# rasd3/TODA

Hardware: AMD Instinct MI355X
Metric: LiDAR training samples/sec (higher is better)
Workload: dtype f32

## Files before the change

include/toda.h:

```cpp
#ifndef TODA_H_
#define TODA_H_

#include <stddef.h>
#include <stdint.h>

#ifdef __cplusplus
extern "C" {
#endif

#define TODA_OK 0
#define TODA_EINVAL (-1)
#define TODA_EWORKSPACE (-2)
#define TODA_ELAUNCH (-3)
#define TODA_EFAULT (-4)

#define TODA_FAULT_BN2D 1u
#define TODA_FAULT_WINO 2u
#define TODA_FAULT_FPS 4u

const char* toda_last_error(void);
int toda_abi_version(void);
int toda_device_fault(void);

size_t toda_voxelize_workspace_bytes(int n_points, int max_voxels);
int toda_voxelize_hard(const float* points, int n, int c,
                       const float* range_host ,
                       const float* vsize_host ,
                       const int32_t* grid_host ,
                       int max_pts, int max_voxels,
                       float* voxels, int32_t* coords_zyx, int32_t* num_pts,
                       int32_t* m_dev, void* ws, size_t ws_bytes, void* stream);
size_t toda_voxelize_batch_workspace_bytes(int batch, int n_cap);
int toda_voxelize_batch(const float* const* points_host, const int32_t* n_points_host, int batch, int n_cap,
                        int c, int row_stride,
                        const float* range_host, const float* vsize_host, const int32_t* grid_host,
                        int max_pts, int max_voxels,
                        float* voxels, int32_t* coords_bzyx, int32_t* num_pts, int32_t* counts_dev,
                        void* ws, size_t ws_bytes, int ws_clean, void* stream);

int toda_mean_vfe_fwd(const float* voxels, const float* num_pts, int m, int p, int c,
                      float* out, void* stream);
int toda_mean_vfe_bwd(const float* grad_out, const float* num_pts, int m, int p, int c,
                      float* grad_voxels, void* stream);

size_t toda_dynvox_workspace_bytes(int n, int batch, const int32_t* grid_host, int pillar);
int toda_dynvox_count(const float* points, int n, int width, int batch, const float* range_host, const float* vsize_host,
                      const int32_t* grid_host, int pillar, int32_t* counts_dev, void* ws, size_t ws_bytes, void* stream);
int toda_dynvox_index(const float* points, int n, int width, int batch, const float* range_host, const float* vsize_host,
                      const int32_t* grid_host, int pillar, int m, int k, uint8_t* keep, int32_t* rows, int32_t* inv,
                      int32_t* seg_pts, int32_t* seg_off, int32_t* cnt, int32_t* coords, void* ws, size_t ws_bytes,
                      void* stream);
int toda_dynvox_seg_sum(const float* src, int ld, int col0, int ncol, const int32_t* rowmap, const int32_t* seg_off,
                        const int32_t* seg_pts, int m, int divide, float* out, void* stream);
int toda_dynvox_pillar_decorate(const float* points, int width, const int32_t* rows, const int32_t* inv,
                                const int32_t* coords, const float* mean, int k, const float* vsize_host,
                                const float* offset_host, int use_abs_xyz, int with_dist, float* out, int f, void* stream);
int toda_dynvox_seg_max_fwd(const float* x, int c, const int32_t* seg_off, const int32_t* seg_pts, int m, float* out,
                            int32_t* arg, void* stream);
int toda_dynvox_seg_max_bwd(const float* gout, const int32_t* arg, int m, int c, int k, float* gx, void* stream);
int toda_dynvox_gather_concat(const float* x, const float* xmax, const int32_t* inv, int k, int c, float* out, void* stream);

size_t toda_gridindex_bytes(int batch, const int32_t* shape_host );
int toda_gridindex_from_coords(const int32_t* idx, int n, const int32_t* n_dev,
                               int batch, const int32_t* shape_host,
                               void* gi, int32_t* rowof, void* stream);
int toda_gridindex_from_coords_unordered(const int32_t* idx, int n, const int32_t* n_dev,
                                         int batch, const int32_t* shape_host,
                                         void* gi, int32_t* rowof, int gi_clean, void* stream);
int toda_gridindex_clear(const int32_t* idx, int n, const int32_t* n_dev, int batch,
                         const int32_t* shape_host, void* gi, void* stream);
int toda_gridindex_from_conv(const int32_t* idx_in, int n_in, const int32_t* n_in_dev,
                             int batch, const int32_t* shape_in_host,
                             const int32_t* ksize_host, const int32_t* stride_host,
                             const int32_t* pad_host, const int32_t* shape_out_host,
                             void* gi_out, int32_t* idx_out, int32_t* n_out_dev,
                             int out_cap, void* stream);
int toda_gridindex_from_bitmap(const void* gi_in, int batch, const int32_t* shape_in_host,
                               const int32_t* ksize_host, const int32_t* stride_host,
                               const int32_t* pad_host, const int32_t* shape_out_host,
                               void* gi_out, int32_t* idx_out, int32_t* n_out_dev,
                               int out_cap, int in_rows_marked, void* stream);

int toda_rulebook_subm(const int32_t* idx, int n, int batch, const int32_t* shape_host,
                       const int32_t* ksize_host, const int32_t* dilation_host,
                       const void* gi, const int32_t* rowof,
                       int32_t* nbr, int32_t* pair_cnt, int cnt_zeroed, void* stream);
int toda_rulebook_conv(const int32_t* idx_in, int n_in, int batch,
                       const int32_t* shape_in_host, const int32_t* ksize_host,
                       const int32_t* stride_host, const int32_t* pad_host,
                       const int32_t* shape_out_host, const void* gi_out, int n_out,
                       int32_t* nbr_o2i, int32_t* nbr_i2o, int32_t* pair_cnt,
                       const int32_t* idx_out, const void* gi_in, const int32_t* rowof_in,
                       int cnt_zeroed, void* stream);

size_t toda_spconv_packed_weight_floats(int k_vol, int c_gather, int c_produce);
int toda_matrix_path(void);
int toda_set_matrix_path(int mode);
int toda_spconv_split_supported(int c_gather, int c_produce);
int toda_spconv_pack_weight(const float* w, int cout, int k_vol, int cin,
                            int transpose, int flip_k, float* wp, void* stream);
int toda_spconv_pack_weights(int n, const float* const* w_host, const int32_t* cout_host, const int32_t* k_vol_host,
                             const int32_t* cin_host, const int32_t* transpose_host, const int32_t* flip_k_host,
                             float* const* wp_host, void* stream);
int toda_spconv_gather_gemm(const float* in, int n_in, int c_gather, const float* wp,
                            const int32_t* nbr, int n_out, int k_vol, int c_produce,
                            const float* bias , float* out, void* stream);
int toda_spconv_gather_gemm_ordered(const float* in, int n_in, int c_gather, const float* wp,
                                    const int32_t* nbr, int n_out, int k_vol, int c_produce,
                                    const float* bias, float* out, const int32_t* order, void* stream);

int toda_rulebook_class_order(const int32_t* in_coords, int n_in, const int32_t* stride_host, const int32_t* padding_host,
                              int32_t* order, unsigned char* cls_sorted, void* stream);
int toda_spconv_gather_gemm_classed(const float* in, int n_in, int c_gather, const float* wp, const int32_t* nbr, int n_out,
                                    int k_vol, int c_produce, const float* bias, float* out, const int32_t* order,
                                    const unsigned char* cls_sorted, const int32_t* ksize_host, const int32_t* stride_host,
                                    const int32_t* padding_host, void* stream);
int toda_spconv_gather_gemm_compact_supported(int c_gather, int c_produce, int k_vol);
int toda_spconv_gather_gemm_compact(const float* in, int n_in, int c_gather, const float* w, int w_cout, int w_cin,
                                    int transpose, int flip_k, const int32_t* nbr, int n_out, int k_vol, int c_produce,
                                    const float* bias , float* out, void* stream);
size_t toda_spconv_gather_gemm_compact_stats_doubles(int n_out, int c_produce);
int toda_spconv_gather_gemm_compact_stats(const float* in, int n_in, int c_gather, const float* w, int w_cout, int w_cin,
                                          int transpose, int flip_k, const int32_t* nbr, int n_out, int k_vol,
                                          int c_produce, const float* bias , float* out, double* sums,
                                          size_t sums_doubles, int* blocks_out , void* stream);

size_t toda_spconv_wgrad_workspace_bytes(int n_out, int k_vol, int cin, int cout);
int toda_spconv_wgrad(const float* in, int n_in, const float* dout, const int32_t* nbr,
                      int n_out, int k_vol, int cin, int cout, float* dw,
                      void* ws, size_t ws_bytes, void* stream);
int toda_sparse_to_dense_fwd(const float* feat, const int32_t* idx, int n, int c,
                             int batch, const int32_t* shape_host, float* dense, void* stream);
int toda_sparse_to_dense_bwd(const float* grad_dense, const int32_t* idx, int n, int c,
                             int batch, const int32_t* shape_host, float* grad_feat, void* stream);

int toda_pillar_scatter_fwd(const float* feat, const int32_t* idx, int n, int c,
                            int batch, int ny, int nx, float* canvas, void* stream);
int toda_pillar_scatter_bwd(const float* grad_canvas, const int32_t* idx, int n, int c,
                            int batch, int ny, int nx, float* grad_feat, void* stream);

size_t toda_rows_reduce_doubles(int n, int c);
int toda_rows_moments(const float* x, int n, int c, double* sums ,
                      void* stream);
int toda_rows_affine_act(const float* x, const float* scale, const float* shift,
                         const float* residual , int n, int c, int relu,
                         float* y, void* stream);

int toda_bn_finalize(const double* sums , int n, int c,
                     const float* gamma, const float* beta, float* running_mean ,
                     float* running_var , float momentum, float eps, int training,
                     float* mean, float* invstd, float* scale, float* shift, void* stream);
int toda_bn_finalize_partials(double* sums, int blocks, int n, int c, const float* gamma, const float* beta,
                              float* running_mean , float* running_var , float momentum, float eps,
                              float* mean, float* invstd, float* scale, float* shift, void* stream);
int toda_rows_bn_bwd(const float* dy, const float* x, const float* stats, const float* gamma,
                     int n, int c, int relu, double* sums , float* dx,
                     void* stream);

int toda_rows_bn_bwd_res(const float* dy, const float* x, const float* residual , const float* stats,
                         const float* gamma, int n, int c, int relu, double* sums, float* dx,
                         float* dres , void* stream);
size_t toda_rows_bn_bwd_colsum_doubles(int n, int c);
int toda_rows_bn_bwd_res_colsum(const float* dy, const float* x, const float* residual , const float* stats,
                                const float* gamma, int n, int c, int relu, double* sums, float* dx,
                                float* dres , double* colsum_ws , float* dx_colsum ,
                                void* stream);

int toda_bn2d_supported(int batch, int c, int hw);
size_t toda_bn2d_sync_bytes(void);
int toda_bn2d_fwd(const float* x, int batch, int c, int hw, const float* gamma, const float* beta,
                  float* running_mean , float* running_var , float momentum, float eps, int relu,
                  float* y, float* save, void* sync , unsigned epoch, void* stream);
int toda_bn2d_bwd(const float* x, const float* dy, int batch, int c, int hw, const float* gamma, const float* beta,
                  const float* save, int relu, float* dx, float* dgamma, float* dbeta, void* sync ,
                  unsigned epoch, void* stream);
int toda_bn2d_fwd_into(const float* x, int batch, int c, int hw, const float* gamma, const float* beta,
                       float* running_mean , float* running_var , float momentum, float eps, int relu,
                       float* y, int y_channels, int y_channel0, float* save, void* sync , unsigned epoch,
                       void* stream);
int toda_bn2d_bwd_from(const float* x, const float* dy, int dy_channels, int dy_channel0, int batch, int c, int hw,
                       const float* gamma, const float* beta, const float* save, int relu, float* dx, float* dgamma,
                       float* dbeta, void* sync , unsigned epoch, void* stream);

int toda_center_assign(const float* gt_boxes, int batch, int n_gt, int code_size,
                       int num_classes, int fm_w, int fm_h,
                       const float* range_host , const float* vsize_host ,
                       int fm_stride, int max_objs, double gaussian_overlap, int min_radius,
                       float* heatmap ,
                       float* ret_boxes ,
                       int64_t* inds , int64_t* mask ,
                       void* stream);

int toda_boxes_iou_bev(const float* boxes_a, int na, const float* boxes_b, int nb,
                       float* iou , void* stream);
int toda_boxes_overlap_bev(const float* boxes_a, int na, const float* boxes_b, int nb,
                           float* overlap , void* stream);
size_t toda_nms_workspace_bytes(int n);
int toda_nms_rotated(const float* boxes_sorted, int n, float thresh, int64_t* keep ,
                     int32_t* n_keep_dev, void* ws, size_t ws_bytes, void* stream);

int toda_roi_grid_pool_bev(const float* feat, int B, int C, int H, int W, const float* rois, int N, int roi_stride,
                           float min_x, float min_y, float step_x, float step_y, int grid_size, float* out, void* stream);
int toda_roi_iou3d_max(const float* rois, int B, int N, int roi_stride, const int64_t* roi_labels, const float* gt, int M,
                       int gt_stride, int by_class, float* max_iou , int64_t* argmax , void* stream);

int toda_voxel_query(const float* new_xyz, const int32_t* new_coords, int M, const float* xyz, int N, const void* gi, const int32_t* rowof,
                     int batch, const int32_t* shape_host, float radius, const int32_t* ranges_host, int nsample, int32_t* idx,
                     uint8_t* empty, void* stream);
size_t toda_voxel_pool_moments_doubles(void);
int toda_voxel_pool_moments(const int32_t* idx, const uint8_t* empty, int M, int nsample, const float* xyz, int N, const float* new_xyz,
                            double* ws, void* stream);
int toda_voxel_pool_fwd(const float* f, int N, int C, const int32_t* idx, const uint8_t* empty, int M, int nsample, const float* xyz,
                        const float* new_xyz, const float* ab, float* out, uint8_t* arg, void* stream);
size_t toda_voxel_pool_table_bytes(int M, int nsample, int N);
int toda_voxel_pool_table(const int32_t* idx, const uint8_t* empty, int M, int nsample, int N, int32_t* off, int32_t* ent, void* ws,
                          size_t ws_bytes, void* stream);
int toda_voxel_pool_bwd_feat(const float* gout, const uint8_t* arg, int M, int nsample, int C, const int32_t* off, const int32_t* ent,
                             int N, float* gf, void* stream);
size_t toda_voxel_pool_bwd_pos_doubles(int C);
int toda_voxel_pool_bwd_pos(const float* gout, const uint8_t* arg, const int32_t* idx, const uint8_t* empty, int M, int nsample, int C,
                            const float* xyz, int N, const float* new_xyz, double* ws, float* gab, void* stream);

int toda_fps_resident_blocks(void);
size_t toda_fps_workspace_bytes(int batch, int npoint);
int toda_fps(const float* xyz, const int32_t* starts_host, int batch, int npoint, int mode, float* temp, int32_t* idx, void* ws,
             size_t ws_bytes, void* stream);
int toda_ball_query_stack(const float* xyz, int N, const int32_t* xyz_start, const float* new_xyz, const int32_t* new_start, int batch,
                          int M, int nr, const float* radii_host, const int32_t* nsample_host, int32_t* const* idx_host,
                          uint8_t* const* empty_host, void* stream);
int toda_sa_gather_fwd(const float* P, int N, int C, const float* wd, const int32_t* idx, const uint8_t* empty, int M, int nsample,
                       const float* xyz, const float* new_xyz, float* z, void* stream);
int toda_sa_gather_bwd_feat(const float* gz, int M, int nsample, int C, const int32_t* off, const int32_t* ent, int N, float* gP,
                            void* stream);
size_t toda_sa_gather_bwd_pos_doubles(int C);
int toda_sa_gather_bwd_pos(const float* gz, const int32_t* idx, const uint8_t* empty, int M, int nsample, int C, const float* xyz, int N,
                           const float* new_xyz, double* ws, float* gwd, void* stream);
int toda_sa_max_fwd(const float* y, int M, int nsample, int C, float* out, uint8_t* arg, void* stream);
int toda_sa_max_bwd(const float* g, const uint8_t* arg, int M, int nsample, int C, float* gy, void* stream);
int toda_bev_interp_fwd(const float* map, int B, int C, int H, int W, const float* xy, const int32_t* bidx, int K, float* out,
                        int32_t* taps, float* wts, void* stream);
int toda_bev_interp_bwd(const float* g, int K, int C, const int32_t* off, const int32_t* ent, const float* wts, int B, int H, int W,
                        float* gmap, void* stream);

int toda_points_in_boxes(const float* points, int n, const int32_t* n_dev, int c, const float* boxes,
                         int k, int box_stride, int mode, int32_t* flags, void* stream);
int toda_points_sector(const float* points, int n, const int32_t* n_dev, int c, double lo, double hi,
                       int32_t* flags, void* stream);
int toda_points_rect(const float* points, int n, const int32_t* n_dev, int c, const double* lo_xy_host,
                     const double* hi_xy_host, int closed, int32_t* flags, void* stream);
int toda_points_polar_cell(const float* points, int n, const int32_t* n_dev, int c, float phase,
                           const double* yaw_edges_host, int n_yaw, const double* dis_edges_host, int n_dis,
                           float dis_lo, float dis_hi, int32_t* cell, void* stream);
int toda_points_polar_select(const float* points, int n, const int32_t* n_dev, int c, double lo, double hi, int yaw_mode,
                             int dis_mode, double dis_th, const float* pitch_range_dev, int32_t* flags, void* stream);
size_t toda_points_pitch_range_workspace_bytes(void);
int toda_points_pitch_range(const float* points, int n, const int32_t* n_dev, int c, float* range_dev, void* ws,
                            size_t ws_bytes, void* stream);
int toda_points_pitch_band(const float* points, int n, const int32_t* n_dev, int c, float z_offset, float clip_lo,
                           float clip_hi, const double* edges_host, int n_bands, int32_t* band, void* stream);
size_t toda_rows_select_workspace_bytes(int n);
int toda_rows_select_append(const float* src, int n, const int32_t* n_dev, int c, const int32_t* keys,
                            int match, int invert, float* dst, int cap_rows, int32_t* cursor_dev,
                            void* ws, size_t ws_bytes, void* stream);
int toda_points_rotate_z(const float* src, int n, const int32_t* n_dev, int c, double cosv, double sinv,
                         float* dst, void* stream);
int toda_points_world_transform(const float* src, int n, const int32_t* n_dev, int c, int flip_x, int flip_y,
                                int rotate, float cosv, float sinv, int rescale, float scale, float* dst,
                                void* stream);

int toda_spconv_gather_gemm_stats_supported(int c_gather, int c_produce);
size_t toda_spconv_gather_gemm_stats_doubles(int n_out, int c_produce);
int toda_spconv_gather_gemm_stats(const float* in, int n_in, int c_gather, const float* packed_w, const int32_t* nbr,
                                  int n_out, int k_vol, int c_produce, const float* bias, float* out, double* sums,
                                  size_t sums_doubles, void* stream);
int toda_spconv_gather_gemm_stats_partials(const float* in, int n_in, int c_gather, const float* wp, const int32_t* nbr,
                                           int n_out, int k_vol, int c_produce, const float* bias , float* out,
                                           double* sums, size_t sums_doubles, int* blocks_out, void* stream);

int toda_conv3x3_supported(int batch, int cin, int cout, int H, int W);
size_t toda_conv3x3_weight_floats(int cout, int cin);
int toda_conv3x3_transform_weight(const float* w, int cout, int cin, int mode, float* u, void* stream);
size_t toda_conv3x3_workspace_bytes(void);
size_t toda_conv3x3_wgrad_workspace_bytes(int batch, int cin, int cout, int H, int W);
int toda_conv3x3_wgrad(const float* x, const float* dy, int batch, int cin, int cout, int H, int W, float* dw,
                       void* ws, size_t ws_bytes, void* stream);
int toda_conv3x3_fwd(const float* x, const float* u, const float* bias, int batch, int cin, int cout, int H,
                     int W, float* y, void* ws, size_t ws_bytes, void* stream);

int toda_conv3x3s2_supported(int batch, int cin, int cout, int H, int W);
int toda_conv3x3s2_fwd(const float* x, const float* w, int batch, int cin, int cout, int H, int W, float* y, void* stream);
int toda_conv3x3s2_dgrad(const float* dy, const float* w, int batch, int cin, int cout, int H, int W, float* dx, void* stream);
size_t toda_conv3x3s2_wgrad_workspace_bytes(int batch, int cin, int cout, int H, int W);
int toda_conv3x3s2_wgrad(const float* x, const float* dy, int batch, int cin, int cout, int H, int W, float* dw, void* ws,
                         size_t ws_bytes, void* stream);
int toda_deconv_supported(int batch, int cin, int cout, int H, int W, int s);
int toda_deconv_fwd(const float* x, const float* w, int batch, int cin, int cout, int H, int W, int s, float* y, void* stream);
int toda_deconv_dgrad(const float* dy, const float* w, int batch, int cin, int cout, int H, int W, int s, float* dx, void* stream);
size_t toda_deconv_wgrad_workspace_bytes(int batch, int cin, int cout, int H, int W, int s);
int toda_deconv_wgrad(const float* x, const float* dy, int batch, int cin, int cout, int H, int W, int s, float* dw, void* ws,
                      size_t ws_bytes, void* stream);

size_t toda_center_loss_workspace_bytes(int batch, int classes, int H, int W, int max_objs, int code_size);
int toda_center_loss_fwd(const float* hm_logits, const float* heatmap, int batch, int classes, int H, int W, int n_branch,
                         const float* const* reg_maps_host, const int32_t* reg_channels_host, const int64_t* inds,
                         const int64_t* mask, const float* target_boxes, int max_objs, int code_size,
                         const float* code_weights_host, float cls_weight, float loc_weight, float* hm_prob, float* out4,
                         void* ws, size_t ws_bytes, void* stream);
int toda_center_loss_bwd(const float* out4, const float* up_hm, const float* up_loc, int batch, int classes, int H, int W,
                         int n_branch, float* const* reg_grads_host, const int32_t* reg_channels_host, const int64_t* inds,
                         const int64_t* mask, int max_objs, int code_size, const float* code_weights_host, float cls_weight, float loc_weight,
                         float* hm_grad, const void* ws, size_t ws_bytes, void* stream);

int toda_conv3x3_narrow_supported(int batch, int cin, int cout, int H, int W);
int toda_conv3x3_narrow_fwd(int n, const float* const* x_host, const float* const* w_host, const float* const* bias_host,
                            const int32_t* cout_host, int batch, int cin, int H, int W, long long x_image_stride,
                            float* const* y_host, void* stream);
int toda_conv3x3_narrow_dgrad(int n, const float* const* dy_host, const float* const* w_host, const int32_t* cout_host,
                              int batch, int cin, int H, int W, long long dx_image_stride, float* const* dx_host, void* stream);
size_t toda_conv3x3_narrow_wgrad_workspace_bytes(int n, int batch, int cin, int H);
int toda_conv3x3_narrow_wgrad(int n, const float* const* x_host, const float* const* dy_host, const int32_t* cout_host,
                              int batch, int cin, int H, int W, long long x_image_stride, float* out, void* ws, size_t ws_bytes,
                              void* stream);

int toda_timing_begin(int capacity);
int toda_timing_end(float* ms_out_host, int cap, int* n_out_host);

int toda_clip_adam_chunk(void);
int toda_clip_adam_step(const unsigned long long* param, const unsigned long long* grad, const unsigned long long* exp_avg,
                        const unsigned long long* exp_avg_sq, const long long* numel, const int* chunk_tensor,
                        const long long* chunk_off, int n_chunks, double* partial, float* norm_out, float max_norm,
                        float lr, float beta1, float beta2, float eps, float weight_decay, int step, void* stream);

#ifdef __cplusplus
}
#endif
#endif
```

toda_amd/csrc/dense.hip:

```cpp
#include "common.h"

namespace toda {

typedef float f32x4 __attribute__((ext_vector_type(4)));

constexpr int DN_BLOCK = 256;
constexpr int DN_ROWS = 64;
constexpr int DN_CH = 32;

struct DenseGeom {
    int D, H, W;
    int pillar;
};

__device__ __forceinline__ long long spatial_offset(const int4 q, const DenseGeom& g) {
    if (g.pillar) return (long long)q.y + (long long)q.z * g.W + q.w;
    return ((long long)q.y * g.H + q.z) * g.W + q.w;
}

template <bool FWD>
__global__ void __launch_bounds__(DN_BLOCK)
dense_tile_kernel(float* __restrict__ feat, const int4* __restrict__ idx, int n, int c, DenseGeom g,
                  float* __restrict__ dense) {
    __shared__ float tile[DN_CH][DN_ROWS + 1];
    __shared__ long long base[DN_ROWS];
    const int row0 = blockIdx.x * DN_ROWS, c0 = blockIdx.y * DN_CH;
    const long long vol = (long long)g.D * g.H * g.W;
    if (threadIdx.x < DN_ROWS) {
        const int r = row0 + threadIdx.x;
        long long b = -1;
        if (r < n) {
            const int4 q = idx[r];
            b = (long long)q.x * c * vol + spatial_offset(q, g);
        }
        base[threadIdx.x] = b;
    }
    const int fr = threadIdx.x >> 2, fc = (threadIdx.x & 3) * 8;
    const int dr = threadIdx.x & 63, dc = threadIdx.x >> 6;
    if (FWD) {
        if (row0 + fr < n) {
#pragma unroll
            for (int j = 0; j < 8; ++j) {
                const int ch = c0 + fc + j;
                tile[fc + j][fr] = ch < c ? feat[(size_t)(row0 + fr) * c + ch] : 0.f;
            }
        }
        __syncthreads();
        const long long b = base[dr];
        if (b >= 0) {
#pragma unroll
            for (int j = 0; j < DN_CH / 4; ++j) {
                const int ch = dc + 4 * j;
                if (c0 + ch < c) dense[b + (long long)(c0 + ch) * vol] = tile[ch][dr];
            }
        }
    } else {
        __syncthreads();
        const long long b = base[dr];
#pragma unroll
        for (int j = 0; j < DN_CH / 4; ++j) {
            const int ch = dc + 4 * j;
            tile[ch][dr] = (b >= 0 && c0 + ch < c) ? dense[b + (long long)(c0 + ch) * vol] : 0.f;
        }
        __syncthreads();
        if (row0 + fr < n) {
#pragma unroll
            for (int j = 0; j < 8; ++j) {
                const int ch = c0 + fc + j;
                if (ch < c) feat[(size_t)(row0 + fr) * c + ch] = tile[fc + j][fr];
            }
        }
    }
}

#ifndef TODA_MOM_ROWS
#define TODA_MOM_ROWS 256
#endif
constexpr int MOM_ROWS = TODA_MOM_ROWS;
constexpr int MOM_MAX_BLOCKS = 2048;

template <class Load>
__device__ __forceinline__ void rows_reduce2(int n, int c, int rows_per_block, Load load, double* __restrict__ sums) {
    __shared__ float sh[2][DN_BLOCK][4];
    const int lanes = c >> 2;
    const int rows_par = DN_BLOCK / lanes;
    const int cl = threadIdx.x % lanes, rsub = threadIdx.x / lanes;
    const int row_begin = blockIdx.x * rows_per_block;
    const int row_end = min(n, row_begin + rows_per_block);
    f32x4 s0 = f32x4{0.f, 0.f, 0.f, 0.f}, t0 = s0, s1 = s0, t1 = s0;
    int r = row_begin + rsub;
    for (; r + rows_par < row_end; r += 2 * rows_par) {
        f32x4 a, b, a2, b2;
        load(r, cl, a, b);
        load(r + rows_par, cl, a2, b2);
        s0 += a;
        t0 += b;
        s1 += a2;
        t1 += b2;
    }
    if (r < row_end) {
        f32x4 a, b;
        load(r, cl, a, b);
        s0 += a;
        t0 += b;
    }
    s0 += s1;
    t0 += t1;
#pragma unroll
    for (int j = 0; j < 4; ++j) {
        sh[0][threadIdx.x][j] = s0[j];
        sh[1][threadIdx.x][j] = t0[j];
    }
    __syncthreads();
    if (threadIdx.x < 2 * c) {
        const int q = threadIdx.x / c, ch = threadIdx.x % c;
        double acc = 0.0;
        for (int j = 0; j < rows_par; ++j) acc += sh[q][j * lanes + (ch >> 2)][ch & 3];
        sums[2 * c + (size_t)(q * c + ch) * gridDim.x + blockIdx.x] = acc;
    }
}

__global__ void __launch_bounds__(DN_BLOCK)
fold_partials_kernel(double* __restrict__ sums, int blocks, int cols) {
    __shared__ double part[DN_BLOCK];
    const double* src = sums + cols + (size_t)blockIdx.x * blocks;
    double acc = 0.0;
    for (int g = threadIdx.x; g < blocks; g += DN_BLOCK) acc += src[g];
    part[threadIdx.x] = acc;
    __syncthreads();
    for (int w = DN_BLOCK / 2; w > 0; w >>= 1) {
        if (threadIdx.x < w) part[threadIdx.x] += part[threadIdx.x + w];
        __syncthreads();
    }
    if (threadIdx.x == 0) sums[blockIdx.x] = part[0];
}

static inline void reduce_plan(int n, int* blocks, int* rows_per_block) {
    const int g = cdiv(n > 0 ? n : 1, MOM_ROWS);
    *blocks = g < MOM_MAX_BLOCKS ? g : MOM_MAX_BLOCKS;
    *rows_per_block = cdiv(n > 0 ? n : 1, *blocks);
}

__global__ void __launch_bounds__(DN_BLOCK)
rows_moments_kernel(const float* __restrict__ x, int n, int c, int rows_per_block, double* __restrict__ sums) {
    const f32x4* x4 = reinterpret_cast<const f32x4*>(x);
    const int lanes = c >> 2;
    rows_reduce2(n, c, rows_per_block, [&](int r, int cl, f32x4& a, f32x4& b) {
        a = x4[(size_t)r * lanes + cl];
        b = a * a;
    }, sums);
}

constexpr int EW_BLOCKS = 2048;

__global__ void __launch_bounds__(DN_BLOCK)
rows_affine_act_kernel(const f32x4* __restrict__ x, const float* __restrict__ scale, const float* __restrict__ shift,
                       const f32x4* __restrict__ res, long long n4, int c, int relu, f32x4* __restrict__ y) {
    const long long t0 = (long long)blockIdx.x * DN_BLOCK + threadIdx.x;
    const long long stride = (long long)gridDim.x * DN_BLOCK;
    const int ch = (int)((t0 * 4) % c);
    const f32x4 sc = *reinterpret_cast<const f32x4*>(scale + ch), sf = *reinterpret_cast<const f32x4*>(shift + ch);
    for (long long t = t0; t < n4; t += stride) {
        f32x4 v = x[t] * sc + sf;
        if (res) v += res[t];
        if (relu) {
#pragma unroll
            for (int j = 0; j < 4; ++j) v[j] = fmaxf(v[j], 0.f);
        }
        y[t] = v;
    }
}

__global__ void __launch_bounds__(DN_BLOCK)
rows_bn_bwd_reduce_kernel(const float* __restrict__ dy, const float* __restrict__ x, const float* __restrict__ res,
                          const float* __restrict__ stats, int n, int c, int relu, int rows_per_block,
                          double* __restrict__ sums) {
    const f32x4* dy4 = reinterpret_cast<const f32x4*>(dy);
    const f32x4* x4 = reinterpret_cast<const f32x4*>(x);
    const f32x4* r4 = reinterpret_cast<const f32x4*>(res);
    const int lanes = c >> 2;
    const int cl0 = threadIdx.x % lanes;
    const f32x4 mu = reinterpret_cast<const f32x4*>(stats)[cl0];
    const f32x4 is = reinterpret_cast<const f32x4*>(stats + c)[cl0];
    const f32x4 sc = reinterpret_cast<const f32x4*>(stats + 2 * c)[cl0];
    const f32x4 sf = reinterpret_cast<const f32x4*>(stats + 3 * c)[cl0];
    rows_reduce2(n, c, rows_per_block, [&](int r, int cl, f32x4& a, f32x4& b) {
        const f32x4 g = dy4[(size_t)r * lanes + cl], xv = x4[(size_t)r * lanes + cl];
        const f32x4 rv = r4 ? r4[(size_t)r * lanes + cl] : f32x4{0.f, 0.f, 0.f, 0.f};
#pragma unroll
        for (int j = 0; j < 4; ++j) {
            float pre = xv[j] * sc[j] + sf[j];
            if (r4) pre += rv[j];
            const float dz = (relu && !(pre > 0.f)) ? 0.f : g[j];
            a[j] = dz;
            b[j] = dz * ((xv[j] - mu[j]) * is[j]);
        }
    }, sums);
}

__global__ void __launch_bounds__(DN_BLOCK)
rows_bn_bwd_apply_kernel(const f32x4* __restrict__ dy, const f32x4* __restrict__ x, const f32x4* __restrict__ res,
                         const float* __restrict__ stats, const float* __restrict__ gamma, double* __restrict__ sums,
                         long long n4, int c, int n, int relu, f32x4* __restrict__ dx, f32x4* __restrict__ dres,
                         double* __restrict__ colsum_part) {
    if (blockIdx.x == 0 && threadIdx.x < 2 * c) reinterpret_cast<float*>(sums + 2 * c)[threadIdx.x] = (float)sums[threadIdx.x];
    const long long t0 = (long long)blockIdx.x * DN_BLOCK + threadIdx.x;
    const long long stride = (long long)gridDim.x * DN_BLOCK;
    const int ch = (int)((t0 * 4) % c);
    const float inv_n = 1.0f / (float)n;
    const f32x4 mu = *reinterpret_cast<const f32x4*>(stats + ch);
    const f32x4 is = *reinterpret_cast<const f32x4*>(stats + c + ch);
    const f32x4 sc = *reinterpret_cast<const f32x4*>(stats + 2 * c + ch);
    const f32x4 sf = *reinterpret_cast<const f32x4*>(stats + 3 * c + ch);
    const f32x4 ga = *reinterpret_cast<const f32x4*>(gamma + ch);
    f32x4 m1, m2;
#pragma unroll
    for (int j = 0; j < 4; ++j) {
        m1[j] = (float)(sums[ch + j] * (double)inv_n);
        m2[j] = (float)(sums[c + ch + j] * (double)inv_n);
    }
    const f32x4 k1 = ga * is, k2 = is * m2;
    f32x4 csum = {0.f, 0.f, 0.f, 0.f};
    for (long long t = t0; t < n4; t += stride) {
        const f32x4 g = dy[t], xv = x[t];
        const f32x4 rv = res ? res[t] : f32x4{0.f, 0.f, 0.f, 0.f};
        f32x4 out, dzv;
#pragma unroll
        for (int j = 0; j < 4; ++j) {
            float pre = xv[j] * sc[j] + sf[j];
            if (res) pre += rv[j];
            const float dz = (relu && !(pre > 0.f)) ? 0.f : g[j];
            dzv[j] = dz;
            out[j] = k1[j] * (dz - m1[j] - (xv[j] - mu[j]) * k2[j]);
        }
        dx[t] = out;
        csum += out;
        if (dres) dres[t] = dzv;
    }
    if (colsum_part) {
        __shared__ float cs[DN_BLOCK][4];
#pragma unroll
        for (int j = 0; j < 4; ++j) cs[threadIdx.x][j] = csum[j];
        __syncthreads();
        if (threadIdx.x < c) {
            const int lanes = c >> 2, cl = threadIdx.x >> 2, j = threadIdx.x & 3;
            double acc = 0.0;
            for (int t = cl; t < DN_BLOCK; t += lanes) acc += (double)cs[t][j];
            colsum_part[(size_t)threadIdx.x * gridDim.x + blockIdx.x] = acc;
        }
    }
}

__global__ void __launch_bounds__(DN_BLOCK)
colsum_fold_kernel(const double* __restrict__ part, int blocks, float* __restrict__ out) {
    __shared__ double sh[DN_BLOCK];
    const double* src = part + (size_t)blockIdx.x * blocks;
    double acc = 0.0;
    for (int g = threadIdx.x; g < blocks; g += DN_BLOCK) acc += src[g];
    sh[threadIdx.x] = acc;
    __syncthreads();
    for (int w = DN_BLOCK / 2; w > 0; w >>= 1) {
        if (threadIdx.x < w) sh[threadIdx.x] += sh[threadIdx.x + w];
        __syncthreads();
    }
    if (threadIdx.x == 0) out[blockIdx.x] = (float)sh[0];
}

__global__ void __launch_bounds__(DN_BLOCK)
bn_finalize_kernel(const double* __restrict__ sums, int n, int c, const float* __restrict__ gamma,
                   const float* __restrict__ beta, float* __restrict__ running_mean, float* __restrict__ running_var,
                   float momentum, float eps, int training, float* __restrict__ mean_out, float* __restrict__ invstd_out,
                   float* __restrict__ scale_out, float* __restrict__ shift_out) {
    const int ch = threadIdx.x;
    if (ch >= c) return;
    float mean, var;
    if (training) {
        const double m = sums[ch] / (double)n;
        double v = sums[c + ch] / (double)n - m * m;
        if (v < 0.0) v = 0.0;
        mean = (float)m;
        var = (float)v;
        if (running_mean) {
            const double unbiased = n > 1 ? v * (double)n / (double)(n - 1) : v;
            running_mean[ch] = (1.0f - momentum) * running_mean[ch] + momentum * mean;
            running_var[ch] = (1.0f - momentum) * running_var[ch] + momentum * (float)unbiased;
        }
    } else {
        mean = running_mean[ch];
        var = running_var[ch];
    }
    const float invstd = 1.0f / sqrtf(var + eps);
    const float g = gamma ? gamma[ch] : 1.0f, b = beta ? beta[ch] : 0.0f;
    mean_out[ch] = mean;
    invstd_out[ch] = invstd;
    scale_out[ch] = g * invstd;
    shift_out[ch] = b - mean * g * invstd;
}

__global__ void __launch_bounds__(DN_BLOCK)
bn_fold_finalize_kernel(double* __restrict__ sums, int blocks, int n, int c, const float* __restrict__ gamma,
                        const float* __restrict__ beta, float* __restrict__ running_mean, float* __restrict__ running_var,
                        float momentum, float eps, float* __restrict__ mean_out, float* __restrict__ invstd_out,
                        float* __restrict__ scale_out, float* __restrict__ shift_out) {
    __shared__ double part[DN_BLOCK];
    const int ch = blockIdx.x;
    double tot[2];
#pragma unroll
    for (int q = 0; q < 2; ++q) {
        const double* src = sums + 2 * c + (size_t)(q * c + ch) * blocks;
        double acc = 0.0;
        for (int g = threadIdx.x; g < blocks; g += DN_BLOCK) acc += src[g];
        part[threadIdx.x] = acc;
        __syncthreads();
        for (int w = DN_BLOCK / 2; w > 0; w >>= 1) {
            if (threadIdx.x < w) part[threadIdx.x] += part[threadIdx.x + w];
            __syncthreads();
        }
        tot[q] = part[0];
        __syncthreads();
    }
    if (threadIdx.x != 0) return;
    sums[ch] = tot[0];
    sums[c + ch] = tot[1];
    const double m = tot[0] / (double)n;
    double v = tot[1] / (double)n - m * m;
    if (v < 0.0) v = 0.0;
    const float mean = (float)m, var = (float)v;
    if (running_mean) {
        const double unbiased = n > 1 ? v * (double)n / (double)(n - 1) : v;
        running_mean[ch] = (1.0f - momentum) * running_mean[ch] + momentum * mean;
        running_var[ch] = (1.0f - momentum) * running_var[ch] + momentum * (float)unbiased;
    }
    const float invstd = 1.0f / sqrtf(var + eps);
    const float g = gamma ? gamma[ch] : 1.0f, b = beta ? beta[ch] : 0.0f;
    mean_out[ch] = mean;
    invstd_out[ch] = invstd;
    scale_out[ch] = g * invstd;
    shift_out[ch] = b - mean * g * invstd;
}

static int ew_grid(long long n4, int c) {
    long long blocks = (n4 + DN_BLOCK - 1) / DN_BLOCK;
    if (blocks > EW_BLOCKS) blocks = EW_BLOCKS;
    while ((blocks * DN_BLOCK * 4) % c != 0) ++blocks;
    return (int)blocks;
}

static int scatter_common(bool fwd, float* feat, const int32_t* idx, int n, int c, int batch, DenseGeom g,
                          float* dense, hipStream_t s) {
    TODA_CHECK_ARG(n >= 0 && c >= 1 && batch >= 1, "sparse<->dense: bad sizes n=%d c=%d batch=%d", n, c, batch);
    const size_t total = (size_t)batch * c * g.D * g.H * g.W;
    if (fwd) TODA_HIP(hipMemsetAsync(dense, 0, total * sizeof(float), s));
    if (n == 0) return TODA_OK;
    const dim3 grid(cdiv(n, DN_ROWS), cdiv(c, DN_CH));
    if (fwd)
        hipLaunchKernelGGL(HIP_KERNEL_NAME(dense_tile_kernel<true>), grid, dim3(DN_BLOCK), 0, s, feat, (const int4*)idx, n,
                           c, g, dense);
    else
        hipLaunchKernelGGL(HIP_KERNEL_NAME(dense_tile_kernel<false>), grid, dim3(DN_BLOCK), 0, s, feat, (const int4*)idx, n,
                           c, g, dense);
    TODA_LAUNCH_CHECK();
    return TODA_OK;
}

}

using namespace toda;

extern "C" int toda_sparse_to_dense_fwd(const float* feat, const int32_t* idx, int n, int c, int batch,
                                        const int32_t* shape_host, float* dense, void* stream) {
    const DenseGeom g{shape_host[0], shape_host[1], shape_host[2], 0};
    return scatter_common(true, const_cast<float*>(feat), idx, n, c, batch, g, dense, (hipStream_t)stream);
}
extern "C" int toda_sparse_to_dense_bwd(const float* grad_dense, const int32_t* idx, int n, int c, int batch,
                                        const int32_t* shape_host, float* grad_feat, void* stream) {
    const DenseGeom g{shape_host[0], shape_host[1], shape_host[2], 0};
    return scatter_common(false, grad_feat, idx, n, c, batch, g, const_cast<float*>(grad_dense), (hipStream_t)stream);
}
extern "C" int toda_pillar_scatter_fwd(const float* feat, const int32_t* idx, int n, int c, int batch, int ny, int nx,
                                       float* canvas, void* stream) {
    const DenseGeom g{1, ny, nx, 1};
    return scatter_common(true, const_cast<float*>(feat), idx, n, c, batch, g, canvas, (hipStream_t)stream);
}
extern "C" int toda_pillar_scatter_bwd(const float* grad_canvas, const int32_t* idx, int n, int c, int batch, int ny,
                                       int nx, float* grad_feat, void* stream) {
    const DenseGeom g{1, ny, nx, 1};
    return scatter_common(false, grad_feat, idx, n, c, batch, g, const_cast<float*>(grad_canvas), (hipStream_t)stream);
}

extern "C" size_t toda_rows_reduce_doubles(int n, int c) {
    int blocks, rpb;
    reduce_plan(n, &blocks, &rpb);
    return (size_t)2 * c * (1 + (size_t)blocks);
}

extern "C" int toda_rows_moments(const float* x, int n, int c, double* sums, void* stream) {
    hipStream_t s = (hipStream_t)stream;
    TODA_CHECK_ARG(c >= 4 && c % 4 == 0 && c <= DN_BLOCK / 2 && DN_BLOCK % c == 0,
                   "rows_moments: channels must be a multiple of 4 dividing 256, <= 128 (got %d)", c);
    if (n <= 0) {
        TODA_HIP(hipMemsetAsync(sums, 0, 2 * c * sizeof(double), s));
        return TODA_OK;
    }
    int blocks, rpb;
    reduce_plan(n, &blocks, &rpb);
    hipLaunchKernelGGL(rows_moments_kernel, dim3(blocks), dim3(DN_BLOCK), 0, s, x, n, c, rpb, sums);
    hipLaunchKernelGGL(fold_partials_kernel, dim3(2 * c), dim3(DN_BLOCK), 0, s, sums, blocks, 2 * c);
    TODA_LAUNCH_CHECK();
    return TODA_OK;
}

extern "C" int toda_rows_affine_act(const float* x, const float* scale, const float* shift, const float* residual,
                                    int n, int c, int relu, float* y, void* stream) {
    TODA_CHECK_ARG(c >= 4 && c % 4 == 0 && c <= 1024, "rows_affine_act: channels must be a multiple of 4, <= 1024 (got %d)", c);
    if (n <= 0) return TODA_OK;
    const long long n4 = (long long)n * c / 4;
    hipLaunchKernelGGL(rows_affine_act_kernel, dim3(ew_grid(n4, c)), dim3(DN_BLOCK), 0, (hipStream_t)stream,
                       (const f32x4*)x, scale, shift, (const f32x4*)residual, n4, c, relu, (f32x4*)y);
    TODA_LAUNCH_CHECK();
    return TODA_OK;
}

extern "C" size_t toda_rows_bn_bwd_colsum_doubles(int n, int c) {
    if (n <= 0 || c < 4) return 1;
    return (size_t)c * ew_grid((long long)n * c / 4, c);
}

extern "C" int toda_rows_bn_bwd_res_colsum(const float* dy, const float* x, const float* residual, const float* stats,
                                           const float* gamma, int n, int c, int relu, double* sums, float* dx, float* dres,
                                           double* colsum_ws, float* dx_colsum, void* stream) {
    hipStream_t s = (hipStream_t)stream;
    TODA_CHECK_ARG((colsum_ws == nullptr) == (dx_colsum == nullptr), "rows_bn_bwd: colsum workspace and result go together");
    TODA_CHECK_ARG(c >= 4 && c % 4 == 0 && c <= DN_BLOCK / 2 && DN_BLOCK % c == 0,
                   "rows_bn_bwd: channels must be a multiple of 4 dividing 256, <= 128 (got %d)", c);
    if (n <= 0) {
        TODA_HIP(hipMemsetAsync(sums, 0, 3 * c * sizeof(double), s));
        if (dx_colsum) TODA_HIP(hipMemsetAsync(dx_colsum, 0, c * sizeof(float), s));
        return TODA_OK;
    }
    int blocks, rpb;
    reduce_plan(n, &blocks, &rpb);
    hipLaunchKernelGGL(rows_bn_bwd_reduce_kernel, dim3(blocks), dim3(DN_BLOCK), 0, s, dy, x, residual, stats, n, c, relu, rpb, sums);
    hipLaunchKernelGGL(fold_partials_kernel, dim3(2 * c), dim3(DN_BLOCK), 0, s, sums, blocks, 2 * c);
    const long long n4 = (long long)n * c / 4;
    const int grid = ew_grid(n4, c);
    hipLaunchKernelGGL(rows_bn_bwd_apply_kernel, dim3(grid), dim3(DN_BLOCK), 0, s, (const f32x4*)dy,
                       (const f32x4*)x, (const f32x4*)residual, stats, gamma, sums, n4, c, n, relu, (f32x4*)dx, (f32x4*)dres, colsum_ws);
    if (dx_colsum) hipLaunchKernelGGL(colsum_fold_kernel, dim3(c), dim3(DN_BLOCK), 0, s, (const double*)colsum_ws, grid, dx_colsum);
    TODA_LAUNCH_CHECK();
    return TODA_OK;
}

extern "C" int toda_rows_bn_bwd_res(const float* dy, const float* x, const float* residual, const float* stats,
                                    const float* gamma, int n, int c, int relu, double* sums, float* dx, float* dres,
                                    void* stream) {
    return toda_rows_bn_bwd_res_colsum(dy, x, residual, stats, gamma, n, c, relu, sums, dx, dres, nullptr, nullptr, stream);
}

extern "C" int toda_rows_bn_bwd(const float* dy, const float* x, const float* stats, const float* gamma, int n, int c,
                                int relu, double* sums, float* dx, void* stream) {
    return toda_rows_bn_bwd_res(dy, x, nullptr, stats, gamma, n, c, relu, sums, dx, nullptr, stream);
}

extern "C" int toda_bn_finalize_partials(double* sums, int blocks, int n, int c, const float* gamma, const float* beta,
                                         float* running_mean, float* running_var, float momentum, float eps, float* mean,
                                         float* invstd, float* scale, float* shift, void* stream) {
    TODA_CHECK_ARG(sums && mean && invstd && scale && shift, "bn_finalize_partials: null argument");
    TODA_CHECK_ARG(c >= 1 && c <= DN_BLOCK && blocks >= 1 && n >= 1, "bn_finalize_partials: channels must be <= 256, blocks and rows >= 1 (got %d, %d, %d)", c,
                   blocks, n);
    TODA_CHECK_ARG((running_mean == nullptr) == (running_var == nullptr), "bn_finalize_partials: running_mean and running_var go together");
    hipLaunchKernelGGL(bn_fold_finalize_kernel, dim3(c), dim3(DN_BLOCK), 0, (hipStream_t)stream, sums, blocks, n, c, gamma, beta, running_mean,
                       running_var, momentum, eps, mean, invstd, scale, shift);
    TODA_LAUNCH_CHECK();
    return TODA_OK;
}

extern "C" int toda_bn_finalize(const double* sums, int n, int c, const float* gamma, const float* beta,
                                float* running_mean, float* running_var, float momentum, float eps, int training,
                                float* mean, float* invstd, float* scale, float* shift, void* stream) {
    TODA_CHECK_ARG(c >= 1 && c <= DN_BLOCK, "bn_finalize: channels must be <= 256 (got %d)", c);
    TODA_CHECK_ARG(training || (running_mean && running_var), "bn_finalize: eval mode needs running statistics");
    hipLaunchKernelGGL(bn_finalize_kernel, dim3(1), dim3(DN_BLOCK), 0, (hipStream_t)stream, sums, n, c, gamma, beta,
                       running_mean, running_var, momentum, eps, training, mean, invstd, scale, shift);
    TODA_LAUNCH_CHECK();
    return TODA_OK;
}
```

toda_amd/csrc/spconv.hip:

```cpp
#include <stdlib.h>

#include <type_traits>

#include <hip/hip_ext.h>

#include <mutex>
#include <vector>

#include "common.h"


namespace toda {

typedef float f32x4 __attribute__((ext_vector_type(4)));

constexpr int SC_BLOCK = 256;

static int tiles_pow2(int channels) {
    int t = (channels + 15) / 16, p = 1;
    while (p < t) p <<= 1;
    return p;
}

__global__ void __launch_bounds__(SC_BLOCK)
// ... 861 lines not shown
    };
    const unsigned long long in_addr = (unsigned long long)in;
    const u32x4 in_desc = {(unsigned)__builtin_amdgcn_readfirstlane((int)(unsigned)in_addr),
                           (unsigned)__builtin_amdgcn_readfirstlane((int)((unsigned)(in_addr >> 32) & 0xFFFFu)),
                           (unsigned)__builtin_amdgcn_readfirstlane((int)((unsigned)n_in * (unsigned)cg * 4u)), 0x00020000u};
    constexpr int LOADS = VEC ? Q : 4 * Q;
    auto prepare = [&](int k, Stage& st) {
        const int i = row_ok ? ids[k] : -1;
        const unsigned long long vote = __ballot(i >= 0);
        int* qi = q_id[wv][k % (CG_DEPTH + 1)];
        int* qr = q_row[wv][k % (CG_DEPTH + 1)];
        st.cnt = __popcll(vote);
        const unsigned long long below = (1ull << lane) - 1;
        const int pos = i >= 0 ? __popcll(vote & below) : st.cnt + __popcll(~vote & below);
        qi[pos] = i;
        qr[pos] = i >= 0 ? lane : 64;
        __builtin_amdgcn_wave_barrier();
        const int src = qi[c];
        const bool ok = src >= 0;
        const unsigned base = (unsigned)src * (unsigned)cg * 4u;
#pragma unroll
        for (int q = 0; q < Q; ++q) {
            if constexpr (VEC) {
                const unsigned off = (ok && 16 * q + 4 * g < cg) ? base + (unsigned)(16 * q + 4 * g) * 4u : OOB;
                asm volatile("buffer_load_dwordx4 %0, %1, %2, 0 offen" : "=v"(st.a[q]) : "v"(off), "s"(in_desc) : "memory");
            } else {
#pragma unroll
                for (int j = 0; j < 4; ++j) {
                    const unsigned off = (ok && 16 * q + 4 * g + j < cg) ? base + (unsigned)(16 * q + 4 * g + j) * 4u : OOB;
                    asm volatile("buffer_load_dword %0, %1, %2, 0 offen" : "=v"(st.s[q][j]) : "v"(off), "s"(in_desc) : "memory");
                }
            }
        }
    };
    auto multiply_add = [&](int k, int tt, int cnt, const f32x4 (&a)[Q]) {
        f32x4 r = f32x4{0.f, 0.f, 0.f, 0.f};
#pragma unroll
        for (int q = 0; q < Q; ++q) {
            const f32x4 b = w_lds[(k * Q + q) * 64 + lane];
#pragma unroll
            for (int j = 0; j < 4; ++j) r = __builtin_amdgcn_mfma_f32_16x16x4f32(a[q][j], b[j], r, 0, 0, 0);
        }
        const i32x4 rows = *reinterpret_cast<const i32x4*>(q_row[wv][k % (CG_DEPTH + 1)] + 16 * tt + 4 * g);
        float* const acc_w = acc_lds + wv * 65 * 16 + c;
        float old[4];
#pragma unroll
        for (int reg = 0; reg < 4; ++reg) old[reg] = acc_w[rows[reg] * 16];
#pragma unroll
        for (int reg = 0; reg < 4; ++reg) acc_w[rows[reg] * 16] = old[reg] + r[reg];
        __builtin_amdgcn_wave_barrier();
    };

    asm volatile("s_waitcnt vmcnt(0)" ::: "memory");
    float dummy = 0.f;
    Stage st[CG_DEPTH];
#pragma unroll
    for (int k = 0; k < CG_DEPTH; ++k) prepare(k, st[k]);
#pragma unroll
    for (int k = 0; k < CG_K; ++k) {
        Stage& ring = st[k % CG_DEPTH];
        if constexpr (VEC) {
            if constexpr (Q == 1)
                asm volatile("s_waitcnt vmcnt(%1)" : "+v"(ring.a[0]) : "n"((CG_DEPTH - 1) * LOADS));
            else
                asm volatile("s_waitcnt vmcnt(%2)" : "+v"(ring.a[0]), "+v"(ring.a[1]) : "n"((CG_DEPTH - 1) * LOADS));
        } else {
#pragma unroll
            for (int q = 0; q < Q; ++q)
                asm volatile("s_waitcnt vmcnt(%4)" : "+v"(ring.s[q][0]), "+v"(ring.s[q][1]), "+v"(ring.s[q][2]), "+v"(ring.s[q][3]) : "n"((CG_DEPTH - 1) * LOADS));
        }
        Stage cur = ring;
        if constexpr (!VEC) {
#pragma unroll
            for (int q = 0; q < Q; ++q) cur.a[q] = f32x4{ring.s[q][0], ring.s[q][1], ring.s[q][2], ring.s[q][3]};
        }
        if (k + CG_DEPTH < CG_K) {
            prepare(k + CG_DEPTH, ring);
        } else {
#pragma unroll
            for (int d = 0; d < LOADS; ++d)
                asm volatile("buffer_load_dword %0, %1, %2, 0 offen" : "+v"(dummy) : "v"(OOB), "s"(in_desc) : "memory");
        }
        multiply_add(k, 0, cur.cnt, cur.a);
        for (int tt = 1; 16 * tt < cur.cnt; ++tt) {
            const int src = q_id[wv][k % (CG_DEPTH + 1)][16 * tt + c];
            const bool ok = src >= 0;
            const unsigned base = (unsigned)src * (unsigned)cg * 4u;
            f32x4 a[Q];
#pragma unroll
            for (int q = 0; q < Q; ++q) {
                if constexpr (VEC) {
                    a[q] = __builtin_bit_cast(f32x4, __builtin_amdgcn_raw_buffer_load_b128(in_rsrc, (ok && 16 * q + 4 * g < cg) ? base + (unsigned)(16 * q + 4 * g) * 4u : OOB, 0, 0));
                } else {
#pragma unroll
                    for (int j = 0; j < 4; ++j)
                        a[q][j] = __builtin_bit_cast(float, __builtin_amdgcn_raw_buffer_load_b32(in_rsrc, (ok && 16 * q + 4 * g + j < cg) ? base + (unsigned)(16 * q + 4 * g + j) * 4u : OOB, 0, 0));
                }
            }
            multiply_add(k, tt, cur.cnt, a);
        }
    }
    asm volatile("s_waitcnt vmcnt(0)" : "+v"(dummy)::"memory");
    __builtin_amdgcn_wave_barrier();
    if (stats) {
        __shared__ float st_sh[2][16][16];
        __syncthreads();
        static_assert(CG_BLOCK % 256 == 0, "one (row group, channel) pair per thread of each 256-thread slice");
        for (int base = 0; base < CG_ROWS; base += 256) {
            float sm = 0.f, sq = 0.f;
            if (tid < 256) {
                const int ch = tid & 15, rg = tid >> 4;
#pragma unroll
                for (int i = 0; i < 16; ++i) {
                    const int R = base + rg * 16 + i;
                    if (blockIdx.x * CG_ROWS + R < n_out) {
                        const float v = acc_lds[((R >> 6) * 65 + (R & 63)) * 16 + ch];
                        sm += v;
                        sq += v * v;
                    }
                }
                st_sh[0][rg][ch] = sm;
                st_sh[1][rg][ch] = sq;
            }
            __syncthreads();
            if (tid < 32) {
                const int qq = tid >> 4, ch = tid & 15;
                double a = 0.0;
#pragma unroll
                for (int rg = 0; rg < 16; ++rg) a += (double)st_sh[qq][rg][ch];
                if (co0 + ch < cp) {
                    double* dst = stats + 2 * cp + (size_t)(qq * cp + co0 + ch) * gridDim.x + blockIdx.x;
                    *dst = base == 0 ? a : *dst + a;
                }
            }
            __syncthreads();
        }
    }
#pragma unroll
    for (int it = 0; it < 4; ++it) {
        const int r = it * 16 + (lane >> 2), c4 = (lane & 3) * 4;
        const f32x4 v = *reinterpret_cast<const f32x4*>(&acc_lds[(wv * 65 + r) * 16 + c4]);
        const int row = row0 + r;
        if (row < n_out) {
            float* dst = out + (size_t)row * cp + co0 + c4;
            if (co0 + c4 + 3 < cp) {
                *reinterpret_cast<f32x4*>(dst) = v;
            } else {
#pragma unroll
                for (int j = 0; j < 4; ++j)
                    if (co0 + c4 + j < cp) dst[j] = v[j];
            }
        }
    }
}

static void wgrad_plan(int n_out, int k_vol, int cin, int cout, int* chunks, int* rows_per_chunk) {
    static const int env_chunks = getenv("TODA_WG_CHUNKS") ? atoi(getenv("TODA_WG_CHUNKS")) : 0;
    int max_chunks = env_chunks > 0 ? env_chunks : ((tiles_pow2(cin) * tiles_pow2(cout) >= 16) ? 48 : 144);
    if (env_chunks <= 0 && k_vol <= 9) max_chunks *= 2;
    int ch = k_vol <= 9 ? n_out / 1024 : n_out / 2048;
    if (ch < 1) ch = 1;
    if (ch > max_chunks) ch = max_chunks;
    if (env_chunks <= 0 && k_vol > 9 && max_chunks == 48 && n_out / 4096 > 48) ch = n_out / 4096 < 96 ? n_out / 4096 : 96;
    if (ch >= 8) ch = (ch + 7) / 8 * 8;
    int rpc = (n_out + ch - 1) / ch;
    rpc = (rpc + 15) / 16 * 16;
    if (rpc < 16) rpc = 16;
    *rows_per_chunk = rpc;
    *chunks = n_out > 0 ? (n_out + rpc - 1) / rpc : 1;
}

}

#include "spconv_split.cuh"

using namespace toda;

#include <atomic>
static std::atomic<int> g_matrix_path{-1};
static int matrix_path() {
    int m = g_matrix_path.load(std::memory_order_relaxed);
    if (m < 0) {
        const char* e = getenv("TODA_MM");
        m = (e && (e[0] == 'n' || e[0] == '0')) ? 0 : 1;
        g_matrix_path.store(m, std::memory_order_relaxed);
    }
    return m;
}
static inline bool use_split(int c_gather, int c_produce) { return matrix_path() == 1 && toda::split_shape_ok(c_gather, c_produce); }

extern "C" int toda_matrix_path(void) { return matrix_path(); }
extern "C" int toda_set_matrix_path(int mode) {
    TODA_CHECK_ARG(mode == 0 || mode == 1, "set_matrix_path: mode must be 0 (native) or 1 (split)");
    g_matrix_path.store(mode, std::memory_order_relaxed);
    return TODA_OK;
}
extern "C" int toda_spconv_split_supported(int c_gather, int c_produce) { return toda::split_shape_ok(c_gather, c_produce) ? 1 : 0; }

extern "C" size_t toda_spconv_packed_weight_floats(int k_vol, int c_gather, int c_produce) {
    const size_t native = (size_t)k_vol * tiles_pow2(c_gather) * tiles_pow2(c_produce) * 256;
    if (!toda::split_shape_ok(c_gather, c_produce)) return native;
    const size_t split = toda::split_packed_bytes(k_vol, c_gather, c_produce) / 4;
    return split > native ? split : native;
}

static void split_pack_fill(toda::SplitPackBatch& b, int i, const float* w, int cout, int k_vol, int cin, int transpose, int flip_k, float* wp) {
    const int cgather = transpose ? cout : cin, cprod = transpose ? cin : cout;
    b.w[i] = w, b.wps[i] = reinterpret_cast<toda::u32x4*>(wp), b.cout[i] = cout, b.K[i] = k_vol, b.cin[i] = cin;
    b.transpose[i] = transpose != 0, b.flip[i] = flip_k != 0;
    b.KC[i] = (unsigned char)(cgather / 32), b.NT[i] = (unsigned char)(cprod / 16);
}

extern "C" int toda_spconv_pack_weight(const float* w, int cout, int k_vol, int cin, int transpose, int flip_k,
                                       float* wp, void* stream) {
    TODA_CHECK_ARG(cout >= 1 && cin >= 1 && k_vol >= 1, "pack_weight: bad shape");
    const int cgather = transpose ? cout : cin, cprod = transpose ? cin : cout;
    TODA_CHECK_ARG(cgather <= 128 && cprod <= 128, "pack_weight: channels > 128 unsupported (gather %d, produce %d)",
                   cgather, cprod);
    if (use_split(cgather, cprod)) {
        toda::SplitPackBatch b = {};
        split_pack_fill(b, 0, w, cout, k_vol, cin, transpose, flip_k, wp);
        hipLaunchKernelGGL(split_pack_batch_kernel, dim3(cdiv((long long)k_vol * b.KC[0] * b.NT[0] * 192, SC_BLOCK), 1), dim3(SC_BLOCK), 0,
                           (hipStream_t)stream, b);
        TODA_LAUNCH_CHECK();
        return TODA_OK;
    }
    const int Q = tiles_pow2(cgather), NT = tiles_pow2(cprod);
    const long long total = (long long)k_vol * Q * NT * 256;
    hipLaunchKernelGGL(pack_weight_kernel, dim3(cdiv(total, SC_BLOCK)), dim3(SC_BLOCK), 0, (hipStream_t)stream, w, cout,
                       k_vol, cin, transpose, flip_k, Q, NT, wp);
    TODA_LAUNCH_CHECK();
    return TODA_OK;
}

extern "C" int toda_spconv_pack_weights(int n, const float* const* w, const int32_t* cout, const int32_t* k_vol, const int32_t* cin,
                                        const int32_t* transpose, const int32_t* flip_k, float* const* wp, void* stream) {
    TODA_CHECK_ARG(n >= 0 && w && cout && k_vol && cin && transpose && flip_k && wp, "pack_weights: null argument");
    PackBatch b = {};
    toda::SplitPackBatch sb = {};
    int m = 0, sm = 0;
    long long most = 0, smost = 0;
    auto flush = [&]() -> int {
        if (m > 0) {
            hipLaunchKernelGGL(pack_weight_batch_kernel, dim3(cdiv(most, SC_BLOCK), m), dim3(SC_BLOCK), 0, (hipStream_t)stream, b);
            TODA_LAUNCH_CHECK();
        }
        m = 0, most = 0;
        return TODA_OK;
    };
    auto sflush = [&]() -> int {
        if (sm > 0) {
            hipLaunchKernelGGL(split_pack_batch_kernel, dim3(cdiv(smost, SC_BLOCK), sm), dim3(SC_BLOCK), 0, (hipStream_t)stream, sb);
            TODA_LAUNCH_CHECK();
        }
        sm = 0, smost = 0;
        return TODA_OK;
    };
    for (int s = 0; s < n; ++s) {
        TODA_CHECK_ARG(w[s] && wp[s] && cout[s] >= 1 && cin[s] >= 1 && k_vol[s] >= 1, "pack_weights: bad segment %d", s);
        const int cgather = transpose[s] ? cout[s] : cin[s], cprod = transpose[s] ? cin[s] : cout[s];
        TODA_CHECK_ARG(cgather <= 128 && cprod <= 128, "pack_weights: channels > 128 unsupported (segment %d)", s);
        if (use_split(cgather, cprod)) {
            split_pack_fill(sb, sm, w[s], cout[s], k_vol[s], cin[s], transpose[s], flip_k[s], wp[s]);
            const long long total = (long long)k_vol[s] * sb.KC[sm] * sb.NT[sm] * 192;
            if (total > smost) smost = total;
            if (++sm == toda::SPLIT_PACK_MAX_SEG) {
                const int rc = sflush();
                if (rc != TODA_OK) return rc;
            }
            continue;
        }
        const int i = m;
        b.w[i] = w[s], b.wp[i] = wp[s], b.cout[i] = cout[s], b.K[i] = k_vol[s], b.cin[i] = cin[s];
        b.transpose[i] = transpose[s] != 0, b.flip[i] = flip_k[s] != 0;
        b.Q[i] = (unsigned char)tiles_pow2(cgather), b.NT[i] = (unsigned char)tiles_pow2(cprod);
        const long long total = (long long)k_vol[s] * b.Q[i] * b.NT[i] * 256;
        if (total > most) most = total;
        if (++m == PACK_MAX_SEG) {
            const int rc = flush();
            if (rc != TODA_OK) return rc;
        }
    }
    {
        const int rc = flush();
        if (rc != TODA_OK) return rc;
    }
    return sflush();
}

namespace toda {
__global__ void fold_partials_kernel(double* __restrict__ sums, int blocks, int cols);
}
static thread_local int* g_stats_blocks_out = nullptr;
static void fold_or_defer(double* stats, int blocks, int c_produce, hipStream_t s) {
    if (g_stats_blocks_out) {
        *g_stats_blocks_out = blocks;
        return;
    }
    hipLaunchKernelGGL(toda::fold_partials_kernel, dim3(2 * c_produce), dim3(256), 0, s, stats, blocks, 2 * c_produce);
}

static int gather_gemm_impl(const float* in, int n_in, int c_gather, const float* wp, const int32_t* nbr, int n_out, int k_vol,
                            int c_produce, const float* bias, float* out, const int32_t* order, double* stats, void* stream,
                            const unsigned char* cls_sorted = nullptr, const toda::GatherClasses* cls_table = nullptr);

namespace toda {
constexpr int CLS_ROWS = 8192, CLS_PER = CLS_ROWS / 256;
struct ClassGeom {
    int stride[3], pad[3];
};
__global__ void __launch_bounds__(256)
class_order_kernel(const int4* __restrict__ coords, int n, const ClassGeom gm, int32_t* __restrict__ order, unsigned char* __restrict__ cls_sorted) {
    __shared__ int cnt[8][256 + 1];
    const int base = blockIdx.x * CLS_ROWS, t = threadIdx.x;
    unsigned char c[CLS_PER];
    int mine[8] = {0, 0, 0, 0, 0, 0, 0, 0};
#pragma unroll
    for (int i = 0; i < CLS_PER; ++i) {
        const int r = base + t * CLS_PER + i;
        int cl = 0;
        if (r < n) {
            const int4 v = coords[r];
            cl = (((v.y + gm.pad[0]) % gm.stride[0]) * gm.stride[1] + (v.z + gm.pad[1]) % gm.stride[1]) * gm.stride[2] + (v.w + gm.pad[2]) % gm.stride[2];
            ++mine[cl & 7];
        }
        c[i] = (unsigned char)cl;
    }
#pragma unroll
    for (int k = 0; k < 8; ++k) cnt[k][t] = mine[k];
    __syncthreads();
    if (t < 8) {
        int run = 0;
        for (int j = 0; j < 256; ++j) {
            const int v = cnt[t][j];
            cnt[t][j] = run;
            run += v;
        }
        cnt[t][256] = run;
    }
    __syncthreads();
    int cls_base[8], run = 0;
#pragma unroll
    for (int k = 0; k < 8; ++k) {
        cls_base[k] = run + cnt[k][t];
        run += cnt[k][256];
    }
#pragma unroll
    for (int i = 0; i < CLS_PER; ++i) {
        const int r = base + t * CLS_PER + i;
        if (r >= n) break;
        const int k = c[i] & 7;
        int pos = 0;
#pragma unroll
        for (int q = 0; q < 8; ++q)
            if (q == k) pos = cls_base[q]++;
        order[base + pos] = r;
        cls_sorted[base + pos] = c[i];
    }
}

static int class_table(const int32_t* ksize, const int32_t* stride, const int32_t* pad, GatherClasses* out) {
    const int n_class = stride[0] * stride[1] * stride[2];
    if (n_class < 1 || n_class > 8 || ksize[0] * ksize[1] * ksize[2] > 27) return -1;
    *out = GatherClasses{};
    for (int rz = 0; rz < stride[0]; ++rz)
        for (int ry = 0; ry < stride[1]; ++ry)
            for (int rx = 0; rx < stride[2]; ++rx) {
                const int c = (rz * stride[1] + ry) * stride[2] + rx;
                int m = 0;
                for (int kz = 0; kz < ksize[0]; ++kz)
                    for (int ky = 0; ky < ksize[1]; ++ky)
                        for (int kx = 0; kx < ksize[2]; ++kx)
                            if (kz % stride[0] == rz && ky % stride[1] == ry && kx % stride[2] == rx)
                                out->k[c][m++] = (unsigned char)((kz * ksize[1] + ky) * ksize[2] + kx);
                out->count[c] = (unsigned char)m;
            }
    return 0;
}
}

extern "C" int toda_rulebook_class_order(const int32_t* in_coords, int n_in, const int32_t* stride, const int32_t* padding, int32_t* order,
                                         unsigned char* cls_sorted, void* stream) {
    TODA_CHECK_ARG(in_coords && stride && padding && order && cls_sorted && n_in >= 0, "rulebook_class_order: null argument");
    ClassGeom gm;
    for (int a = 0; a < 3; ++a) {
        TODA_CHECK_ARG(stride[a] >= 1 && stride[a] <= 2 && padding[a] >= 0, "rulebook_class_order: stride 1 or 2 per axis (got %d)", stride[a]);
        gm.stride[a] = stride[a], gm.pad[a] = padding[a];
    }
    if (n_in == 0) return TODA_OK;
    hipLaunchKernelGGL(class_order_kernel, dim3(cdiv(n_in, CLS_ROWS)), dim3(256), 0, (hipStream_t)stream, (const int4*)in_coords, n_in, gm, order,
                       cls_sorted);
    TODA_LAUNCH_CHECK();
    return TODA_OK;
}

extern "C" int toda_spconv_gather_gemm_classed(const float* in, int n_in, int c_gather, const float* wp, const int32_t* nbr, int n_out, int k_vol,
                                               int c_produce, const float* bias, float* out, const int32_t* order,
                                               const unsigned char* cls_sorted, const int32_t* ksize, const int32_t* stride,
                                               const int32_t* padding, void* stream) {
    TODA_CHECK_ARG(order && cls_sorted && ksize && stride && padding, "gather_gemm_classed: null argument");
    TODA_CHECK_ARG(ksize[0] * ksize[1] * ksize[2] == k_vol, "gather_gemm_classed: kernel size does not match the table's %d offsets", k_vol);
    GatherClasses table;
    TODA_CHECK_ARG(class_table(ksize, stride, padding, &table) == 0, "gather_gemm_classed: needs <= 8 residue classes and <= 27 offsets");
    return gather_gemm_impl(in, n_in, c_gather, wp, nbr, n_out, k_vol, c_produce, bias, out, order, nullptr, stream, cls_sorted, &table);
}

namespace toda {
struct LaunchTimer {
    std::vector<hipEvent_t> ev;
    int used = 0;
    bool on = false;
};
static LaunchTimer g_timer;
static std::mutex g_timer_mu;
static inline void timer_next(hipEvent_t* start, hipEvent_t* stop) {
    *start = *stop = nullptr;
    if (!g_timer.on) return;
    std::lock_guard<std::mutex> lock(g_timer_mu);
    if (!g_timer.on || 2 * (g_timer.used + 1) > (int)g_timer.ev.size()) return;
    *start = g_timer.ev[2 * g_timer.used];
    *stop = g_timer.ev[2 * g_timer.used + 1];
    g_timer.used++;
}
}

#define GG_LAUNCH(kernel, grid, block, shmem, stream, ...)                                              \
    do {                                                                                               \
        hipEvent_t t0_, t1_;                                                                           \
        toda::timer_next(&t0_, &t1_);                                                                  \
        hipExtLaunchKernelGGL(kernel, grid, block, shmem, stream, t0_, t1_, 0, __VA_ARGS__);           \
    } while (0)

extern "C" int toda_timing_begin(int capacity) {
    TODA_CHECK_ARG(capacity > 0 && capacity <= (1 << 20), "timing_begin: capacity in (0, 2^20]");
    std::lock_guard<std::mutex> lock(toda::g_timer_mu);
    for (hipEvent_t e : g_timer.ev) (void)hipEventDestroy(e);
    g_timer.ev.assign((size_t)2 * capacity, nullptr);
    for (auto& e : g_timer.ev) TODA_HIP(hipEventCreate(&e));
    g_timer.used = 0;
    g_timer.on = true;
    return TODA_OK;
}

extern "C" int toda_timing_end(float* ms_out, int cap, int* n_out) {
    std::lock_guard<std::mutex> lock(toda::g_timer_mu);
    g_timer.on = false;
    const int n = g_timer.used < cap ? g_timer.used : cap;
    for (int i = 0; i < n; ++i) {
        TODA_HIP(hipEventSynchronize(g_timer.ev[2 * i + 1]));
        TODA_HIP(hipEventElapsedTime(&ms_out[i], g_timer.ev[2 * i], g_timer.ev[2 * i + 1]));
    }
    if (n_out) *n_out = g_timer.used;
    for (hipEvent_t e : g_timer.ev) (void)hipEventDestroy(e);
    g_timer.ev.clear();
    g_timer.used = 0;
    return TODA_OK;
}

namespace toda {
__global__ void fold_partials_kernel(double* __restrict__ sums, int blocks, int cols);
static bool gg_stats_supported(int c_gather, int c_produce) {
    const int Q = tiles_pow2(c_gather), NT = tiles_pow2(c_produce);
    return (c_gather & 3) == 0 && Q >= 2 && NT >= Q && Q * NT <= 32 && !(Q == 8 && NT == 8) && c_produce % 4 == 0 && c_produce == 16 * NT;
}
}



extern "C" int toda_spconv_gather_gemm_ordered(const float* in, int n_in, int c_gather, const float* wp, const int32_t* nbr,
                                               int n_out, int k_vol, int c_produce, const float* bias, float* out,
                                               const int32_t* order, void* stream) {
    return gather_gemm_impl(in, n_in, c_gather, wp, nbr, n_out, k_vol, c_produce, bias, out, order, nullptr, stream);
}

extern "C" int toda_spconv_gather_gemm_stats_supported(int c_gather, int c_produce) {
    return gg_stats_supported(c_gather, c_produce) ? 1 : 0;
}

extern "C" size_t toda_spconv_gather_gemm_stats_doubles(int n_out, int c_produce) {
    return (size_t)2 * c_produce * (1 + (size_t)cdiv(n_out > 0 ? n_out : 1, 64));
}

extern "C" int toda_spconv_gather_gemm_stats(const float* in, int n_in, int c_gather, const float* wp, const int32_t* nbr,
                                             int n_out, int k_vol, int c_produce, const float* bias, float* out, double* sums,
                                             size_t sums_doubles, void* stream) {
    TODA_CHECK_ARG(sums != nullptr && gg_stats_supported(c_gather, c_produce) && n_out > 0 && n_in > 0,
                   "gather_gemm_stats: unsupported channel pair (%d -> %d) or empty table", c_gather, c_produce);
    TODA_CHECK_ARG(sums_doubles >= toda_spconv_gather_gemm_stats_doubles(n_out, c_produce), "gather_gemm_stats: statistics buffer too small");
    return gather_gemm_impl(in, n_in, c_gather, wp, nbr, n_out, k_vol, c_produce, bias, out, nullptr, sums, stream);
}

extern "C" int toda_spconv_gather_gemm_stats_partials(const float* in, int n_in, int c_gather, const float* wp, const int32_t* nbr,
                                                      int n_out, int k_vol, int c_produce, const float* bias, float* out, double* sums,
                                                      size_t sums_doubles, int* blocks_out, void* stream) {
    TODA_CHECK_ARG(sums != nullptr && blocks_out != nullptr && gg_stats_supported(c_gather, c_produce) && n_out > 0 && n_in > 0,
                   "gather_gemm_stats_partials: unsupported channel pair (%d -> %d), empty table or null argument", c_gather, c_produce);
    TODA_CHECK_ARG(sums_doubles >= toda_spconv_gather_gemm_stats_doubles(n_out, c_produce), "gather_gemm_stats_partials: statistics buffer too small");
    *blocks_out = 0;
    g_stats_blocks_out = blocks_out;
    const int rc = gather_gemm_impl(in, n_in, c_gather, wp, nbr, n_out, k_vol, c_produce, bias, out, nullptr, sums, stream);
    g_stats_blocks_out = nullptr;
    if (rc == TODA_OK && *blocks_out <= 0) {
        set_error("gather_gemm_stats_partials: the launch took no statistics");
        return TODA_EINVAL;
    }
    return rc;
}


static int gather_gemm_impl(const float* in, int n_in, int c_gather, const float* wp, const int32_t* nbr, int n_out, int k_vol,
                            int c_produce, const float* bias, float* out, const int32_t* order, double* stats, void* stream,
                            const unsigned char* cls_sorted, const toda::GatherClasses* cls_table) {
    toda::GatherClasses classes = {};
    if (cls_sorted && cls_table) classes = *cls_table;
    else cls_sorted = nullptr;
    TODA_CHECK_ARG(c_gather >= 1 && c_gather <= 128 && c_produce >= 1 && c_produce <= 128,
                   "gather_gemm: channels must be in [1,128] (gather %d, produce %d)", c_gather, c_produce);
    TODA_CHECK_ARG(n_out >= 0 && n_in >= 0 && k_vol >= 1, "gather_gemm: bad sizes");
    TODA_CHECK_ARG((unsigned long long)n_in * c_gather * 4ull < 0xFFFFFFF0ull, "gather_gemm: gathered table must be < 4 GiB");
    if (n_out == 0) return TODA_OK;
    if (n_in == 0) {
        TODA_CHECK_ARG(bias == nullptr, "gather_gemm: empty input with bias is unsupported");
        TODA_HIP(hipMemsetAsync(out, 0, (size_t)n_out * c_produce * sizeof(float), (hipStream_t)stream));
        return TODA_OK;
    }
    const int Q = tiles_pow2(c_gather), NT = tiles_pow2(c_produce);
    hipStream_t s = (hipStream_t)stream;
    const bool vec_ok = (c_gather & 3) == 0;
    static const int env_lds_raw = getenv("TODA_GG_LDS") ? atoi(getenv("TODA_GG_LDS")) : 1;
    const int env_lds = env_lds_raw == 2 ? 1 : (env_lds_raw == 1 ? (Q >= 2 && NT >= Q) : 0);
    if (use_split(c_gather, c_produce)) {
        TODA_CHECK_ARG(k_vol >= 1 && !(cls_sorted && stats), "gather_gemm (split path): no statistics on a class-sorted launch");
        const toda::u32x4* wps = reinterpret_cast<const toda::u32x4*>(wp);
#define SPL(KK, SS, NN, BB, WW)                                                                                                            \
    GG_LAUNCH(HIP_KERNEL_NAME(gg_split_kernel<KK, SS, NN, 2, BB, WW, (NN == 2)>), dim3(cdiv(cdiv(n_out, 32), BB / 64)), dim3(BB), 0, s, in, n_in, wps, \
              nbr, n_out, k_vol, c_produce, bias, out, order, stats, cls_sorted, classes)
        const int blk = 256;
        const int kc = c_gather / 32, nt = c_produce / 16;
        if (0) {}
        else if (kc == 1 && nt == 2) SPL(1, 1, 2, 256, 4);
        else if (kc == 1 && nt == 4) SPL(1, 1, 4, 256, 4);
        else if (kc == 1 && nt == 8) SPL(1, 1, 8, 256, 3);
        else if (kc == 2 && nt == 2) SPL(2, 1, 2, 256, 4);
        else if (kc == 2 && nt == 4) SPL(2, 1, 4, 256, 4);
        else if (kc == 2 && nt == 8) SPL(2, 1, 8, 256, 3);
        else if (kc == 4 && nt == 2) SPL(4, 1, 2, 256, 4);
        else if (kc == 4 && nt == 4) SPL(4, 1, 4, 256, 4);
        else SPL(4, 1, 8, 256, 3);
#undef SPL
        TODA_LAUNCH_CHECK();
        if (stats) {
            fold_or_defer(stats, cdiv(cdiv(n_out, 32), blk / 64), c_produce, s);
            TODA_LAUNCH_CHECK();
        }
        return TODA_OK;
    }
    if (vec_ok && Q == 8 && NT == 8 && !cls_sorted) {
        GG_LAUNCH(HIP_KERNEL_NAME(gather_gemm_lds_kernel<8, 8, 1, true, false, 512>), dim3(cdiv(cdiv(n_out, 16), 8)), dim3(512), 0, s, in, n_in,
                  c_gather, wp, nbr, n_out, k_vol, c_produce, bias, out, order, stats);
        TODA_LAUNCH_CHECK();
        return TODA_OK;
    }
    if ((env_lds || stats) && !cls_sorted && vec_ok && Q * NT <= 32) {
#define GL(QQ, NN, RR)                                                                                                   \
    GG_LAUNCH(HIP_KERNEL_NAME(gather_gemm_lds_kernel<QQ, NN, RR, true, true, SC_BLOCK, false, (QQ <= 4 && NN <= 4 && RR == 2)>), \
              dim3(cdiv(cdiv(n_out, 16 * RR), SC_BLOCK / 64)), dim3(SC_BLOCK), 0, s, in, n_in, c_gather, wp, nbr, n_out, k_vol,  \
              c_produce, bias, out, order, stats)
#define GL_ROW(QQ)                 \
    switch (NT) {                  \
        case 1: GL(QQ, 1, 2); break; \
        case 2: GL(QQ, 2, 2); break; \
        case 4: GL(QQ, 4, 2); break; \
        default: GL(QQ, 8, 1); break; \
    }
        switch (Q) {
            case 1: GL_ROW(1); break;
            case 2: GL_ROW(2); break;
            case 4: GL_ROW(4); break;
            default: GL_ROW(8); break;
        }
#undef GL_ROW
#undef GL
        TODA_LAUNCH_CHECK();
        if (stats) {
            const int rr = NT >= 8 ? 1 : 2;
            fold_or_defer(stats, cdiv(cdiv(n_out, 16 * rr), SC_BLOCK / 64), c_produce, s);
            TODA_LAUNCH_CHECK();
        }
        return TODA_OK;
    }
    TODA_CHECK_ARG(stats == nullptr, "gather_gemm: statistics requested on a launch shape without the fused epilogue");
#define GGV(QQ, NN, RR, VV)                                                                                           \
    if (cls_sorted && (VV))                                                                                           \
        GG_LAUNCH(HIP_KERNEL_NAME(gather_gemm_kernel<QQ, NN, RR, false, true, true>),                                 \
                  dim3(cdiv(cdiv(n_out, 16 * RR), SC_BLOCK / 64)), dim3(SC_BLOCK), 0, s, in, n_in, c_gather, wp, nbr, \
                  n_out, k_vol, c_produce, bias, out, 0, order, cls_sorted, classes);                                 \
    else                                                                                                              \
        GG_LAUNCH(HIP_KERNEL_NAME(gather_gemm_kernel<QQ, NN, RR, false, VV>),                                         \
                  dim3(cdiv(cdiv(n_out, 16 * RR), SC_BLOCK / 64)), dim3(SC_BLOCK), 0, s, in, n_in, c_gather, wp, nbr, \
                  n_out, k_vol, c_produce, bias, out, 0, order, nullptr, classes)
#define GG_ROW(QQ)                                                                      \
    switch (NT) {                                                                       \
        case 1: GGV(QQ, 1, 2, true); break;                                             \
        case 2: GGV(QQ, 2, 2, true); break;                                             \
        case 4: GGV(QQ, 4, 2, true); break;                                             \
        default:                                                                        \
            if (QQ < 8) { GGV(QQ, 8, 1, true); } else { GGV(QQ, 8, 2, true); }           \
            break;          \
    }
    if (!vec_ok) {
        TODA_CHECK_ARG(Q == 1, "gather_gemm: gathered channel counts above 16 must be multiples of 4 (got %d)", c_gather);
        switch (NT) {
            case 1: GGV(1, 1, 2, false); break;
            case 2: GGV(1, 2, 2, false); break;
            case 4: GGV(1, 4, 2, false); break;
            default: GGV(1, 8, 1, false); break;
        }
        TODA_LAUNCH_CHECK();
        return TODA_OK;
    }
    switch (Q) {
        case 1: GG_ROW(1); break;
        case 2: GG_ROW(2); break;
        case 4: GG_ROW(4); break;
        default: GG_ROW(8); break;
    }
#undef GG_ROW
#undef GGV
    TODA_LAUNCH_CHECK();
    return TODA_OK;
}

extern "C" int toda_spconv_gather_gemm(const float* in, int n_in, int c_gather, const float* wp, const int32_t* nbr,
                                       int n_out, int k_vol, int c_produce, const float* bias, float* out,
                                       void* stream) {
    return toda_spconv_gather_gemm_ordered(in, n_in, c_gather, wp, nbr, n_out, k_vol, c_produce, bias, out, nullptr, stream);
}

extern "C" int toda_spconv_gather_gemm_compact_supported(int c_gather, int c_produce, int k_vol) {
    return k_vol == CG_K && c_gather >= 1 && c_gather <= 32 && c_produce >= 1 && c_produce <= 32 && c_produce % 4 == 0;
}

static int gather_gemm_compact_impl(const float* in, int n_in, int c_gather, const float* w, int w_cout, int w_cin, int transpose,
                                    int flip_k, const int32_t* nbr, int n_out, int k_vol, int c_produce, const float* bias,
                                    float* out, double* stats, void* stream) {
    TODA_CHECK_ARG(toda_spconv_gather_gemm_compact_supported(c_gather, c_produce, k_vol),
                   "gather_gemm_compact: needs K = 27, <= 32 gathered and <= 32 produced channels (a multiple of 4) (got K %d, %d -> %d)", k_vol, c_gather,
                   c_produce);
    TODA_CHECK_ARG((transpose ? w_cout : w_cin) == c_gather && (transpose ? w_cin : w_cout) == c_produce,
                   "gather_gemm_compact: weight [%d][27][%d] (transpose %d) does not map %d -> %d channels", w_cout, w_cin, transpose, c_gather, c_produce);
    TODA_CHECK_ARG(n_out >= 0 && n_in >= 0, "gather_gemm_compact: bad sizes");
    TODA_CHECK_ARG((unsigned long long)n_in * c_gather * 4ull < 0xFFFFFFF0ull && (unsigned long long)n_out * CG_K * 4ull < 0xFFFFFFF0ull,
                   "gather_gemm_compact: gathered table and neighbour table must be < 4 GiB each");
    if (n_out == 0) return TODA_OK;
    hipStream_t s = (hipStream_t)stream;
    const dim3 grid(cdiv(n_out, CG_ROWS), cdiv(c_produce, 16));
    const bool vec = c_gather % 4 == 0;
#define CG_LAUNCH(QQ, VV)                                                                                                       \
    hipLaunchKernelGGL(HIP_KERNEL_NAME(gather_gemm_compact_kernel<QQ, VV>), grid, dim3(CG_BLOCK), 0, s, in, n_in, c_gather, w, w_cout, w_cin, \
                       transpose, flip_k, nbr, n_out, c_produce, bias, out, stats)
    if (c_gather <= 16) {
        if (vec) CG_LAUNCH(1, true);
        else CG_LAUNCH(1, false);
    } else {
        if (vec) CG_LAUNCH(2, true);
        else CG_LAUNCH(2, false);
    }
#undef CG_LAUNCH
    TODA_LAUNCH_CHECK();
    return TODA_OK;
}

extern "C" int toda_spconv_gather_gemm_compact(const float* in, int n_in, int c_gather, const float* w, int w_cout, int w_cin, int transpose,
                                               int flip_k, const int32_t* nbr, int n_out, int k_vol, int c_produce, const float* bias,
                                               float* out, void* stream) {
    return gather_gemm_compact_impl(in, n_in, c_gather, w, w_cout, w_cin, transpose, flip_k, nbr, n_out, k_vol, c_produce, bias, out, nullptr, stream);
}

extern "C" size_t toda_spconv_gather_gemm_compact_stats_doubles(int n_out, int c_produce) {
    return (size_t)2 * c_produce * (1 + (size_t)cdiv(n_out > 0 ? n_out : 1, CG_ROWS));
}

extern "C" int toda_spconv_gather_gemm_compact_stats(const float* in, int n_in, int c_gather, const float* w, int w_cout, int w_cin,
                                                     int transpose, int flip_k, const int32_t* nbr, int n_out, int k_vol, int c_produce,
                                                     const float* bias, float* out, double* sums, size_t sums_doubles, int* blocks_out,
                                                     void* stream) {
    TODA_CHECK_ARG(sums != nullptr && n_out > 0, "gather_gemm_compact_stats: null statistics buffer or no output rows");
    TODA_CHECK_ARG(sums_doubles >= toda_spconv_gather_gemm_compact_stats_doubles(n_out, c_produce), "gather_gemm_compact_stats: statistics buffer too small");
    const int rc = gather_gemm_compact_impl(in, n_in, c_gather, w, w_cout, w_cin, transpose, flip_k, nbr, n_out, k_vol, c_produce, bias, out, sums, stream);
    if (rc != TODA_OK) return rc;
    const int blocks = cdiv(n_out, CG_ROWS);
    if (blocks_out) {
        *blocks_out = blocks;
        return TODA_OK;
    }
    hipLaunchKernelGGL(toda::fold_partials_kernel, dim3(2 * c_produce), dim3(256), 0, (hipStream_t)stream, sums, blocks, 2 * c_produce);
    TODA_LAUNCH_CHECK();
    return TODA_OK;
}

extern "C" size_t toda_spconv_wgrad_workspace_bytes(int n_out, int k_vol, int cin, int cout) {
    int chunks, rpc;
    wgrad_plan(n_out, k_vol, cin, cout, &chunks, &rpc);
    return align_up((size_t)chunks * k_vol * cin * cout * sizeof(float), 256);
}

extern "C" int toda_spconv_wgrad(const float* in, int n_in, const float* dout, const int32_t* nbr, int n_out, int k_vol,
                                 int cin, int cout, float* dw, void* ws, size_t ws_bytes, void* stream) {
    TODA_CHECK_ARG(cin >= 1 && cin <= 128 && cout >= 1 && cout <= 128, "wgrad: channels must be in [1,128]");
    TODA_CHECK_ARG(n_out >= 0 && n_in >= 0 && k_vol >= 1, "wgrad: bad sizes");
    TODA_CHECK_ARG((unsigned long long)n_in * cin * 4ull < 0xFFFFFFF0ull && (unsigned long long)n_out * cout * 4ull < 0xFFFFFFF0ull,
                   "wgrad: feature tables must be < 4 GiB");
    hipStream_t s = (hipStream_t)stream;
    const long long elems = (long long)cout * k_vol * cin;
    if (n_out == 0 || n_in == 0) {
        TODA_HIP(hipMemsetAsync(dw, 0, elems * sizeof(float), s));
        return TODA_OK;
    }
    int chunks, rpc;
    wgrad_plan(n_out, k_vol, cin, cout, &chunks, &rpc);
    const size_t need = (size_t)chunks * elems * sizeof(float);
    if (ws_bytes < need) {
        set_error("wgrad: workspace %zu < required %zu", ws_bytes, need);
        return TODA_EWORKSPACE;
    }
    const int MT = tiles_pow2(cin), NT = tiles_pow2(cout);
    static const int env_sub = getenv("TODA_WG_SUB") ? atoi(getenv("TODA_WG_SUB")) : 7;
    int mtb = MT < 4 ? MT : 4, ntb = NT < 4 ? NT : 4;
    if (MT == 8 && (env_sub & 1)) mtb = 8;
    if (NT == 8 && (env_sub & 2)) ntb = 8;
    const int nsub_m = MT / mtb, nsub_n = NT / ntb;
    float* slab = (float*)ws;
    static const int env_wg_xcd = getenv("TODA_WG_XCD") ? atoi(getenv("TODA_WG_XCD")) : 1;
    const int chunks_launch = env_wg_xcd ? (chunks + 7) / 8 * 8 : chunks;
    const int xcd_chunks = env_wg_xcd ? chunks_launch : -chunks;
    if (matrix_path() == 1 && toda::wgrad_split_shape_ok(cin, cout)) {
        const dim3 g(chunks_launch * k_vol);
#define WGS(MM, NN)                                                                                                                       \
    hipLaunchKernelGGL(HIP_KERNEL_NAME(wgrad_split_kernel<MM, NN>), g, dim3(SC_BLOCK), 0, s, in, n_in, dout, nbr, n_out, k_vol, rpc, slab, \
                       xcd_chunks)
        if (cin == 128 && cout == 128) hipLaunchKernelGGL(HIP_KERNEL_NAME(wgrad_split_kernel<4, 4, 2, 2>), g, dim3(SC_BLOCK), 0, s, in, n_in, dout, nbr, n_out, k_vol, rpc, slab, xcd_chunks);
        else if (cin == 64 && cout == 128) hipLaunchKernelGGL(HIP_KERNEL_NAME(wgrad_split_kernel<4, 4, 1, 2>), g, dim3(SC_BLOCK), 0, s, in, n_in, dout, nbr, n_out, k_vol, rpc, slab, xcd_chunks);
        else if (cin == 128 && cout == 64) hipLaunchKernelGGL(HIP_KERNEL_NAME(wgrad_split_kernel<4, 4, 2, 1>), g, dim3(SC_BLOCK), 0, s, in, n_in, dout, nbr, n_out, k_vol, rpc, slab, xcd_chunks);
        else if (cin == 32 && cout == 32) WGS(2, 2);
        else if (cin == 32) WGS(2, 4);
        else if (cout == 32) WGS(4, 2);
        else WGS(4, 4);
#undef WGS
        hipLaunchKernelGGL(wgrad_reduce_kernel, dim3(cdiv(elems, SC_BLOCK)), dim3(SC_BLOCK), 0, s, slab, chunks, elems, dw);
        TODA_LAUNCH_CHECK();
        return TODA_OK;
    }
    if (MT == 8 && NT == 8 && (env_sub & 4)) {
        if (cin == 128 && cout == 128)
            hipLaunchKernelGGL(HIP_KERNEL_NAME(wgrad_kernel<4, 4, true, true>), dim3(chunks_launch * k_vol), dim3(SC_BLOCK), 0, s, in, n_in, cin, dout,
                               cout, nbr, n_out, k_vol, rpc, MT, NT, 2, slab, xcd_chunks);
        else
            hipLaunchKernelGGL(HIP_KERNEL_NAME(wgrad_kernel<4, 4, true>), dim3(chunks_launch * k_vol), dim3(SC_BLOCK), 0, s, in, n_in, cin, dout,
                               cout, nbr, n_out, k_vol, rpc, MT, NT, 2, slab, xcd_chunks);
        hipLaunchKernelGGL(wgrad_reduce_kernel, dim3(cdiv(elems, SC_BLOCK)), dim3(SC_BLOCK), 0, s, slab, chunks, elems, dw);
        TODA_LAUNCH_CHECK();
        return TODA_OK;
    }
    const dim3 grid(chunks_launch * k_vol * nsub_m * nsub_n);
    const bool exact = cin == 16 * MT && cout == 16 * NT;
#define WG(MM, NN)                                                                                                  \
    if (exact)                                                                                                      \
        hipLaunchKernelGGL(HIP_KERNEL_NAME(wgrad_kernel<MM, NN, false, true>), grid, dim3(SC_BLOCK), 0, s, in, n_in, cin, dout, cout, nbr, \
                           n_out, k_vol, rpc, MT, NT, nsub_n, slab, xcd_chunks);                                    \
    else                                                                                                            \
        hipLaunchKernelGGL(HIP_KERNEL_NAME(wgrad_kernel<MM, NN>), grid, dim3(SC_BLOCK), 0, s, in, n_in, cin, dout, cout, nbr, \
                       n_out, k_vol, rpc, MT, NT, nsub_n, slab, xcd_chunks)
#define WG_ROW(MM)             \
    switch (ntb) {             \
        case 1: WG(MM, 1); break; \
        case 2: WG(MM, 2); break; \
        case 4: WG(MM, 4); break; \
        default: WG(MM, 8); break; \
    }
    switch (mtb) {
        case 1: WG_ROW(1); break;
        case 2: WG_ROW(2); break;
        case 4: WG_ROW(4); break;
        default: WG_ROW(8); break;
    }
#undef WG_ROW
#undef WG
    hipLaunchKernelGGL(wgrad_reduce_kernel, dim3(cdiv(elems, SC_BLOCK)), dim3(SC_BLOCK), 0, s, slab, chunks, elems, dw);
    TODA_LAUNCH_CHECK();
    return TODA_OK;
}
```

toda_amd/csrc/spconv_split.cuh:

```cuda
#pragma once
#include "split_common.cuh"

namespace toda {

#ifndef WGS_ACCS
#define WGS_ACCS 2
#endif
#ifndef SP_STAMPS
#define SP_STAMPS 0
#endif
#if SP_STAMPS
#define SP_STAMP(i)                                                                               \
    do {                                                                                          \
        unsigned long long t_;                                                                    \
        __builtin_amdgcn_sched_barrier(0);                                                        \
        asm volatile("s_memtime %0\n\ts_waitcnt lgkmcnt(0)" : "=s"(t_)::"memory");                \
        __builtin_amdgcn_sched_barrier(0);                                                        \
        seg[i] += t_ - t_prev;                                                                    \
        t_prev = t_;                                                                              \
    } while (0)
#else
#define SP_STAMP(i)
#endif
#ifndef SP_ABLATE
#define SP_ABLATE 0
#endif
__device__ __forceinline__ void sp_split8(const f32x4& v0, const f32x4& v1, u32x4& h, u32x4& m, u32x4& l) {
#pragma unroll
    for (int p = 0; p < 4; ++p) {
        const float x0 = p < 2 ? v0[2 * p] : v1[2 * p - 4], x1 = p < 2 ? v0[2 * p + 1] : v1[2 * p - 3];
        h[p] = sp_pack_hi(x0, x1);
#if SP_ABLATE & 1
        m[p] = h[p] ^ 0x00010001u, l[p] = h[p] ^ 0x00020002u;
        continue;
#endif
        const float r0 = x0 - sp_trunc(x0), r1 = x1 - sp_trunc(x1);
        m[p] = sp_pack_hi(r0, r1);
        const float l0 = r0 - sp_trunc(r0), l1 = r1 - sp_trunc(r1);
        l[p] = sp_pack_hi(l0, l1);
    }
}
__device__ __forceinline__ unsigned short sp_plane_of(float v, int plane) {
    const float h = sp_trunc(v), r = v - h, m = sp_trunc(r), l = r - m;
    const float pick = plane == 0 ? h : (plane == 1 ? m : l);
    return (unsigned short)(__builtin_bit_cast(unsigned, pick) >> 16);
}

constexpr int SPLIT_PACK_MAX_SEG = 48;
struct SplitPackBatch {
    const float* w[SPLIT_PACK_MAX_SEG];
    u32x4* wps[SPLIT_PACK_MAX_SEG];
    int cout[SPLIT_PACK_MAX_SEG], K[SPLIT_PACK_MAX_SEG], cin[SPLIT_PACK_MAX_SEG];
    unsigned char transpose[SPLIT_PACK_MAX_SEG], flip[SPLIT_PACK_MAX_SEG], KC[SPLIT_PACK_MAX_SEG], NT[SPLIT_PACK_MAX_SEG];
};
__global__ void __launch_bounds__(SC_BLOCK)
split_pack_batch_kernel(const SplitPackBatch b) {
    const int sg = blockIdx.y;
    const int K = b.K[sg], KC = b.KC[sg], NT = b.NT[sg], cin = b.cin[sg], cout = b.cout[sg];
    const long long e = (long long)blockIdx.x * SC_BLOCK + threadIdx.x;
    if (e >= (long long)K * KC * NT * 192) return;
    const int lane = (int)(e & 63);
    long long t = e >> 6;
    const int plane = (int)(t % 3);
    t /= 3;
    const int n = (int)(t % NT);
    t /= NT;
    const int kc = (int)(t % KC);
    const int k = (int)(t / KC);
    const int c = lane & 15, g = lane >> 4;
    const int pch = NT * c + n;
    const int kk = b.flip[sg] ? K - 1 - k : k;
    const float* __restrict__ w = b.w[sg];
    unsigned short v[8];
#pragma unroll
    for (int j = 0; j < 8; ++j) {
        const int gch = 32 * kc + 16 * (j >> 2) + 4 * g + (j & 3);
        float x = 0.0f;
        if (!b.transpose[sg]) {
            if (gch < cin && pch < cout) x = w[((size_t)pch * K + kk) * cin + gch];
        } else {
            if (gch < cout && pch < cin) x = w[((size_t)gch * K + kk) * cin + pch];
        }
        v[j] = sp_plane_of(x, plane);
    }
    b.wps[sg][e] = u32x4{(unsigned)v[0] | ((unsigned)v[1] << 16), (unsigned)v[2] | ((unsigned)v[3] << 16), (unsigned)v[4] | ((unsigned)v[5] << 16),
                         (unsigned)v[6] | ((unsigned)v[7] << 16)};
}

template <int KC, int KCS, int NT, int RT, int BLK, int WAVES, bool IL = false>
__global__ void __launch_bounds__(BLK, WAVES)
gg_split_kernel(const float* __restrict__ in, int n_in, const u32x4* __restrict__ wps, const int* __restrict__ nbr, int n_out, int K, int cp,
                const float* __restrict__ bias, float* __restrict__ out, const int* __restrict__ order, double* __restrict__ stats,
                const unsigned char* __restrict__ cls_sorted, const GatherClasses classes) {
    static_assert(KC % KCS == 0, "whole stages per offset");
    constexpr int CG = 32 * KC;
    constexpr int SPO = KC / KCS;
    constexpr int UNITS = KCS * NT * 3;
    constexpr int SLICE = UNITS * 64;
    static_assert(2 * SLICE * 16 >= (BLK / 64) * 2 * 16 * NT * 4, "the statistics scratch aliases the weight buffers");
    __shared__ u32x4 wl[2 * SLICE];
    const int lane = threadIdx.x & 63, wv = threadIdx.x >> 6;
    const int blk = xcd_chunked_block(blockIdx.x, gridDim.x);
    const int wave = blk * (BLK / 64) + wv;
    const int r = lane & 15, g = lane >> 4;
    const int row0 = wave * (16 * RT);

    f32x4 acc[RT][NT];
#pragma unroll
    for (int n = 0; n < NT; ++n) {
        float b = 0.0f;
        if (bias && NT * r + n < cp) b = bias[NT * r + n];
#pragma unroll
        for (int rt = 0; rt < RT; ++rt) acc[rt][n] = f32x4{b, b, b, b};
    }
    const __amdgpu_buffer_rsrc_t in_rsrc = table_rsrc(in, (unsigned)n_in * (unsigned)CG * 4u);
    int rows[RT];
    bool live[RT];
#pragma unroll
    for (int rt = 0; rt < RT; ++rt) {
        live[rt] = row0 + rt * 16 + r < n_out;
        rows[rt] = live[rt] ? (order ? order[row0 + rt * 16 + r] : row0 + rt * 16 + r) : n_out - 1;
    }
    int KE = K;
    bool listed = false;
    unsigned long long kpack = 0;
    if (cls_sorted) {
        const int p = row0 + (lane & (16 * RT - 1));
        const int c = cls_sorted[p < n_out ? p : n_out - 1], c0 = __builtin_amdgcn_readfirstlane(c);
        const bool same = __all(c == c0 || p >= n_out);
        int* cw = reinterpret_cast<int*>(wl);
        if (lane == 0) cw[wv] = same ? c0 : -1;
        __syncthreads();
        int cb = cw[0];
#pragma unroll
        for (int w = 1; w < BLK / 64; ++w) cb = (cw[w] == cb) ? cb : -1;
        __syncthreads();
        if (cb >= 0 && classes.count[cb & 7] > 0 && classes.count[cb & 7] <= 8) {
            listed = true;
            KE = classes.count[cb & 7];
#pragma unroll
            for (int i = 0; i < 8; ++i) kpack |= (unsigned long long)classes.k[cb & 7][i] << (8 * i);
            kpack = ((unsigned long long)__builtin_amdgcn_readfirstlane((int)(kpack >> 32)) << 32) | (unsigned)__builtin_amdgcn_readfirstlane((int)kpack);
        }
    }
    auto kof = [&](int j) { return listed ? (int)((kpack >> (8 * j)) & 0xFF) : j; };
    auto load_ids = [&](int j, int (&dst)[RT]) {
        const int kk = kof(j < KE ? j : KE - 1);
#pragma unroll
        for (int rt = 0; rt < RT; ++rt) {
            dst[rt] = __builtin_nontemporal_load(nbr + (size_t)kk * n_out + rows[rt]);
        }
    };
    auto gather = [&](const int (&src)[RT], int part, bool valid, f32x4 (&raw)[RT][2 * KCS]) {
#pragma unroll
        for (int rt = 0; rt < RT; ++rt) {
            const bool ok = src[rt] >= 0 && valid;
            const unsigned base = (unsigned)src[rt] * (unsigned)(CG * 4) + (unsigned)(16 * g) + (unsigned)(128 * KCS) * (unsigned)part;
#pragma unroll
            for (int i = 0; i < 2 * KCS; ++i)
                raw[rt][i] = __builtin_bit_cast(f32x4, __builtin_amdgcn_raw_buffer_load_b128(in_rsrc, ok ? base + 64u * i : OOB, 0, 0));
        }
    };
    auto gather_rt = [&](const int (&src)[RT], int part, bool valid, f32x4 (&raw)[RT][2 * KCS], int rt) {
        const bool ok = src[rt] >= 0 && valid;
        const unsigned base = (unsigned)src[rt] * (unsigned)(CG * 4) + (unsigned)(16 * g) + (unsigned)(128 * KCS) * (unsigned)part;
#pragma unroll
        for (int i = 0; i < 2 * KCS; ++i)
            raw[rt][i] = __builtin_bit_cast(f32x4, __builtin_amdgcn_raw_buffer_load_b128(in_rsrc, ok ? base + 64u * i : OOB, 0, 0));
    };
    auto stage = [&](int st, int buf) {
        const int sc = st < KE * SPO ? st : KE * SPO - 1;
        const int ss = kof(sc / SPO) * SPO + sc % SPO;
#pragma unroll
        for (int t = 0; t < (UNITS + BLK / 64 - 1) / (BLK / 64); ++t) {
            const int u = t * (BLK / 64) + wv;
            if (UNITS % (BLK / 64) == 0 || u < UNITS)
                __builtin_amdgcn_global_load_lds(reinterpret_cast<const float*>(wps + (size_t)ss * SLICE + u * 64 + lane),
                                                 reinterpret_cast<float*>(&wl[buf * SLICE + u * 64]), 16, 0, 0);
        }
    };

    int idA[RT], idB[RT], idC[RT];
    f32x4 raw[RT][2 * KCS];
    load_ids(0, idA);
    load_ids(1, idB);
    stage(0, 0);
    gather(idA, 0, true, raw);
    __syncthreads();

#if SP_STAMPS
    unsigned long long seg[6] = {0, 0, 0, 0, 0, 0}, t_prev;
    asm volatile("s_memtime %0\n\ts_waitcnt lgkmcnt(0)" : "=s"(t_prev)::"memory");
#endif
    auto body = [&](int k, const int (&ids_cur)[RT], const int (&ids_nxt)[RT], int (&ids_new)[RT]) {
        SP_STAMP(5);
        bool any = false;
#pragma unroll
        for (int rt = 0; rt < RT; ++rt) any = any || __any(ids_cur[rt] >= 0);
#pragma unroll
        for (int part = 0; part < SPO; ++part) {
            const int cur = (k * SPO + part) & 1;
            u32x4 ah[RT][KCS], am[RT][KCS], al[RT][KCS];
            f32x4 (&rw)[RT][2 * KCS] = raw;
            if (any) {
#pragma unroll
                for (int rt = 0; rt < RT; ++rt)
#pragma unroll
                    for (int kc = 0; kc < KCS; ++kc) sp_split8(rw[rt][2 * kc], rw[rt][2 * kc + 1], ah[rt][kc], am[rt][kc], al[rt][kc]);
            }
            SP_STAMP(0);
            if constexpr (IL) {
                constexpr int ITER = KCS * NT, PIECES = RT + 2;
                auto piece = [&](int p) {
                    if (p == 0) {
#if !(SP_ABLATE & 4)
                        stage(k * SPO + part + 1, cur ^ 1);
#endif
                    } else if (p <= RT) {
                        if (part + 1 < SPO) gather_rt(ids_cur, part + 1, true, raw, p - 1);
                        else gather_rt(ids_nxt, 0, k + 1 < KE, raw, p - 1);
                    } else if (part == SPO - 1) load_ids(k + 2, ids_new);
                    asm volatile("" ::: "memory");
                };
                if (any) {
                    const u32x4* __restrict__ wb = wl + cur * SLICE + lane;
#pragma unroll
                    for (int st = 0; st < ITER; ++st) {
                        const int kc = st / NT, n = st % NT;
                        const bf16x8 bh = __builtin_bit_cast(bf16x8, wb[(st * 3 + 0) * 64]), bm = __builtin_bit_cast(bf16x8, wb[(st * 3 + 1) * 64]),
                                     bl = __builtin_bit_cast(bf16x8, wb[(st * 3 + 2) * 64]);
#pragma unroll
                        for (int p = 0; p < PIECES; ++p)
                            if (p * ITER / PIECES == st) piece(p);
#define SP_TERM(AA, BB)                                                                                                              \
    _Pragma("unroll") for (int rt = 0; rt < RT; ++rt)                                                                                \
        acc[rt][n] = __builtin_amdgcn_mfma_f32_16x16x32_bf16(__builtin_bit_cast(bf16x8, AA[rt][kc]), BB, acc[rt][n], 0, 0, 0)
                        SP_TERM(al, bh);
                        SP_TERM(ah, bl);
                        SP_TERM(am, bm);
                        SP_TERM(am, bh);
                        SP_TERM(ah, bm);
                        SP_TERM(ah, bh);
#undef SP_TERM
                    }
                } else {
#pragma unroll
                    for (int p = 0; p < PIECES; ++p) piece(p);
                }
            } else {
#if !(SP_ABLATE & 4)
            stage(k * SPO + part + 1, cur ^ 1);
#endif
            asm volatile("" ::: "memory");
#if SP_ABLATE & 8
            if (k < 0)
#endif
            if (part + 1 < SPO) gather(ids_cur, part + 1, true, raw);
            else gather(ids_nxt, 0, k + 1 < KE, raw);
            asm volatile("" ::: "memory");
#if !(SP_ABLATE & 16)
            if (part == SPO - 1) load_ids(k + 2, ids_new);
#endif
            asm volatile("" ::: "memory");
            SP_STAMP(1);
            if (any) {
                const u32x4* __restrict__ wb = wl + cur * SLICE + lane;
#pragma unroll
                for (int st = 0; st < KCS * NT; ++st) {
                    const int kc = st / NT, n = st % NT;
                    const bf16x8 bh = __builtin_bit_cast(bf16x8, wb[(st * 3 + 0) * 64]), bm = __builtin_bit_cast(bf16x8, wb[(st * 3 + 1) * 64]),
                                 bl = __builtin_bit_cast(bf16x8, wb[(st * 3 + 2) * 64]);
#if SP_ABLATE & 2
#define SP_TERM(AA, BB)                                                                                                              \
    _Pragma("unroll") for (int rt = 0; rt < RT; ++rt)                                                                                \
        acc[rt][n][0] += __builtin_bit_cast(float, AA[rt][kc][0] ^ __builtin_bit_cast(u32x4, BB)[0])
#else
#define SP_TERM(AA, BB)                                                                                                              \
    _Pragma("unroll") for (int rt = 0; rt < RT; ++rt)                                                                                \
        acc[rt][n] = __builtin_amdgcn_mfma_f32_16x16x32_bf16(__builtin_bit_cast(bf16x8, AA[rt][kc]), BB, acc[rt][n], 0, 0, 0)
#endif
                    SP_TERM(al, bh);
                    SP_TERM(ah, bl);
                    SP_TERM(am, bm);
                    SP_TERM(am, bh);
                    SP_TERM(ah, bm);
                    SP_TERM(ah, bh);
#undef SP_TERM
                }
            }
            }
            SP_STAMP(2);
#if SP_ABLATE & (4 | 8 | 16)
            asm volatile("s_waitcnt vmcnt(0)" ::: "memory");
#else
            if (part == SPO - 1) asm volatile("s_waitcnt vmcnt(%0)" ::"n"(RT * 2 * KCS + RT) : "memory");
            else asm volatile("s_waitcnt vmcnt(%0)" ::"n"(RT * 2 * KCS) : "memory");
#endif
            SP_STAMP(3);
            __builtin_amdgcn_s_barrier();
            SP_STAMP(4);
        }
    };
    for (int k = 0;;) {
        body(k, idA, idB, idC);
        if (++k >= KE) break;
        body(k, idB, idC, idA);
        if (++k >= KE) break;
        body(k, idC, idA, idB);
        if (++k >= KE) break;
    }
    asm volatile("s_waitcnt vmcnt(0)" ::: "memory");
    if (row0 >= n_out && !stats) return;

#if SP_STAMPS
    if (stats) {
        if (lane == 0)
            for (int i = 0; i < 6; ++i) reinterpret_cast<unsigned long long*>(stats)[(size_t)wave * 6 + i] = seg[i];
        stats = nullptr;
    }
#endif
    if (stats) {
        float (*st_sh)[2][16 * NT] = reinterpret_cast<float (*)[2][16 * NT]>(wl);
        float sm[NT], sq[NT];
#pragma unroll
        for (int n = 0; n < NT; ++n) {
            sm[n] = sq[n] = 0.0f;
#pragma unroll
            for (int rt = 0; rt < RT; ++rt)
#pragma unroll
                for (int reg = 0; reg < 4; ++reg)
                    if (row0 + rt * 16 + 4 * g + reg < n_out) {
                        const float v = acc[rt][n][reg];
                        sm[n] += v;
                        sq[n] += v * v;
                    }
            sm[n] += __shfl_xor(sm[n], 16, 64);
            sq[n] += __shfl_xor(sq[n], 16, 64);
            sm[n] += __shfl_xor(sm[n], 32, 64);
            sq[n] += __shfl_xor(sq[n], 32, 64);
            if (g == 0) {
                st_sh[wv][0][NT * r + n] = sm[n];
                st_sh[wv][1][NT * r + n] = sq[n];
            }
        }
        __syncthreads();
        if ((int)threadIdx.x < 2 * cp) {
            const int qq = threadIdx.x / cp, ch = threadIdx.x - qq * cp;
            double a = 0.0;
#pragma unroll
            for (int w = 0; w < BLK / 64; ++w) a += (double)st_sh[w][qq][ch];
            stats[2 * cp + (size_t)(qq * cp + ch) * gridDim.x + blk] = a;
        }
    }

    const bool full = cp == 16 * NT;
#pragma unroll
    for (int rt = 0; rt < RT; ++rt) {
#pragma unroll
        for (int reg = 0; reg < 4; ++reg) {
            const int pos = row0 + rt * 16 + 4 * g + reg;
            const int row = __shfl(rows[rt], 4 * g + reg, 64);
            if (pos >= n_out) continue;
            float* dst = out + (size_t)row * cp + NT * r;
            if (full) {
                if constexpr (NT == 2) {
                    *reinterpret_cast<float2*>(dst) = make_float2(acc[rt][0][reg], acc[rt][1][reg]);
                } else {
#pragma unroll
                    for (int n = 0; n < NT; n += 4)
                        *reinterpret_cast<f32x4*>(dst + n) = f32x4{acc[rt][n][reg], acc[rt][n + 1][reg], acc[rt][n + 2][reg], acc[rt][n + 3][reg]};
                }
            } else {
#pragma unroll
                for (int n = 0; n < NT; ++n)
                    if (NT * r + n < cp) dst[n] = acc[rt][n][reg];
            }
        }
    }
}

template <int MTB, int NTB, int QM = 1, int QN = 1>
__global__ void __launch_bounds__(SC_BLOCK, (MTB * NTB <= 4) ? 4 : ((MTB == 4 && NTB == 2) ? 3 : 2))
wgrad_split_kernel(const float* __restrict__ in, int n_in, const float* __restrict__ dout, const int* __restrict__ nbr, int n_out, int K,
                   int rows_per_chunk, float* __restrict__ slab, int xcd_chunks) {
    static_assert((MTB == 2 || MTB == 4) && (NTB == 2 || NTB == 4), "32 or 64 channels a side");
    static_assert(QM * QN == 1 || (MTB == 4 && NTB == 4), "quarters are 64 x 64");
    static_assert(QM * QN == 1 || QM * QN == 2 || QM * QN == 4, "1, 2 or 4 quarters");
    constexpr int NQ = QM * QN, TEAMS = (SC_BLOCK / 64) / NQ;
    constexpr int MT = MTB * QM, NT = NTB * QN;
    constexpr int cin = 16 * MT, cout = 16 * NT;
    constexpr int QCAP = 64 + 32;
    __shared__ float red[TEAMS == 1 ? 1 : NQ * MTB * NTB * 4 * 64];
    __shared__ int q_in[SC_BLOCK / 64][QCAP], q_out[SC_BLOCK / 64][QCAP];
    const int lane = threadIdx.x & 63, wv = threadIdx.x >> 6;
    const int ii = lane & 15, g = lane >> 4;
    const int n_chunks = xcd_chunks < 0 ? -xcd_chunks : xcd_chunks;
    int chunk, k;
    {
        const int b = blockIdx.x;
        if (xcd_chunks > 0) {
            const int xcd = b & 7, t = (b >> 3) / K;
            k = (b >> 3) - t * K;
            chunk = t * 8 + xcd;
        } else {
            chunk = b % n_chunks;
            k = b / n_chunks;
        }
    }
    const int row_begin = chunk * rows_per_chunk;
    if (row_begin >= n_out) return;
    const int row_end = min(n_out, row_begin + rows_per_chunk);
    int* qi = q_in[wv];
    int* qo = q_out[wv];

    f32x4 acc[MTB][NTB];
#if WGS_ACCS >= 2
    f32x4 acc_s[MTB][NTB];
#endif
#if WGS_ACCS >= 3
    f32x4 acc_m[MTB][NTB];
#endif
#pragma unroll
    for (int m = 0; m < MTB; ++m)
#pragma unroll
        for (int n = 0; n < NTB; ++n) {
            acc[m][n] = f32x4{0.f, 0.f, 0.f, 0.f};
#if WGS_ACCS >= 2
            acc_s[m][n] = f32x4{0.f, 0.f, 0.f, 0.f};
#endif
#if WGS_ACCS >= 3
            acc_m[m][n] = f32x4{0.f, 0.f, 0.f, 0.f};
#endif
        }
    const __amdgpu_buffer_rsrc_t in_rsrc = table_rsrc(in, (unsigned)n_in * (unsigned)cin * 4u);
    const __amdgpu_buffer_rsrc_t dout_rsrc = table_rsrc(dout, (unsigned)n_out * (unsigned)cout * 4u);
    const int qd = wv % NQ, team = wv / NQ;
    const int m0 = (qd / QN) * MTB, n0 = (qd % QN) * NTB;
    const unsigned lane_a = (unsigned)(MT * ii + m0) * 4u, lane_b = (unsigned)(NT * ii + n0) * 4u;
    constexpr unsigned row_a = (unsigned)cin * 4u, row_b = (unsigned)cout * 4u;

    auto round32 = [&](int d, int limit, auto full_tag) {
        constexpr bool FULL = decltype(full_tag)::value;
        float a[8][MTB], b[8][NTB];
#pragma unroll
        for (int j = 0; j < 8; ++j) {
            const int p = d + 8 * g + j;
            const bool ok = FULL || p < limit;
            const int pc = ok ? p : d;
            const unsigned ia = (unsigned)qi[pc] + lane_a, ib = (unsigned)qo[pc] + lane_b;
            if constexpr (MTB == 4) {
                const f32x4 v = __builtin_bit_cast(f32x4, __builtin_amdgcn_raw_buffer_load_b128(in_rsrc, ok ? ia : OOB, 0, 0));
#pragma unroll
                for (int m = 0; m < 4; ++m) a[j][m] = v[m];
            } else {
                const f32x2w v = __builtin_bit_cast(f32x2w, __builtin_amdgcn_raw_buffer_load_b64(in_rsrc, ok ? ia : OOB, 0, 0));
                a[j][0] = v[0], a[j][1] = v[1];
            }
            if constexpr (NTB == 4) {
                const f32x4 v = __builtin_bit_cast(f32x4, __builtin_amdgcn_raw_buffer_load_b128(dout_rsrc, ok ? ib : OOB, 0, 0));
#pragma unroll
                for (int n = 0; n < 4; ++n) b[j][n] = v[n];
            } else {
                const f32x2w v = __builtin_bit_cast(f32x2w, __builtin_amdgcn_raw_buffer_load_b64(dout_rsrc, ok ? ib : OOB, 0, 0));
                b[j][0] = v[0], b[j][1] = v[1];
            }
        }
        u32x4 ah[MTB], am[MTB], al[MTB];
#pragma unroll
        for (int m = 0; m < MTB; ++m)
#pragma unroll
            for (int q = 0; q < 4; ++q) {
                unsigned h_, m_, l_;
                sp_split2(a[2 * q][m], a[2 * q + 1][m], h_, m_, l_);
                ah[m][q] = h_, am[m][q] = m_, al[m][q] = l_;
            }
#pragma unroll
        for (int n = 0; n < NTB; ++n) {
            u32x4 bh, bm, bl;
#pragma unroll
            for (int q = 0; q < 4; ++q) {
                unsigned h_, m_, l_;
                sp_split2(b[2 * q][n], b[2 * q + 1][n], h_, m_, l_);
                bh[q] = h_, bm[q] = m_, bl[q] = l_;
            }
#define WS_TERM(ACC, AA, BB)                                                                                             \
    _Pragma("unroll") for (int m = 0; m < MTB; ++m)                                                                       \
        ACC[m][n] = __builtin_amdgcn_mfma_f32_16x16x32_bf16(__builtin_bit_cast(bf16x8, AA[m]), __builtin_bit_cast(bf16x8, BB), ACC[m][n], 0, 0, 0)
#if WGS_ACCS == 1
            WS_TERM(acc, al, bh);
            WS_TERM(acc, ah, bl);
            WS_TERM(acc, am, bm);
            WS_TERM(acc, am, bh);
            WS_TERM(acc, ah, bm);
            WS_TERM(acc, ah, bh);
#elif WGS_ACCS == 2
            WS_TERM(acc_s, al, bh);
            WS_TERM(acc_s, ah, bl);
            WS_TERM(acc_s, am, bm);
            WS_TERM(acc, am, bh);
            WS_TERM(acc, ah, bm);
            WS_TERM(acc, ah, bh);
#else
            WS_TERM(acc_s, al, bh);
            WS_TERM(acc_s, ah, bl);
            WS_TERM(acc_s, am, bm);
            WS_TERM(acc_m, am, bh);
            WS_TERM(acc_m, ah, bm);
            WS_TERM(acc, ah, bh);
#endif
#undef WS_TERM
        }
    };

    int qn = 0;
    constexpr int BSTEP = TEAMS * 64;
    const int base0 = row_begin + team * 64;
    int iv_next = nbr[(size_t)k * n_out + min(base0 + lane, n_out - 1)];
    for (int base = base0; base < row_end; base += BSTEP) {
        const int o = base + lane;
        const int iv = iv_next;
        iv_next = nbr[(size_t)k * n_out + min(o + BSTEP, n_out - 1)];
        const int i = o < row_end ? iv : -1;
        const unsigned long long vote = __ballot(i >= 0);
        if (vote == 0) continue;
        if (i >= 0) {
            const int pos = qn + __popcll(vote & ((1ull << lane) - 1));
            qi[pos] = (int)((unsigned)i * row_a);
            qo[pos] = (int)((unsigned)o * row_b);
        }
        qn += __popcll(vote);
        __builtin_amdgcn_wave_barrier();
        int done = 0;
        while (qn - done >= 32) {
            round32(done, qn, std::true_type{});
            done += 32;
        }
        const int left = qn - done;
        if (done > 0 && left > 0) {
            int ti = 0, to = 0;
            if (lane < left) {
                ti = qi[done + lane];
                to = qo[done + lane];
            }
            __builtin_amdgcn_wave_barrier();
            if (lane < left) {
                qi[lane] = ti;
                qo[lane] = to;
            }
        }
        qn = left;
        __builtin_amdgcn_wave_barrier();
    }
    if (qn > 0) round32(0, qn, std::false_type{});
#if WGS_ACCS >= 2
#pragma unroll
    for (int m = 0; m < MTB; ++m)
#pragma unroll
        for (int n = 0; n < NTB; ++n) {
#if WGS_ACCS >= 3
            acc[m][n] = (acc_s[m][n] + acc_m[m][n]) + acc[m][n];
#else
            acc[m][n] = acc_s[m][n] + acc[m][n];
#endif
        }
#endif

    for (int src = 1; src < TEAMS; ++src) {
        float* const rq = red + qd * (MTB * NTB * 4 * 64);
        if (team == src) {
#pragma unroll
            for (int m = 0; m < MTB; ++m)
#pragma unroll
                for (int n = 0; n < NTB; ++n)
#pragma unroll
                    for (int reg = 0; reg < 4; ++reg) rq[((m * NTB + n) * 4 + reg) * 64 + lane] = acc[m][n][reg];
        }
        __syncthreads();
        if (team == 0) {
#pragma unroll
            for (int m = 0; m < MTB; ++m)
#pragma unroll
                for (int n = 0; n < NTB; ++n)
#pragma unroll
                    for (int reg = 0; reg < 4; ++reg) acc[m][n][reg] += rq[((m * NTB + n) * 4 + reg) * 64 + lane];
        }
        __syncthreads();
    }
    if (team != 0) return;
    float* dst = slab + (size_t)chunk * cout * K * cin;
#pragma unroll
    for (int m = 0; m < MTB; ++m)
#pragma unroll
        for (int n = 0; n < NTB; ++n)
#pragma unroll
            for (int reg = 0; reg < 4; ++reg) {
                const int ci = MT * (4 * g + reg) + m0 + m;
                const int co = NT * ii + n0 + n;
                dst[((size_t)co * K + k) * cin + ci] = acc[m][n][reg];
            }
}

static inline bool wgrad_split_shape_ok(int cin, int cout) {
    return ((cin == 32 || cin == 64) && (cout == 32 || cout == 64)) || ((cin == 64 || cin == 128) && (cout == 64 || cout == 128));
}

static inline bool split_shape_ok(int c_gather, int c_produce) {
    return (c_gather == 32 || c_gather == 64 || c_gather == 128) && (c_produce == 32 || c_produce == 64 || c_produce == 128);
}
static inline size_t split_packed_bytes(int k_vol, int c_gather, int c_produce) {
    return (size_t)k_vol * (c_gather / 32) * (c_produce / 16) * 3 * 1024;
}

}
```

toda_amd/lib.py:

```python
import ctypes as C
import os

import torch

_HERE = os.path.dirname(os.path.abspath(__file__))
LIB_PATH = os.environ.get("TODA_HIP_LIB") or os.path.join(_HERE, "libtoda_hip.so")

_vp, _i, _sz, _dbl = C.c_void_p, C.c_int, C.c_size_t, C.c_double

SIGNATURES = {
    "toda_last_error": (C.c_char_p, []),
    "toda_abi_version": (_i, []),
    "toda_device_fault": (_i, []),
    "toda_voxelize_workspace_bytes": (_sz, [_i, _i]),
    "toda_voxelize_hard": (_i, [_vp, _i, _i, _vp, _vp, _vp, _i, _i, _vp, _vp, _vp, _vp, _vp, _sz, _vp]),
    "toda_mean_vfe_fwd": (_i, [_vp, _vp, _i, _i, _i, _vp, _vp]),
    "toda_mean_vfe_bwd": (_i, [_vp, _vp, _i, _i, _i, _vp, _vp]),
    "toda_dynvox_workspace_bytes": (_sz, [_i, _i, _vp, _i]),
    "toda_dynvox_count": (_i, [_vp, _i, _i, _i, _vp, _vp, _vp, _i, _vp, _vp, _sz, _vp]),
    "toda_dynvox_index": (_i, [_vp, _i, _i, _i, _vp, _vp, _vp, _i, _i, _i, _vp, _vp, _vp, _vp, _vp, _vp, _vp, _vp, _sz, _vp]),
    "toda_dynvox_seg_sum": (_i, [_vp, _i, _i, _i, _vp, _vp, _vp, _i, _i, _vp, _vp]),
    "toda_dynvox_pillar_decorate": (_i, [_vp, _i, _vp, _vp, _vp, _vp, _i, _vp, _vp, _i, _i, _vp, _i, _vp]),
    "toda_dynvox_seg_max_fwd": (_i, [_vp, _i, _vp, _vp, _i, _vp, _vp, _vp]),
    "toda_dynvox_seg_max_bwd": (_i, [_vp, _vp, _i, _i, _i, _vp, _vp]),
    "toda_dynvox_gather_concat": (_i, [_vp, _vp, _vp, _i, _i, _vp, _vp]),
    "toda_gridindex_bytes": (_sz, [_i, _vp]),
    "toda_gridindex_from_coords": (_i, [_vp, _i, _vp, _i, _vp, _vp, _vp, _vp]),
    "toda_gridindex_from_conv": (_i, [_vp, _i, _vp, _i, _vp, _vp, _vp, _vp, _vp, _vp, _vp, _vp, _i, _vp]),
    "toda_rulebook_subm": (_i, [_vp, _i, _i, _vp, _vp, _vp, _vp, _vp, _vp, _vp, _i, _vp]),
    "toda_rulebook_conv": (_i, [_vp, _i, _i, _vp, _vp, _vp, _vp, _vp, _vp, _i, _vp, _vp, _vp, _vp, _vp, _vp, _i, _vp]),
    "toda_voxelize_batch_workspace_bytes": (_sz, [_i, _i]),
    "toda_voxelize_batch": (_i, [_vp, _vp, _i, _i, _i, _i, _vp, _vp, _vp, _i, _i, _vp, _vp, _vp, _vp, _vp, _sz, _i, _vp]),
    "toda_gridindex_from_coords_unordered": (_i, [_vp, _i, _vp, _i, _vp, _vp, _vp, _i, _vp]),
    "toda_gridindex_clear": (_i, [_vp, _i, _vp, _i, _vp, _vp, _vp]),
    "toda_gridindex_from_bitmap": (_i, [_vp, _i, _vp, _vp, _vp, _vp, _vp, _vp, _vp, _vp, _i, _i, _vp]),
    "toda_spconv_packed_weight_floats": (_sz, [_i, _i, _i]),
    "toda_matrix_path": (_i, []),
    "toda_set_matrix_path": (_i, [_i]),
    "toda_spconv_split_supported": (_i, [_i, _i]),
    "toda_spconv_pack_weight": (_i, [_vp, _i, _i, _i, _i, _i, _vp, _vp]),
    "toda_spconv_pack_weights": (_i, [_i, _vp, _vp, _vp, _vp, _vp, _vp, _vp, _vp]),
    "toda_spconv_gather_gemm": (_i, [_vp, _i, _i, _vp, _vp, _i, _i, _i, _vp, _vp, _vp]),
    "toda_spconv_gather_gemm_ordered": (_i, [_vp, _i, _i, _vp, _vp, _i, _i, _i, _vp, _vp, _vp, _vp]),
    "toda_rulebook_class_order": (_i, [_vp, _i, _vp, _vp, _vp, _vp, _vp]),
    "toda_spconv_gather_gemm_classed": (_i, [_vp, _i, _i, _vp, _vp, _i, _i, _i, _vp, _vp, _vp, _vp, _vp, _vp, _vp, _vp]),
    "toda_spconv_gather_gemm_stats_supported": (_i, [_i, _i]),
    "toda_spconv_gather_gemm_stats_doubles": (_sz, [_i, _i]),
    "toda_spconv_gather_gemm_stats": (_i, [_vp, _i, _i, _vp, _vp, _i, _i, _i, _vp, _vp, _vp, _sz, _vp]),
    "toda_spconv_gather_gemm_stats_partials": (_i, [_vp, _i, _i, _vp, _vp, _i, _i, _i, _vp, _vp, _vp, _sz, _vp, _vp]),
    "toda_spconv_gather_gemm_compact_supported": (_i, [_i, _i, _i]),
    "toda_spconv_gather_gemm_compact": (_i, [_vp, _i, _i, _vp, _i, _i, _i, _i, _vp, _i, _i, _i, _vp, _vp, _vp]),
    "toda_spconv_gather_gemm_compact_stats_doubles": (_sz, [_i, _i]),
    "toda_spconv_gather_gemm_compact_stats": (_i, [_vp, _i, _i, _vp, _i, _i, _i, _i, _vp, _i, _i, _i, _vp, _vp, _vp, _sz, _vp, _vp]),
    "toda_spconv_wgrad_workspace_bytes": (_sz, [_i, _i, _i, _i]),
    "toda_spconv_wgrad": (_i, [_vp, _i, _vp, _vp, _i, _i, _i, _i, _vp, _vp, _sz, _vp]),
    "toda_sparse_to_dense_fwd": (_i, [_vp, _vp, _i, _i, _i, _vp, _vp, _vp]),
    "toda_sparse_to_dense_bwd": (_i, [_vp, _vp, _i, _i, _i, _vp, _vp, _vp]),
    "toda_pillar_scatter_fwd": (_i, [_vp, _vp, _i, _i, _i, _i, _i, _vp, _vp]),
    "toda_pillar_scatter_bwd": (_i, [_vp, _vp, _i, _i, _i, _i, _i, _vp, _vp]),
    "toda_rows_reduce_doubles": (_sz, [_i, _i]),
    "toda_rows_moments": (_i, [_vp, _i, _i, _vp, _vp]),
    "toda_rows_affine_act": (_i, [_vp, _vp, _vp, _vp, _i, _i, _i, _vp, _vp]),
    "toda_bn_finalize": (_i, [_vp, _i, _i, _vp, _vp, _vp, _vp, C.c_float, C.c_float, _i, _vp, _vp, _vp, _vp, _vp]),
    "toda_bn_finalize_partials": (_i, [_vp, _i, _i, _i, _vp, _vp, _vp, _vp, C.c_float, C.c_float, _vp, _vp, _vp, _vp, _vp]),
    "toda_rows_bn_bwd": (_i, [_vp, _vp, _vp, _vp, _i, _i, _i, _vp, _vp, _vp]),
    "toda_rows_bn_bwd_res": (_i, [_vp, _vp, _vp, _vp, _vp, _i, _i, _i, _vp, _vp, _vp, _vp]),
    "toda_rows_bn_bwd_colsum_doubles": (_sz, [_i, _i]),
    "toda_rows_bn_bwd_res_colsum": (_i, [_vp, _vp, _vp, _vp, _vp, _i, _i, _i, _vp, _vp, _vp, _vp, _vp, _vp]),
    "toda_conv3x3s2_supported": (_i, [_i, _i, _i, _i, _i]),
    "toda_conv3x3s2_fwd": (_i, [_vp, _vp, _i, _i, _i, _i, _i, _vp, _vp]),
    "toda_conv3x3s2_dgrad": (_i, [_vp, _vp, _i, _i, _i, _i, _i, _vp, _vp]),
    "toda_conv3x3s2_wgrad_workspace_bytes": (_sz, [_i, _i, _i, _i, _i]),
    "toda_conv3x3s2_wgrad": (_i, [_vp, _vp, _i, _i, _i, _i, _i, _vp, _vp, _sz, _vp]),
    "toda_deconv_supported": (_i, [_i, _i, _i, _i, _i, _i]),
    "toda_deconv_fwd": (_i, [_vp, _vp, _i, _i, _i, _i, _i, _i, _vp, _vp]),
    "toda_deconv_dgrad": (_i, [_vp, _vp, _i, _i, _i, _i, _i, _i, _vp, _vp]),
    "toda_deconv_wgrad_workspace_bytes": (_sz, [_i, _i, _i, _i, _i, _i]),
    "toda_deconv_wgrad": (_i, [_vp, _vp, _i, _i, _i, _i, _i, _i, _vp, _vp, _sz, _vp]),
    "toda_bn2d_supported": (_i, [_i, _i, _i]),
    "toda_bn2d_sync_bytes": (_sz, []),
    "toda_bn2d_fwd": (_i, [_vp, _i, _i, _i, _vp, _vp, _vp, _vp, C.c_float, C.c_float, _i, _vp, _vp, _vp, C.c_uint, _vp]),
    "toda_bn2d_bwd": (_i, [_vp, _vp, _i, _i, _i, _vp, _vp, _vp, _i, _vp, _vp, _vp, _vp, C.c_uint, _vp]),
    "toda_bn2d_fwd_into": (_i, [_vp, _i, _i, _i, _vp, _vp, _vp, _vp, C.c_float, C.c_float, _i, _vp, _i, _i, _vp, _vp, C.c_uint, _vp]),
    "toda_bn2d_bwd_from": (_i, [_vp, _vp, _i, _i, _i, _i, _i, _vp, _vp, _vp, _i, _vp, _vp, _vp, _vp, C.c_uint, _vp]),
    "toda_boxes_iou_bev": (_i, [_vp, _i, _vp, _i, _vp, _vp]),
    "toda_boxes_overlap_bev": (_i, [_vp, _i, _vp, _i, _vp, _vp]),
    "toda_nms_workspace_bytes": (_sz, [_i]),
    "toda_nms_rotated": (_i, [_vp, _i, C.c_float, _vp, _vp, _vp, _sz, _vp]),
    "toda_roi_grid_pool_bev": (_i, [_vp, _i, _i, _i, _i, _vp, _i, _i, C.c_float, C.c_float, C.c_float, C.c_float, _i, _vp, _vp]),
    "toda_roi_iou3d_max": (_i, [_vp, _i, _i, _i, _vp, _vp, _i, _i, _i, _vp, _vp, _vp]),
    "toda_voxel_query": (_i, [_vp, _vp, _i, _vp, _i, _vp, _vp, _i, _vp, C.c_float, _vp, _i, _vp, _vp, _vp]),
    "toda_voxel_pool_moments_doubles": (_sz, []),
    "toda_voxel_pool_moments": (_i, [_vp, _vp, _i, _i, _vp, _i, _vp, _vp, _vp]),
    "toda_voxel_pool_fwd": (_i, [_vp, _i, _i, _vp, _vp, _i, _i, _vp, _vp, _vp, _vp, _vp, _vp]),
    "toda_voxel_pool_table_bytes": (_sz, [_i, _i, _i]),
    "toda_voxel_pool_table": (_i, [_vp, _vp, _i, _i, _i, _vp, _vp, _vp, _sz, _vp]),
    "toda_voxel_pool_bwd_feat": (_i, [_vp, _vp, _i, _i, _i, _vp, _vp, _i, _vp, _vp]),
    "toda_voxel_pool_bwd_pos_doubles": (_sz, [_i]),
    "toda_voxel_pool_bwd_pos": (_i, [_vp, _vp, _vp, _vp, _i, _i, _i, _vp, _i, _vp, _vp, _vp, _vp]),
    "toda_fps_resident_blocks": (_i, []),
    "toda_fps_workspace_bytes": (_sz, [_i, _i]),
    "toda_fps": (_i, [_vp, _vp, _i, _i, _i, _vp, _vp, _vp, _sz, _vp]),
    "toda_ball_query_stack": (_i, [_vp, _i, _vp, _vp, _vp, _i, _i, _i, _vp, _vp, _vp, _vp, _vp]),
    "toda_sa_gather_fwd": (_i, [_vp, _i, _i, _vp, _vp, _vp, _i, _i, _vp, _vp, _vp, _vp]),
    "toda_sa_gather_bwd_feat": (_i, [_vp, _i, _i, _i, _vp, _vp, _i, _vp, _vp]),
    "toda_sa_gather_bwd_pos_doubles": (_sz, [_i]),
    "toda_sa_gather_bwd_pos": (_i, [_vp, _vp, _vp, _i, _i, _i, _vp, _i, _vp, _vp, _vp, _vp]),
    "toda_sa_max_fwd": (_i, [_vp, _i, _i, _i, _vp, _vp, _vp]),
    "toda_sa_max_bwd": (_i, [_vp, _vp, _i, _i, _i, _vp, _vp]),
    "toda_bev_interp_fwd": (_i, [_vp, _i, _i, _i, _i, _vp, _vp, _i, _vp, _vp, _vp, _vp]),
    "toda_bev_interp_bwd": (_i, [_vp, _i, _i, _vp, _vp, _vp, _i, _i, _i, _vp, _vp]),
    "toda_clip_adam_chunk": (_i, []),
    "toda_clip_adam_step": (_i, [_vp, _vp, _vp, _vp, _vp, _vp, _vp, _i, _vp, _vp, C.c_float, C.c_float, C.c_float, C.c_float, C.c_float, C.c_float, _i, _vp]),
    "toda_points_in_boxes": (_i, [_vp, _i, _vp, _i, _vp, _i, _i, _i, _vp, _vp]),
    "toda_points_sector": (_i, [_vp, _i, _vp, _i, _dbl, _dbl, _vp, _vp]),
    "toda_points_rect": (_i, [_vp, _i, _vp, _i, _vp, _vp, _i, _vp, _vp]),
    "toda_points_polar_cell": (_i, [_vp, _i, _vp, _i, C.c_float, _vp, _i, _vp, _i, C.c_float, C.c_float, _vp, _vp]),
    "toda_points_polar_select": (_i, [_vp, _i, _vp, _i, _dbl, _dbl, _i, _i, _dbl, _vp, _vp, _vp]),
    "toda_points_pitch_range_workspace_bytes": (_sz, []),
    "toda_points_pitch_range": (_i, [_vp, _i, _vp, _i, _vp, _vp, _sz, _vp]),
    "toda_points_pitch_band": (_i, [_vp, _i, _vp, _i, C.c_float, C.c_float, C.c_float, _vp, _i, _vp, _vp]),
    "toda_rows_select_workspace_bytes": (_sz, [_i]),
    "toda_rows_select_append": (_i, [_vp, _i, _vp, _i, _vp, _i, _i, _vp, _i, _vp, _vp, _sz, _vp]),
    "toda_points_rotate_z": (_i, [_vp, _i, _vp, _i, _dbl, _dbl, _vp, _vp]),
    "toda_points_world_transform": (_i, [_vp, _i, _vp, _i, _i, _i, _i, C.c_float, C.c_float, _i, C.c_float, _vp, _vp]),
    "toda_conv3x3_supported": (_i, [_i, _i, _i, _i, _i]),
    "toda_conv3x3_weight_floats": (_sz, [_i, _i]),
    "toda_conv3x3_transform_weight": (_i, [_vp, _i, _i, _i, _vp, _vp]),
    "toda_conv3x3_workspace_bytes": (_sz, []),
    "toda_conv3x3_wgrad_workspace_bytes": (_sz, [_i, _i, _i, _i, _i]),
    "toda_conv3x3_wgrad": (_i, [_vp, _vp, _i, _i, _i, _i, _i, _vp, _vp, _sz, _vp]),
    "toda_conv3x3_fwd": (_i, [_vp, _vp, _vp, _i, _i, _i, _i, _i, _vp, _vp, _sz, _vp]),
    "toda_conv3x3_narrow_supported": (_i, [_i, _i, _i, _i, _i]),
    "toda_conv3x3_narrow_fwd": (_i, [_i, _vp, _vp, _vp, _vp, _i, _i, _i, _i, C.c_longlong, _vp, _vp]),
    "toda_conv3x3_narrow_dgrad": (_i, [_i, _vp, _vp, _vp, _i, _i, _i, _i, C.c_longlong, _vp, _vp]),
    "toda_conv3x3_narrow_wgrad_workspace_bytes": (_sz, [_i, _i, _i, _i]),
    "toda_conv3x3_narrow_wgrad": (_i, [_i, _vp, _vp, _vp, _i, _i, _i, _i, C.c_longlong, _vp, _vp, _sz, _vp]),
    "toda_center_loss_workspace_bytes": (_sz, [_i, _i, _i, _i, _i, _i]),
    "toda_center_loss_fwd": (_i, [_vp, _vp, _i, _i, _i, _i, _i, _vp, _vp, _vp, _vp, _vp, _i, _i, _vp, C.c_float, C.c_float, _vp, _vp, _vp, _sz, _vp]),
    "toda_center_loss_bwd": (_i, [_vp, _vp, _vp, _i, _i, _i, _i, _i, _vp, _vp, _vp, _vp, _i, _i, _vp, C.c_float, C.c_float, _vp, _vp, _sz, _vp]),
    "toda_timing_begin": (_i, [_i]),
    "toda_timing_end": (_i, [_vp, _i, _vp]),
    "toda_center_assign": (_i, [_vp, _i, _i, _i, _i, _i, _i, _vp, _vp, _i, _i, _dbl, _i, _vp, _vp, _vp, _vp, _vp]),
}

_lib = None


def load():
    global _lib
    if _lib is not None:
        return _lib
    if not os.path.exists(LIB_PATH):
        raise RuntimeError(
            f"{LIB_PATH} not found: build it with `python -c 'import __graft_entry__ as g; g.build()'` "
            "(hipcc --offload-arch=gfx950).  toda_amd has no CPU fallback."
        )
    try:
        lib = C.CDLL(LIB_PATH)
    except OSError as e:
        raise RuntimeError(f"cannot load {LIB_PATH}: {e}") from e
    for name, (res, args) in SIGNATURES.items():
        try:
            fn = getattr(lib, name)
        except AttributeError as e:
            raise RuntimeError(f"{LIB_PATH} does not export {name}") from e
        fn.restype = res
        fn.argtypes = args
    _lib = lib
    return lib


def last_error():
    return load().toda_last_error().decode()


def check(rc, what):
    if rc != 0:
        raise RuntimeError(f"{what} failed (code {rc}): {last_error()}")


def ptr(t):
    if t is None:
        return None
    if not t.is_cuda:
        raise RuntimeError("toda_amd ops need tensors on the GPU (there is no CPU path)")
    if not t.is_contiguous():
        raise RuntimeError("toda_amd ops need contiguous tensors")
    return t.data_ptr()


_raw_stream = getattr(torch._C, "_cuda_getCurrentRawStream", None)
_raw_device = getattr(torch._C, "_cuda_getDevice", None)


def stream():
    if _raw_stream is not None and _raw_device is not None:
        return _raw_stream(_raw_device())
    return torch.cuda.current_stream().cuda_stream


def host_ptrs(tensors):
    return (C.c_void_p * len(tensors))(*[ptr(t) for t in tensors])


def host_addrs(addrs):
    return (C.c_void_p * len(addrs))(*[int(a) for a in addrs])


def host_i32(vals):
    arr = (C.c_int32 * len(vals))(*[int(v) for v in vals])
    return arr


def host_f32(vals):
    arr = (C.c_float * len(vals))(*[float(v) for v in vals])
    return arr


def host_f64(vals):
    arr = (C.c_double * len(vals))(*[float(v) for v in vals])
    return arr


def hptr(arr):
    return C.cast(arr, C.c_void_p)
```

toda_amd/ops.py:

```python
import numpy as np
import torch

from . import arena as _arena
from . import lib as L


def _triple(v):
    if isinstance(v, (list, tuple)):
        assert len(v) == 3
        return [int(x) for x in v]
    return [int(v)] * 3


def grid_size_xyz(pc_range, voxel_size):
    r = np.asarray(pc_range, dtype=np.float64)
    return np.round((r[3:6] - r[0:3]) / np.asarray(voxel_size, dtype=np.float64)).astype(np.int64)


import os as _os
import os as _os_early
import time as _time

_COUNT_PINNED = {}
_LAST_WAIT_S = 0.0
# ... 322 lines not shown
            lib, buf, bt, shp = L.load(), self.buf, self.batch, self._shape_c

            def clear():
                L.check(lib.toda_gridindex_clear(L.ptr(indices), n, L.ptr(n_dev), bt, L.hptr(shp), L.ptr(buf), L.stream()), "toda_gridindex_clear")

            slot.marks[self._name] = clear
        return self

    @classmethod
    def from_coords_unordered(cls, indices, batch, shape, n_dev=None, name="gi0"):
        return cls.unordered_begin(batch, shape, indices.device, name).unordered_build(indices, n_dev)


class Rulebook:

    def __init__(self, kind, ksize, n_in, n_out, nbr_fwd, nbr_bwd, flip_bwd, pair_cnt, **geom):
        self.kind = kind
        self.ksize = ksize
        self.k_vol = int(ksize[0] * ksize[1] * ksize[2])
        self.n_in, self.n_out = n_in, n_out
        self.nbr_fwd = nbr_fwd
        self.nbr_bwd = nbr_bwd
        self.flip_bwd = flip_bwd
        self.pair_cnt = pair_cnt
        nbr_fwd._toda_pair_cnt = pair_cnt
        if nbr_bwd is not nbr_fwd:
            nbr_bwd._toda_pair_cnt = pair_cnt
        self.geom = geom
        self.in_indices = None
        self._inverse = None
        self._class_order = None

    def class_order(self):
        if (not CLASS_DGRAD or self.kind != "conv" or self.in_indices is None or self.k_vol > 27 or self.k_vol < 2
                or self.n_in < CLASS_DGRAD_MIN_ROWS or any(int(v) not in (1, 2) for v in self.geom["stride"])):
            return None
        if self._class_order is None:
            lib = L.load()
            dev = self.in_indices.device
            order = _alloc((self.n_in,), torch.int32, dev)
            cls = _alloc((self.n_in,), torch.uint8, dev)
            st, pd = L.host_i32(self.geom["stride"]), L.host_i32(self.geom["padding"])
            L.check(lib.toda_rulebook_class_order(L.ptr(self.in_indices), self.n_in, L.hptr(st), L.hptr(pd), L.ptr(order), L.ptr(cls), L.stream()),
                    "toda_rulebook_class_order")
            self._class_order = (order, cls)
        return self._class_order

    def num_pairs(self):
        return int(self.pair_cnt.sum().item())

    def inverse(self):
        if self.kind != "conv":
            raise ValueError("only the tables of a strided SparseConv3d have an inverse")
        if self._inverse is None:
            inv = Rulebook("inverse", self.ksize, self.n_out, self.n_in, self.nbr_bwd, self.nbr_fwd, False, self.pair_cnt, **self.geom)
            self._inverse = inv
        return self._inverse


def conv_out_shape(shape, ksize, stride, padding):
    return [(int(s) + 2 * p - k) // t + 1 for s, k, t, p in zip(shape, ksize, stride, padding)]


def build_subm_rulebook(indices, batch, shape, ksize=3, dilation=1, grid_index=None, pair_cnt=None):
    lib = L.load()
    ks, dl = _triple(ksize), _triple(dilation)
    indices = indices.contiguous()
    assert indices.dtype == torch.int32 and indices.shape[1] == 4
    n = indices.shape[0]
    if grid_index is None:
        grid_index = GridIndex.from_coords_unordered(indices, batch, shape, name=("gi_lazy", tuple(int(v) for v in shape)))
    K = ks[0] * ks[1] * ks[2]
    nbr = _alloc((K, n), torch.int32, indices.device)
    zeroed = pair_cnt is not None
    cnt = pair_cnt if zeroed else torch.empty((K,), dtype=torch.int32, device=indices.device)
    ks_c, dl_c = L.host_i32(ks), L.host_i32(dl)
    rc = lib.toda_rulebook_subm(L.ptr(indices), n, int(batch), L.hptr(grid_index._shape_c), L.hptr(ks_c), L.hptr(dl_c),
                                L.ptr(grid_index.buf), L.ptr(grid_index.rowof), L.ptr(nbr), L.ptr(cnt), int(zeroed), L.stream())
    L.check(rc, "toda_rulebook_subm")
    return Rulebook("subm", ks, n, n, nbr, nbr, True, cnt, dilation=dl), grid_index


def _conv_tables(indices, n_in, idx_out, n_out, batch, shape, out_shape, ks, st, pd, gi_out, gi_in=None, pair_cnt=None):
    lib = L.load()
    dev = indices.device
    K = ks[0] * ks[1] * ks[2]
    o2i = _alloc((K, n_out), torch.int32, dev)
    i2o = _alloc((K, n_in), torch.int32, dev)
    zeroed = pair_cnt is not None
    cnt = pair_cnt if zeroed else torch.empty((K,), dtype=torch.int32, device=dev)
    hs = [L.host_i32(v) for v in (shape, ks, st, pd, out_shape)]
    rc = lib.toda_rulebook_conv(L.ptr(indices), n_in, int(batch), L.hptr(hs[0]), L.hptr(hs[1]), L.hptr(hs[2]), L.hptr(hs[3]),
                                L.hptr(hs[4]), L.ptr(gi_out.buf), n_out, L.ptr(o2i), L.ptr(i2o), L.ptr(cnt),
                                L.ptr(idx_out) if gi_in is not None else None, L.ptr(gi_in.buf) if gi_in is not None else None,
                                L.ptr(gi_in.rowof) if gi_in is not None else None, int(zeroed), L.stream())
    L.check(rc, "toda_rulebook_conv")
    rb = Rulebook("conv", ks, n_in, n_out, o2i, i2o, False, cnt, stride=st, padding=pd, in_shape=[int(v) for v in shape])
    rb.in_indices = indices
    return rb


def _conv_cap(n_upper, batch, out_shape, ks, st):
    per_in = 1
    for k, s_ in zip(ks, st):
        per_in *= -(-k // s_)
    return int(min(n_upper * per_in, batch * out_shape[0] * out_shape[1] * out_shape[2]))


def build_conv_rulebook(indices, batch, shape, ksize, stride, padding):
    lib = L.load()
    ks, st, pd = _triple(ksize), _triple(stride), _triple(padding)
    indices = indices.contiguous()
    assert indices.dtype == torch.int32 and indices.shape[1] == 4
    n_in = indices.shape[0]
    shape = [int(s) for s in shape]
    out_shape = conv_out_shape(shape, ks, st, pd)
    dev = indices.device
    gi_out = GridIndex(batch, out_shape, dev)
    cap = _conv_cap(n_in, batch, out_shape, ks, st)
    idx_out = torch.empty((max(cap, 1), 4), dtype=torch.int32, device=dev)
    n_out_dev = torch.zeros((1,), dtype=torch.int32, device=dev)
    shi, sho = L.host_i32(shape), L.host_i32(out_shape)
    ks_c, st_c, pd_c = L.host_i32(ks), L.host_i32(st), L.host_i32(pd)
    rc = lib.toda_gridindex_from_conv(L.ptr(indices), n_in, None, int(batch), L.hptr(shi), L.hptr(ks_c), L.hptr(st_c),
                                      L.hptr(pd_c), L.hptr(sho), L.ptr(gi_out.buf), L.ptr(idx_out), L.ptr(n_out_dev),
                                      cap, L.stream())
    L.check(rc, "toda_gridindex_from_conv")
    n_out = int(n_out_dev.item())
    if n_out > cap:
        raise RuntimeError(f"strided rulebook: {n_out} outputs exceed the bound {cap}")
    idx_out = idx_out[:n_out]
    rb = _conv_tables(indices, n_in, idx_out, n_out, batch, shape, out_shape, ks, st, pd, gi_out)
    return idx_out, out_shape, rb, gi_out


def _plan_enqueue(level0, batch, shape, steps, counts, c0, gi0=None):
    lib = L.load()
    idx0, n_upper, n_dev = level0
    dev = idx0.device
    slot = _arena.current_slot()
    tag = slot.plans if slot is not None else 0
    if gi0 is None:
        gi0 = GridIndex.unordered_begin(batch, shape, dev, name=("gi0", tag))
    gi0.unordered_build(idx0, n_dev)
    levels = [{"idx": idx0, "n_upper": n_upper, "shape": [int(v) for v in shape], "gi": gi0}]
    li = 0
    for st in steps:
        if st["kind"] != "conv":
            continue
        cur = levels[-1]
        ks, sd, pd = _triple(st["ksize"]), _triple(st["stride"]), _triple(st["padding"])
        out_shape = conv_out_shape(cur["shape"], ks, sd, pd)
        cap = _conv_cap(cur["n_upper"], batch, out_shape, ks, sd)
        li += 1
        shape_c = L.host_i32(out_shape)
        buf, _ = _persistent(("gi", tag, li), (int(batch), tuple(out_shape)), lib.toda_gridindex_bytes(int(batch), L.hptr(shape_c)), dev)
        gi_out = GridIndex(batch, out_shape, dev, buf=buf)
        idx_out = _alloc((max(cap, 1), 4), torch.int32, dev)
        hs = [L.host_i32(v) for v in (cur["shape"], ks, sd, pd, out_shape)]
        rc = lib.toda_gridindex_from_bitmap(L.ptr(cur["gi"].buf), int(batch), L.hptr(hs[0]), L.hptr(hs[1]), L.hptr(hs[2]), L.hptr(hs[3]),
                                            L.hptr(hs[4]), L.ptr(gi_out.buf), L.ptr(idx_out), counts.data_ptr() + 4 * (c0 + li - 1),
                                            cap, 1 if li == 1 else 0, L.stream())
        L.check(rc, "toda_gridindex_from_bitmap")
        levels.append({"idx": idx_out, "n_upper": cap, "shape": out_shape, "gi": gi_out, "cap": cap, "step": st})
    if slot is not None:
        slot.plans += 1
    return levels


def _plan_tables(levels, level_counts, batch, steps, training):
    dev = levels[0]["idx"].device
    for lv, n in zip(levels, level_counts):
        if lv.get("cap") is not None and n > lv["cap"]:
            raise RuntimeError(f"strided rulebook {lv['step']['key']}: {n} outputs exceed the bound {lv['cap']}")
        lv["n"] = int(n)
        lv["idx"] = lv["idx"][:int(n)]
    keys = []
    for st in steps:
        if st["key"] not in keys:
            keys.append(st["key"])
    cnts = torch.zeros((len(keys), 64), dtype=torch.int32, device=dev)
    out = {}
    li = 0
    for st in steps:
        cur = levels[li]
        if st["kind"] == "subm":
            if st["key"] in out:
                continue
            ks = _triple(st["ksize"])
            rb, gi = build_subm_rulebook(cur["idx"], batch, cur["shape"], st["ksize"], st.get("dilation", 1), grid_index=cur["gi"],
                                         pair_cnt=cnts[keys.index(st["key"])][:ks[0] * ks[1] * ks[2]])
            out[st["key"]] = {"kind": "subm", "rb": rb, "n_in": cur["n"]}
        else:
            nxt = levels[li + 1]
            ks, sd, pd = _triple(st["ksize"]), _triple(st["stride"]), _triple(st["padding"])
            rb = _conv_tables(cur["idx"], cur["n"], nxt["idx"], nxt["n"], batch, cur["shape"], nxt["shape"], ks, sd, pd, nxt["gi"],
                              gi_in=cur["gi"], pair_cnt=cnts[keys.index(st["key"])][:ks[0] * ks[1] * ks[2]])
            if training:
                rb.class_order()
            out[st["key"]] = {"kind": "conv", "rb": rb, "n_in": cur["n"], "out_indices": nxt["idx"],
                              "out_shape": nxt["shape"], "gi": nxt["gi"]}
            li += 1
    return out


def build_index_plan(indices, batch, shape, steps, while_waiting=None, training=None):
    indices = indices.contiguous()
    n_conv = sum(1 for st in steps if st["kind"] == "conv")
    counts = _alloc((max(n_conv, 1),), torch.int32, indices.device)
    levels = _plan_enqueue((indices, indices.shape[0], None), batch, shape, steps, counts, 0)
    got = read_counts(counts, while_waiting) if n_conv else []
    if training is None:
        training = torch.is_grad_enabled()
    return _plan_tables(levels, [indices.shape[0]] + list(got[:n_conv]), batch, steps, training)


def build_input_plan(clouds, voxel_cfg, batch, shape, steps, training=True, while_waiting=None):
    n_conv = sum(1 for st in steps if st["kind"] == "conv")
    bsz = len(clouds)
    dev = clouds[0][0].device
    slot = _arena.current_slot()
    gi0 = GridIndex.unordered_begin(batch, shape, dev, name=("gi0", slot.plans if slot is not None else 0))
    counts = _alloc((bsz + 1 + n_conv,), torch.int32, dev)
    voxels, coords, num, _ = voxelize_enqueue(clouds, voxel_cfg["point_cloud_range"], voxel_cfg["voxel_size"],
                                              voxel_cfg["max_points_per_voxel"], voxel_cfg["max_num_voxels"], counts=counts,
                                              tag=slot.plans if slot is not None else 0)
    levels = _plan_enqueue((coords, coords.shape[0], counts[bsz:bsz + 1]), batch, shape, steps, counts, bsz + 1, gi0=gi0)
    got = read_counts(counts, while_waiting)
    m = got[bsz]
    plan = _plan_tables(levels, [m] + list(got[bsz + 1:bsz + 1 + n_conv]), batch, steps, training)
    return voxels[:m], levels[0]["idx"], num[:m], plan


MATRIX_PATHS = ("native", "split")
_MM = None


def matrix_path():
    global _MM
    if _MM is None:
        _MM = MATRIX_PATHS[L.load().toda_matrix_path()]
    return _MM


def set_matrix_path(name):
    global _MM
    L.check(L.load().toda_set_matrix_path(MATRIX_PATHS.index(name)), "toda_set_matrix_path")
    _MM = name


def _tag_mm(wp, cg, cp):
    wp._toda_mm = matrix_path() if L.load().toda_spconv_split_supported(int(cg), int(cp)) else None
    return wp


def _check_mm(wp):
    mm = getattr(wp, "_toda_mm", None)
    if mm is not None and mm != matrix_path():
        raise RuntimeError(f"packed sparse-conv operand was written under matrix path {mm!r}, the current path is {matrix_path()!r}: re-pack it")


def pack_weight(weight, transpose, flip_k):
    lib = L.load()
    cout, cin = weight.shape[0], weight.shape[-1]
    K = weight.numel() // (cout * cin)
    cg, cp = (cout, cin) if transpose else (cin, cout)
    n = lib.toda_spconv_packed_weight_floats(K, cg, cp)
    wp = torch.empty((n,), dtype=torch.float32, device=weight.device)
    rc = lib.toda_spconv_pack_weight(L.ptr(weight.contiguous()), cout, K, cin, int(transpose), int(flip_k), L.ptr(wp),
                                     L.stream())
    L.check(rc, "toda_spconv_pack_weight")
    return _tag_mm(wp, cg, cp)


def pack_weights_batched(items):
    lib = L.load()
    if not items:
        return []
    dev = items[0][0].device
    sizes, couts, ks, cins, pairs = [], [], [], [], []
    for w, tr, _ in items:
        cout, cin = w.shape[0], w.shape[-1]
        K = w.numel() // (cout * cin)
        cg, cp = (cout, cin) if tr else (cin, cout)
        sizes.append(lib.toda_spconv_packed_weight_floats(K, cg, cp))
        couts.append(cout), ks.append(K), cins.append(cin), pairs.append((cg, cp))
    flat = torch.empty((sum(sizes),), dtype=torch.float32, device=dev)
    outs, off = [], 0
    for n, (cg, cp) in zip(sizes, pairs):
        outs.append(_tag_mm(flat[off:off + n], cg, cp))
        off += n
    ws = [w.contiguous() for w, _, _ in items]
    rc = lib.toda_spconv_pack_weights(len(items), L.host_ptrs(ws), L.hptr(L.host_i32(couts)), L.hptr(L.host_i32(ks)), L.hptr(L.host_i32(cins)),
                                      L.hptr(L.host_i32([int(bool(t)) for _, t, _ in items])), L.hptr(L.host_i32([int(bool(f)) for _, _, f in items])),
                                      L.host_ptrs(outs), L.stream())
    L.check(rc, "toda_spconv_pack_weights")
    return outs


def gather_gemm_stats_supported(c_gather, c_produce):
    return bool(L.load().toda_spconv_gather_gemm_stats_supported(int(c_gather), int(c_produce)))


def gather_gemm_with_stats(feat, wp, nbr, c_produce, bias=None, partials=False):
    lib = L.load()
    K, n_out = nbr.shape
    out = torch.empty((n_out, c_produce), dtype=torch.float32, device=feat.device)
    nd = lib.toda_spconv_gather_gemm_stats_doubles(n_out, c_produce)
    sums = torch.empty((nd,), dtype=torch.float64, device=feat.device)
    if partials:
        import ctypes
        blocks = ctypes.c_int(0)
        rc = lib.toda_spconv_gather_gemm_stats_partials(L.ptr(feat), feat.shape[0], feat.shape[1], L.ptr(wp), L.ptr(nbr), n_out, K, c_produce,
                                                        L.ptr(bias), L.ptr(out), L.ptr(sums), nd, ctypes.addressof(blocks), L.stream())
        L.check(rc, "toda_spconv_gather_gemm_stats_partials")
        return out, sums, int(blocks.value)
    rc = lib.toda_spconv_gather_gemm_stats(L.ptr(feat), feat.shape[0], feat.shape[1], L.ptr(wp), L.ptr(nbr), n_out, K, c_produce,
                                           L.ptr(bias), L.ptr(out), L.ptr(sums), nd, L.stream())
    L.check(rc, "toda_spconv_gather_gemm_stats")
    return out, sums


def gather_gemm(feat, wp, nbr, c_produce, bias=None, order=None):
    lib = L.load()
    K, n_out = nbr.shape
    out = torch.empty((n_out, c_produce), dtype=torch.float32, device=feat.device)
    rc = lib.toda_spconv_gather_gemm_ordered(L.ptr(feat), feat.shape[0], feat.shape[1], L.ptr(wp), L.ptr(nbr), n_out, K,
                                             c_produce, L.ptr(bias), L.ptr(out), L.ptr(order), L.stream())
    L.check(rc, "toda_spconv_gather_gemm_ordered")
    return out


def _refuse_retired_knobs():
    retired = [k for k in ("TODA_GG_LINE", "TODA_HALO", "TODA_WG_TILE", "TODA_ROW_ORDER", "TODA_GG_WS", "TODA_GG_STAGE", "TODA_GG_WRES", "TODA_GG_LDS_PF",
                           "TODA_GG_BLK512", "TODA_GG_RT", "TODA_SPLIT_BLK", "TODA_SPLIT_KCS", "TODA_WINO_WGRAD") if _os.environ.get(k, "0") not in ("0", "")]
    if retired:
        raise RuntimeError(f"{', '.join(retired)}: these kernel variants were retired (profiles/EXPERIMENTS.md); unset the variable(s)")
    ablate = [k for k in ("TODA_GG_ABLATE", "TODA_WINO_ABLATE", "TODA_WINO_WG_ABLATE") if _os.environ.get(k, "0") not in ("0", "")]
    if ablate and not _os.environ.get("TODA_HIP_LIB"):
        raise RuntimeError(f"{', '.join(ablate)} only act in a measurement build (-DTODA_ABLATE=1, loaded through TODA_HIP_LIB): the library "
                           "that ships ignores them, and a run that believes it ablated something would report wrong conclusions")


_refuse_retired_knobs()


COMPACT = _os.environ.get("TODA_GG_COMPACT", "1") == "1"


def _compact_route(c_gather, c_produce, nbr):
    return (COMPACT and nbr.shape[0] == 27 and nbr.shape[1] > 0 and c_produce in (16, 32) and c_gather <= 32
            and (c_gather <= 16 or c_produce == 16))


def gather_gemm_compact_supported(c_gather, c_produce, k_vol):
    return bool(L.load().toda_spconv_gather_gemm_compact_supported(int(c_gather), int(c_produce), int(k_vol)))


def gather_gemm_compact(feat, weight, nbr, c_produce, bias=None, transpose=False, flip_k=False, stats=False):
    lib = L.load()
    K, n_out = nbr.shape
    out = torch.empty((n_out, c_produce), dtype=torch.float32, device=feat.device)
    if stats:
        import ctypes
        nd = lib.toda_spconv_gather_gemm_compact_stats_doubles(n_out, c_produce)
        sums = torch.empty((nd,), dtype=torch.float64, device=feat.device)
        blocks = ctypes.c_int(0)
        rc = lib.toda_spconv_gather_gemm_compact_stats(L.ptr(feat), feat.shape[0], feat.shape[1], L.ptr(weight), weight.shape[0], weight.shape[-1],
                                                       int(bool(transpose)), int(bool(flip_k)), L.ptr(nbr), n_out, K, c_produce, L.ptr(bias), L.ptr(out),
                                                       L.ptr(sums), nd, ctypes.addressof(blocks), L.stream())
        L.check(rc, "toda_spconv_gather_gemm_compact_stats")
        return out, sums, int(blocks.value)
    rc = lib.toda_spconv_gather_gemm_compact(L.ptr(feat), feat.shape[0], feat.shape[1], L.ptr(weight), weight.shape[0], weight.shape[-1],
                                             int(bool(transpose)), int(bool(flip_k)), L.ptr(nbr), n_out, K, c_produce, L.ptr(bias), L.ptr(out), L.stream())
    L.check(rc, "toda_spconv_gather_gemm_compact")
    return out


def gather_gemm_classed(feat, wp, nbr, c_produce, order, cls_sorted, ksize, stride, padding):
    lib = L.load()
    K, n_out = nbr.shape
    out = torch.empty((n_out, c_produce), dtype=torch.float32, device=feat.device)
    ks, st, pd = L.host_i32(ksize), L.host_i32(stride), L.host_i32(padding)
    rc = lib.toda_spconv_gather_gemm_classed(L.ptr(feat), feat.shape[0], feat.shape[1], L.ptr(wp), L.ptr(nbr), n_out, K, c_produce, None,
                                             L.ptr(out), L.ptr(order), L.ptr(cls_sorted), L.hptr(ks), L.hptr(st), L.hptr(pd), L.stream())
    L.check(rc, "toda_spconv_gather_gemm_classed")
    return out


def wgrad(feat, dout, nbr, wshape):
    lib = L.load()
    K, n_out = nbr.shape
    cout, cin = wshape[0], wshape[-1]
    dw = torch.empty(wshape, dtype=torch.float32, device=feat.device)
    ws_bytes = lib.toda_spconv_wgrad_workspace_bytes(n_out, K, cin, cout)
    ws = torch.empty((max(ws_bytes, 16),), dtype=torch.uint8, device=feat.device)
    rc = lib.toda_spconv_wgrad(L.ptr(feat), feat.shape[0], L.ptr(dout), L.ptr(nbr), n_out, K, cin, cout, L.ptr(dw),
                               L.ptr(ws), ws_bytes, L.stream())
    L.check(rc, "toda_spconv_wgrad")
    return dw


CLASS_DGRAD = _os.environ.get("TODA_CLASS_DGRAD", "1") == "1"
CLASS_DGRAD_MIN_ROWS = int(_os.environ.get("TODA_CLASS_DGRAD_MIN_ROWS", "4096"))
WGRAD_ON_SIDE_STREAM = _os.environ.get("TODA_WGRAD_STREAM", "0") == "1"
_SIDE_STREAMS = {}


def _side_stream(device):
    key = (device.type, device.index)
    if key not in _SIDE_STREAMS:
        _SIDE_STREAMS[key] = torch.cuda.Stream(device=device)
    return _SIDE_STREAMS[key]


class _SparseConv(torch.autograd.Function):

    @staticmethod
    def forward(ctx, features, weight, bias, rb, wp_fwd, want_stats=False, wp_bwd=None):
        features = features.contiguous()
        compact = _compact_route(features.shape[1], weight.shape[0], rb.nbr_fwd)
        if wp_fwd is None and not compact:
            wp_fwd = pack_weight(weight, False, False)
        if wp_fwd is not None:
            _check_mm(wp_fwd)
        sums, blocks = None, 0
        if compact and want_stats:
            out, sums, blocks = gather_gemm_compact(features, weight.contiguous(), rb.nbr_fwd, weight.shape[0], bias, stats=True)
        elif want_stats and FOLD_IN_FINALIZE:
            out, sums, blocks = gather_gemm_with_stats(features, wp_fwd, rb.nbr_fwd, weight.shape[0], bias, partials=True)
        elif want_stats:
            out, sums = gather_gemm_with_stats(features, wp_fwd, rb.nbr_fwd, weight.shape[0], bias)
        elif compact:
            out = gather_gemm_compact(features, weight.contiguous(), rb.nbr_fwd, weight.shape[0], bias)
        else:
            out = gather_gemm(features, wp_fwd, rb.nbr_fwd, weight.shape[0], bias)
        ctx.set_materialize_grads(False)
        ctx.save_for_backward(features, weight)
        ctx.rb = rb
        ctx.wp_bwd = wp_bwd
        ctx.has_bias = bias is not None
        if want_stats:
            ctx.mark_non_differentiable(sums)
            return out, sums, blocks
        return out

    @staticmethod
    def backward(ctx, gout, *unused):
        features, weight = ctx.saved_tensors
        rb = ctx.rb
        if gout is None:
            return None, None, None, None, None, None, None
        gout = gout.contiguous()
        gfeat = gw = gb = None
        need_d, need_w = ctx.needs_input_grad[0], ctx.needs_input_grad[1]
        side = _side_stream(gout.device) if (need_d and need_w and WGRAD_ON_SIDE_STREAM) else None
        if side is not None:
            main = torch.cuda.current_stream(gout.device)
            side.wait_stream(main)
            with torch.cuda.stream(side):
                gw = wgrad(features, gout, rb.nbr_fwd, tuple(weight.shape))
            for t in (features, gout, rb.nbr_fwd):
                t.record_stream(side)
            need_w = False
        if need_d and _compact_route(gout.shape[1], weight.shape[-1], rb.nbr_bwd):
            gfeat = gather_gemm_compact(gout, weight.contiguous(), rb.nbr_bwd, weight.shape[-1], None, True, rb.flip_bwd)
        elif need_d:
            wp_t = ctx.wp_bwd if ctx.wp_bwd is not None else pack_weight(weight, True, rb.flip_bwd)
            _check_mm(wp_t)
            co = rb.class_order()
            if co is not None:
                gfeat = gather_gemm_classed(gout, wp_t, rb.nbr_bwd, weight.shape[-1], co[0], co[1], rb.ksize, rb.geom["stride"], rb.geom["padding"])
            else:
                gfeat = gather_gemm(gout, wp_t, rb.nbr_bwd, weight.shape[-1], None)
        if need_w:
            gw = wgrad(features, gout, rb.nbr_fwd, tuple(weight.shape))
        if ctx.has_bias and ctx.needs_input_grad[2]:
            gb = _take_colsum(gout)
            if gb is None:
                gb = gout.sum(0)
        if side is not None:
            torch.cuda.current_stream(gout.device).wait_stream(side)
            gw.record_stream(torch.cuda.current_stream(gout.device))
        return gfeat, gw, gb, None, None, None, None


FUSE_BN_STATS = _os.environ.get("TODA_FUSE_BN_STATS", "1") == "1"
FOLD_IN_FINALIZE = _os.environ.get("TODA_BN_FOLD_FINALIZE", "1") == "1"


def sparse_conv(features, weight, bias, rulebook, packed_weight=None, want_stats=False, packed_dgrad=None):
    if not want_stats:
        return _SparseConv.apply(features, weight, bias, rulebook, packed_weight, False, packed_dgrad)
    narrow = FOLD_IN_FINALIZE and _compact_route(features.shape[1], weight.shape[0], rulebook.nbr_fwd)
    ok = (FUSE_BN_STATS and (narrow or gather_gemm_stats_supported(weight.shape[-1], weight.shape[0])) and rulebook.nbr_fwd.shape[1] > 1
          and features.shape[0] > 0)
    if not ok:
        return _SparseConv.apply(features, weight, bias, rulebook, packed_weight, False, packed_dgrad), None
    out, sums, blocks = _SparseConv.apply(features, weight, bias, rulebook, packed_weight, True, packed_dgrad)
    return out, ((sums, blocks) if blocks else sums)


class _ToDense(torch.autograd.Function):
    @staticmethod
    def forward(ctx, features, indices, batch, shape):
        lib = L.load()
        n, c = features.shape
        shape = [int(s) for s in shape]
        dense = torch.empty((batch, c, *shape), dtype=torch.float32, device=features.device)
        sh = L.host_i32(shape)
        rc = lib.toda_sparse_to_dense_fwd(L.ptr(features.contiguous()), L.ptr(indices), n, c, batch, L.hptr(sh),
                                          L.ptr(dense), L.stream())
        L.check(rc, "toda_sparse_to_dense_fwd")
        ctx.save_for_backward(indices)
        ctx.meta = (n, c, batch, shape)
        return dense

    @staticmethod
    def backward(ctx, gdense):
        (indices,) = ctx.saved_tensors
        n, c, batch, shape = ctx.meta
        g = torch.empty((n, c), dtype=torch.float32, device=gdense.device)
        sh = L.host_i32(shape)
        rc = L.load().toda_sparse_to_dense_bwd(L.ptr(gdense.contiguous()), L.ptr(indices), n, c, batch, L.hptr(sh),
                                               L.ptr(g), L.stream())
        L.check(rc, "toda_sparse_to_dense_bwd")
        return g, None, None, None


def sparse_to_dense(features, indices, batch, shape):
    return _ToDense.apply(features, indices.contiguous(), int(batch), shape)


class _PillarScatter(torch.autograd.Function):
    @staticmethod
    def forward(ctx, features, indices, batch, ny, nx):
        n, c = features.shape
        canvas = torch.empty((batch, c, ny, nx), dtype=torch.float32, device=features.device)
        rc = L.load().toda_pillar_scatter_fwd(L.ptr(features.contiguous()), L.ptr(indices), n, c, batch, ny, nx,
                                              L.ptr(canvas), L.stream())
        L.check(rc, "toda_pillar_scatter_fwd")
        ctx.save_for_backward(indices)
        ctx.meta = (n, c, batch, ny, nx)
        return canvas

    @staticmethod
    def backward(ctx, gcanvas):
        (indices,) = ctx.saved_tensors
        n, c, batch, ny, nx = ctx.meta
        g = torch.empty((n, c), dtype=torch.float32, device=gcanvas.device)
        rc = L.load().toda_pillar_scatter_bwd(L.ptr(gcanvas.contiguous()), L.ptr(indices), n, c, batch, ny, nx, L.ptr(g),
                                              L.stream())
        L.check(rc, "toda_pillar_scatter_bwd")
        return g, None, None, None, None


def pillar_scatter(features, indices, batch, ny, nx):
    return _PillarScatter.apply(features, indices.contiguous(), int(batch), int(ny), int(nx))


def rows_moments(x):
    n, c = x.shape
    lib = L.load()
    sums = torch.empty((lib.toda_rows_reduce_doubles(n, c),), dtype=torch.float64, device=x.device)
    L.check(lib.toda_rows_moments(L.ptr(x.contiguous()), n, c, L.ptr(sums), L.stream()), "toda_rows_moments")
    return sums[:2 * c]


def rows_affine_act(x, scale, shift, residual=None, relu=True):
    n, c = x.shape
    y = torch.empty_like(x)
    rc = L.load().toda_rows_affine_act(L.ptr(x.contiguous()), L.ptr(scale.contiguous()), L.ptr(shift.contiguous()),
                                       L.ptr(residual), n, c, int(bool(relu)), L.ptr(y), L.stream())
    L.check(rc, "toda_rows_affine_act")
    return y


_DX_COLSUM = {}
BN_BWD_COLSUM = _os.environ.get("TODA_BN_BWD_COLSUM", "1") == "1"


def _take_colsum(gout):
    ent = _DX_COLSUM.pop(gout.data_ptr(), None) if _DX_COLSUM else None
    if ent is None or ent[0].shape != gout.shape or ent[0]._version != ent[2] or gout.stride() != ent[0].stride():
        return None
    return ent[1]


class _BNRows(torch.autograd.Function):

    @staticmethod
    def forward(ctx, x, weight, bias, running_mean, running_var, training, momentum, eps, relu, residual=None, sums=None, colsum=False):
        lib = L.load()
        if _DX_COLSUM:
            _DX_COLSUM.clear()
        ctx.colsum = bool(colsum) and BN_BWD_COLSUM
        x = x.contiguous()
        residual = residual.contiguous() if residual is not None else None
        n, c = x.shape
        dev = x.device
        stats = torch.empty((4, c), dtype=torch.float32, device=dev)
        if isinstance(sums, tuple) and training:
            part, blocks = sums
            rc = lib.toda_bn_finalize_partials(L.ptr(part), int(blocks), n, c, L.ptr(weight), L.ptr(bias), L.ptr(running_mean), L.ptr(running_var),
                                               float(momentum), float(eps), L.ptr(stats[0]), L.ptr(stats[1]), L.ptr(stats[2]), L.ptr(stats[3]), L.stream())
            L.check(rc, "toda_bn_finalize_partials")
            sums = part
        else:
            if isinstance(sums, tuple):
                sums = None
            sums = _BNRows._finalize(lib, x, n, c, dev, sums, training, weight, bias, running_mean, running_var, momentum, eps, stats)
        y = torch.empty_like(x)
        rc = lib.toda_rows_affine_act(L.ptr(x), L.ptr(stats[2]), L.ptr(stats[3]), L.ptr(residual), n, c, int(bool(relu)), L.ptr(y),
                                      L.stream())
        L.check(rc, "toda_rows_affine_act")
        ctx.save_for_backward(x, stats, weight, residual)
        ctx.meta = (n, c, bool(relu), bool(training))
        return y

    @staticmethod
    def _finalize(lib, x, n, c, dev, sums, training, weight, bias, running_mean, running_var, momentum, eps, stats):
        if sums is None or not training:
            sums = torch.empty((lib.toda_rows_reduce_doubles(n, c),), dtype=torch.float64, device=dev)
            if training:
                L.check(lib.toda_rows_moments(L.ptr(x), n, c, L.ptr(sums), L.stream()), "toda_rows_moments")
        rc = lib.toda_bn_finalize(L.ptr(sums), n, c, L.ptr(weight), L.ptr(bias), L.ptr(running_mean), L.ptr(running_var),
                                  float(momentum), float(eps), int(bool(training)), L.ptr(stats[0]), L.ptr(stats[1]),
                                  L.ptr(stats[2]), L.ptr(stats[3]), L.stream())
        L.check(rc, "toda_bn_finalize")
        return sums

    @staticmethod
    def backward(ctx, gy):
        x, stats, weight, residual = ctx.saved_tensors
        n, c, relu, training = ctx.meta
        gy = gy.contiguous()
        want_res = residual is not None and ctx.needs_input_grad[9]
        if not training:
            pre = x * stats[2] + stats[3]
            if residual is not None:
                pre = pre + residual
            dz = gy * (pre > 0) if relu else gy
            gx = dz * stats[2]
            xhat = (x - stats[0]) * stats[1]
            return gx, (dz * xhat).sum(0), dz.sum(0), None, None, None, None, None, None, (dz if want_res else None), None, None
        sums = torch.empty((L.load().toda_rows_reduce_doubles(n, c),), dtype=torch.float64, device=x.device)
        gx = torch.empty_like(x)
        gamma = weight if weight is not None else torch.ones(c, device=x.device)
        gres = torch.empty_like(x) if want_res else None
        if ctx.colsum:
            lib = L.load()
            cs_ws = torch.empty((lib.toda_rows_bn_bwd_colsum_doubles(n, c),), dtype=torch.float64, device=x.device)
            cs = torch.empty((c,), dtype=torch.float32, device=x.device)
            rc = lib.toda_rows_bn_bwd_res_colsum(L.ptr(gy), L.ptr(x), L.ptr(residual), L.ptr(stats), L.ptr(gamma), n, c, int(relu),
                                                 L.ptr(sums), L.ptr(gx), L.ptr(gres), L.ptr(cs_ws), L.ptr(cs), L.stream())
            L.check(rc, "toda_rows_bn_bwd_res_colsum")
            _DX_COLSUM[gx.data_ptr()] = (gx, cs, gx._version)
        else:
            rc = L.load().toda_rows_bn_bwd_res(L.ptr(gy), L.ptr(x), L.ptr(residual), L.ptr(stats), L.ptr(gamma), n, c, int(relu),
                                               L.ptr(sums), L.ptr(gx), L.ptr(gres), L.stream())
            L.check(rc, "toda_rows_bn_bwd_res")
        gs = sums[2 * c:3 * c].view(torch.float32)
        return gx, gs[c:], gs[:c], None, None, None, None, None, None, gres, None, None


def bn_rows(x, bn, relu, residual=None, sums=None, colsum=False):
    training = bn.training or not bn.track_running_stats
    bump_bn_counter(bn)
    momentum = 0.0 if bn.momentum is None else bn.momentum
    return _BNRows.apply(x, bn.weight, bn.bias, bn.running_mean, bn.running_var, training, momentum, bn.eps, relu, residual, sums, colsum)


def bn_rows_supported(x, bn):
    c = x.shape[1]
    return (type(bn) is torch.nn.BatchNorm1d and x.is_cuda and x.dtype == torch.float32 and 4 <= c <= 128 and 256 % c == 0 and bn.affine and bn.momentum is not None
            and x.shape[0] > 1)


_BN2D_SYNC = {}


def _bn2d_sync(device):
    key = (device.index, L.stream())
    ent = _BN2D_SYNC.get(key)
    if ent is None:
        ent = _BN2D_SYNC[key] = [torch.zeros((L.load().toda_bn2d_sync_bytes(),), dtype=torch.uint8, device=device), 0]
    ent[1] = ent[1] % 0xFFFFFFF0 + 1
    return ent[0], ent[1]


class _BN2d(torch.autograd.Function):

    @staticmethod
    def forward(ctx, x, weight, bias, running_mean, running_var, momentum, eps, relu):
        lib = L.load()
        x = x.contiguous()
        b, c, h, w = x.shape
        y = torch.empty_like(x)
        save = torch.empty((2, c), dtype=torch.float32, device=x.device)
        ws, epoch = _bn2d_sync(x.device)
        rc = lib.toda_bn2d_fwd(L.ptr(x), b, c, h * w, L.ptr(weight), L.ptr(bias), L.ptr(running_mean), L.ptr(running_var), float(momentum),
                               float(eps), int(bool(relu)), L.ptr(y), L.ptr(save), L.ptr(ws), epoch, L.stream())
        L.check(rc, "toda_bn2d_fwd")
        ctx.save_for_backward(x, weight, bias, save)
        ctx.relu = bool(relu)
        return y

    @staticmethod
    def backward(ctx, gy):
        x, weight, bias, save = ctx.saved_tensors
        lib = L.load()
        b, c, h, w = x.shape
        gy = gy.contiguous()
        gx = torch.empty_like(x)
        gwb = torch.empty((2, c), dtype=torch.float32, device=x.device)
        ws, epoch = _bn2d_sync(x.device)
        rc = lib.toda_bn2d_bwd(L.ptr(x), L.ptr(gy), b, c, h * w, L.ptr(weight), L.ptr(bias), L.ptr(save), int(ctx.relu), L.ptr(gx),
                               L.ptr(gwb[0]), L.ptr(gwb[1]), L.ptr(ws), epoch, L.stream())
        L.check(rc, "toda_bn2d_bwd")
        return gx, gwb[0], gwb[1], None, None, None, None, None


class _BN2dCat(torch.autograd.Function):

    @staticmethod
    def forward(ctx, relu, n, *flat):
        lib = L.load()
        items = [flat[7 * i:7 * i + 7] for i in range(n)]
        xs = [it[0].contiguous() for it in items]
        b, _, h, w = xs[0].shape
        chans = [x.shape[1] for x in xs]
        out = torch.empty((b, sum(chans), h, w), dtype=torch.float32, device=xs[0].device)
        saves, c0 = [], 0
        for x, it in zip(xs, items):
            _, weight, bias, rm, rv, momentum, eps = it
            c = x.shape[1]
            save = torch.empty((2, c), dtype=torch.float32, device=x.device)
            ws, epoch = _bn2d_sync(x.device)
            rc = lib.toda_bn2d_fwd_into(L.ptr(x), b, c, h * w, L.ptr(weight), L.ptr(bias), L.ptr(rm), L.ptr(rv), float(momentum), float(eps),
                                        int(bool(relu)), L.ptr(out), out.shape[1], c0, L.ptr(save), L.ptr(ws), epoch, L.stream())
            L.check(rc, "toda_bn2d_fwd_into")
            saves.append(save)
            c0 += c
        ctx.save_for_backward(*xs, *[it[1] for it in items], *[it[2] for it in items], *saves)
        ctx.meta = (bool(relu), n, chans)
        return out

    @staticmethod
    def backward(ctx, g):
        relu, n, chans = ctx.meta
        t = ctx.saved_tensors
        xs, weights, biases, saves = t[:n], t[n:2 * n], t[2 * n:3 * n], t[3 * n:]
        lib = L.load()
        g = g.contiguous()
        b, ctot, h, w = g.shape
        grads, c0 = [], 0
        for x, weight, bias, save, c in zip(xs, weights, biases, saves, chans):
            gx = torch.empty_like(x)
            gwb = torch.empty((2, c), dtype=torch.float32, device=x.device)
            ws, epoch = _bn2d_sync(x.device)
            rc = lib.toda_bn2d_bwd_from(L.ptr(x), L.ptr(g), ctot, c0, b, c, h * w, L.ptr(weight), L.ptr(bias), L.ptr(save), int(relu), L.ptr(gx),
                                        L.ptr(gwb[0]), L.ptr(gwb[1]), L.ptr(ws), epoch, L.stream())
            L.check(rc, "toda_bn2d_bwd_from")
            grads += [gx, gwb[0], gwb[1], None, None, None, None]
            c0 += c
        return (None, None, *grads)


FUSED_BN2D = _os.environ.get("TODA_BN2D", "1") == "1"
BN2D_CAT = _os.environ.get("TODA_BN2D_CAT", "1") == "1"


def bn2d_supported(x, bn):
    if not (FUSED_BN2D and type(bn) is torch.nn.BatchNorm2d and bn.training and bn.affine and bn.track_running_stats and bn.momentum is not None):
        return False
    if not (x.is_cuda and x.dtype == torch.float32 and x.dim() == 4 and x.is_contiguous()):
        return False
    return bool(L.load().toda_bn2d_supported(x.shape[0], x.shape[1], x.shape[2] * x.shape[3]))


def bn2d(x, bn, relu):
    bump_bn_counter(bn)
    return _BN2d.apply(x, bn.weight, bn.bias, bn.running_mean, bn.running_var, bn.momentum, bn.eps, relu)


def bn2d_cat(pairs, relu=True):
    flat = []
    for x, bn in pairs:
        bump_bn_counter(bn)
        flat += [x, bn.weight, bn.bias, bn.running_mean, bn.running_var, bn.momentum, bn.eps]
    return _BN2dCat.apply(relu, len(pairs), *flat)


def bn_relu_tail(seq):
    mods = list(seq)
    if len(mods) >= 2 and type(mods[-1]) is torch.nn.ReLU and type(mods[-2]) is torch.nn.BatchNorm2d:
        return mods[:-2], mods[-2]
    return None


def run_dense_sequential(seq, x):
    mods = list(seq)
    i = 0
    while i < len(mods):
        m = mods[i]
        if isinstance(m, torch.nn.Sequential):
            x = run_dense_sequential(m, x)
        elif (type(m) is torch.nn.ZeroPad2d and tuple(m.padding) == (1, 1, 1, 1) and i + 1 < len(mods) and type(mods[i + 1]) is torch.nn.Conv2d
              and mods[i + 1].padding == (0, 0) and conv3x3_supported(x, mods[i + 1])):
            x = conv3x3(x, mods[i + 1].weight, mods[i + 1].bias)
            i += 2
            continue
        elif (type(m) is torch.nn.ZeroPad2d and tuple(m.padding) == (1, 1, 1, 1) and i + 1 < len(mods) and conv3x3s2_supported(x, mods[i + 1])):
            x = conv3x3s2(x, mods[i + 1].weight, mods[i + 1].bias)
            i += 2
            continue
        elif deconv_supported(x, m):
            x = deconv(x, m.weight, m.stride[0], m.bias)
        elif type(m) is torch.nn.Conv2d and m.padding == (1, 1) and conv3x3_supported(x, m):
            x = conv3x3(x, m.weight, m.bias)
        elif type(m) is torch.nn.BatchNorm2d and bn2d_supported(x, m):
            relu = i + 1 < len(mods) and type(mods[i + 1]) is torch.nn.ReLU
            x = bn2d(x, m, relu)
            i += 2 if relu else 1
            continue
        elif type(m) is torch.nn.BatchNorm2d and x.is_cuda and m.track_running_stats and m.momentum is not None:
            bump_bn_counter(m)
            x = torch.nn.functional.batch_norm(x, m.running_mean, m.running_var, m.weight, m.bias, m.training, m.momentum, m.eps)
        else:
            x = m(x)
        i += 1
    return x


DENSE_CONV = _os.environ.get("TODA_DENSE_CONV", "winograd")
_WINO_CACHE = {}


def conv3x3_supported(x, conv):
    if DENSE_CONV != "winograd" or type(conv) is not torch.nn.Conv2d or not x.is_cuda or x.dtype != torch.float32 or x.dim() != 4:
        return False
    if conv.kernel_size != (3, 3) or conv.stride != (1, 1) or conv.dilation != (1, 1) or conv.groups != 1:
        return False
    if conv.padding_mode != "zeros" or conv.in_channels != x.shape[1]:
        return False
    b, c, h, w = x.shape
    return bool(L.load().toda_conv3x3_supported(b, conv.in_channels, conv.out_channels, h, w))


def conv3x3_transform_weight(weight, mode):
    lib = L.load()
    cout, cin = weight.shape[0], weight.shape[1]
    n = lib.toda_conv3x3_weight_floats(cout, cin)
    u = torch.empty((2, n) if mode == 2 else (n,), dtype=torch.float32, device=weight.device)
    L.check(lib.toda_conv3x3_transform_weight(L.ptr(weight.contiguous()), cout, cin, int(mode), L.ptr(u), L.stream()),
            "toda_conv3x3_transform_weight")
    return u


def _conv3x3_workspace(device):
    key = (device.index, L.stream())
    ws = _WINO_CACHE.get(key)
    if ws is None:
        ws = _WINO_CACHE[key] = torch.zeros((L.load().toda_conv3x3_workspace_bytes(),), dtype=torch.uint8, device=device)
    return ws


def conv3x3_run(x, u, bias, cout):
    lib = L.load()
    b, cin, h, w = x.shape
    y = torch.empty((b, cout, h, w), dtype=torch.float32, device=x.device)
    ws = _conv3x3_workspace(x.device)
    L.check(lib.toda_conv3x3_fwd(L.ptr(x), L.ptr(u), L.ptr(bias), b, cin, cout, h, w, L.ptr(y), L.ptr(ws), ws.numel(), L.stream()),
            "toda_conv3x3_fwd")
    return y


class _Conv3x3(torch.autograd.Function):

    @staticmethod
    def forward(ctx, x, weight, bias):
        x = x.contiguous()
        need_dx = ctx.needs_input_grad[0]
        u = conv3x3_transform_weight(weight, 2 if need_dx else 0)
        y = conv3x3_run(x, u[0] if need_dx else u, bias, weight.shape[0])
        ctx.save_for_backward(x, weight, u[1] if need_dx else None)
        ctx.has_bias = bias is not None
        return y

    @staticmethod
    def backward(ctx, gy):
        x, weight, u_dgrad = ctx.saved_tensors
        gy = gy.contiguous()
        gx = gw = gb = None
        if ctx.needs_input_grad[0]:
            gx = conv3x3_run(gy, u_dgrad if u_dgrad is not None else conv3x3_transform_weight(weight, 1), None, weight.shape[1])
        if ctx.needs_input_grad[1]:
            gw = conv3x3_wgrad(x, gy, weight.shape)
        if ctx.has_bias and ctx.needs_input_grad[2]:
            gb = gy.sum((0, 2, 3))
        return gx, gw, gb


def conv3x3_wgrad(x, gy, wshape):
    lib = L.load()
    b, cin, h, w = x.shape
    cout = gy.shape[1]
    dw = torch.empty(tuple(wshape), dtype=torch.float32, device=x.device)
    ws_bytes = lib.toda_conv3x3_wgrad_workspace_bytes(b, cin, cout, h, w)
    ws = torch.empty((max(ws_bytes, 16),), dtype=torch.uint8, device=x.device)
    L.check(lib.toda_conv3x3_wgrad(L.ptr(x), L.ptr(gy), b, cin, cout, h, w, L.ptr(dw), L.ptr(ws), ws_bytes, L.stream()),
            "toda_conv3x3_wgrad")
    return dw


def conv3x3(x, weight, bias=None):
    return _Conv3x3.apply(x, weight, bias)


class _Conv3x3S2(torch.autograd.Function):

    @staticmethod
    def forward(ctx, x, weight):
        lib = L.load()
        x, weight = x.contiguous(), weight.contiguous()
        b, cin, h, w = x.shape
        cout = weight.shape[0]
        y = torch.empty((b, cout, h // 2, w // 2), dtype=torch.float32, device=x.device)
        L.check(lib.toda_conv3x3s2_fwd(L.ptr(x), L.ptr(weight), b, cin, cout, h, w, L.ptr(y), L.stream()), "toda_conv3x3s2_fwd")
        ctx.save_for_backward(x, weight)
        return y

    @staticmethod
    def backward(ctx, gy):
        x, weight = ctx.saved_tensors
        lib = L.load()
        gy = gy.contiguous()
        b, cin, h, w = x.shape
        cout = weight.shape[0]
        gx = gw = None
        if ctx.needs_input_grad[0]:
            gx = torch.empty_like(x)
            L.check(lib.toda_conv3x3s2_dgrad(L.ptr(gy), L.ptr(weight), b, cin, cout, h, w, L.ptr(gx), L.stream()), "toda_conv3x3s2_dgrad")
        if ctx.needs_input_grad[1]:
            gw = torch.empty_like(weight)
            nb = lib.toda_conv3x3s2_wgrad_workspace_bytes(b, cin, cout, h, w)
            ws = torch.empty((max(nb, 16),), dtype=torch.uint8, device=x.device)
            L.check(lib.toda_conv3x3s2_wgrad(L.ptr(x), L.ptr(gy), b, cin, cout, h, w, L.ptr(gw), L.ptr(ws), nb, L.stream()), "toda_conv3x3s2_wgrad")
        return gx, gw


# ... 758 lines not shown
```

Before: 148.6.

## Fuse BatchNorm-backward reductions into sparse-conv dgrad gather-GEMM epilogue

The sparse-conv backward gather-GEMM gains a BatchNorm-backward epilogue. It applies the ReLU mask from the saved BN input and stats, and accumulates the per-channel dz and dz*xhat partial sums while the output tile is still in registers. The following BN rows backward then folds those partials and runs only the apply kernel, skipping its separate pass that rereads dy and x to reduce them. The two ops are linked through Python-side tensor-identity dictionaries, and the pre-activation math is pinned to a non-contracted multiply-add so the masks match across kernels. The cost is extra x loads in the GEMM epilogue and more host-side bookkeeping.

```diff
diff --git a/include/toda.h b/include/toda.h
--- a/include/toda.h
+++ b/include/toda.h
@@ -165,6 +165,9 @@
                                 const float* gamma, int n, int c, int relu, double* sums, float* dx,
                                 float* dres , double* colsum_ws , float* dx_colsum ,
                                 void* stream);
+int toda_rows_bn_bwd_from_partials(const float* dy, const float* x, const float* stats, const float* gamma, int n, int c,
+                                   int relu, double* sums, int blocks, float* dx, double* colsum_ws ,
+                                   float* dx_colsum , void* stream);
 
 int toda_bn2d_supported(int batch, int c, int hw);
 size_t toda_bn2d_sync_bytes(void);
@@ -277,6 +280,15 @@
                                            int n_out, int k_vol, int c_produce, const float* bias , float* out,
                                            double* sums, size_t sums_doubles, int* blocks_out, void* stream);
 
+int toda_spconv_gather_gemm_bnbwd_supported(int c_gather, int c_produce);
+size_t toda_spconv_gather_gemm_bnbwd_doubles(int n_out, int c_produce);
+int toda_spconv_gather_gemm_bnbwd(const float* in, int n_in, int c_gather, const float* wp, const int32_t* nbr, int n_out, int k_vol,
+                                  int c_produce, float* out, const int32_t* order ,
+                                  const unsigned char* cls_sorted , const int32_t* ksize_host,
+                                  const int32_t* stride_host, const int32_t* padding_host, const float* bn_x,
+                                  const float* bn_stats, int relu, double* sums, size_t sums_doubles, int* blocks_out,
+                                  void* stream);
+
 int toda_conv3x3_supported(int batch, int cin, int cout, int H, int W);
 size_t toda_conv3x3_weight_floats(int cout, int cin);
 int toda_conv3x3_transform_weight(const float* w, int cout, int cin, int mode, float* u, void* stream);
diff --git a/toda_amd/csrc/bn_rows.cuh b/toda_amd/csrc/bn_rows.cuh
--- /dev/null
+++ b/toda_amd/csrc/bn_rows.cuh
@@ -0,0 +1,14 @@
+#pragma once
+#include <hip/hip_runtime.h>
+
+namespace toda {
+
+__device__ __forceinline__ float bn_pre(float x, float scale, float shift) {
+#pragma clang fp contract(off)
+    const float p = x * scale;
+    return p + shift;
+}
+
+__device__ __forceinline__ float bn_relu_mask(float g, float pre, int relu) { return (relu && !(pre > 0.f)) ? 0.f : g; }
+
+}
diff --git a/toda_amd/csrc/dense.hip b/toda_amd/csrc/dense.hip
--- a/toda_amd/csrc/dense.hip
+++ b/toda_amd/csrc/dense.hip
@@ -1,4 +1,5 @@
 #include "common.h"
+#include "bn_rows.cuh"
 
 namespace toda {
 
@@ -161,7 +162,10 @@
     const int ch = (int)((t0 * 4) % c);
     const f32x4 sc = *reinterpret_cast<const f32x4*>(scale + ch), sf = *reinterpret_cast<const f32x4*>(shift + ch);
     for (long long t = t0; t < n4; t += stride) {
-        f32x4 v = x[t] * sc + sf;
+        const f32x4 xv = x[t];
+        f32x4 v;
+#pragma unroll
+        for (int j = 0; j < 4; ++j) v[j] = bn_pre(xv[j], sc[j], sf[j]);
         if (res) v += res[t];
         if (relu) {
 #pragma unroll
@@ -189,9 +193,9 @@
         const f32x4 rv = r4 ? r4[(size_t)r * lanes + cl] : f32x4{0.f, 0.f, 0.f, 0.f};
 #pragma unroll
         for (int j = 0; j < 4; ++j) {
-            float pre = xv[j] * sc[j] + sf[j];
+            float pre = bn_pre(xv[j], sc[j], sf[j]);
             if (r4) pre += rv[j];
-            const float dz = (relu && !(pre > 0.f)) ? 0.f : g[j];
+            const float dz = bn_relu_mask(g[j], pre, relu);
             a[j] = dz;
             b[j] = dz * ((xv[j] - mu[j]) * is[j]);
         }
@@ -227,9 +231,9 @@
         f32x4 out, dzv;
 #pragma unroll
         for (int j = 0; j < 4; ++j) {
-            float pre = xv[j] * sc[j] + sf[j];
+            float pre = bn_pre(xv[j], sc[j], sf[j]);
             if (res) pre += rv[j];
-            const float dz = (relu && !(pre > 0.f)) ? 0.f : g[j];
+            const float dz = bn_relu_mask(g[j], pre, relu);
             dzv[j] = dz;
             out[j] = k1[j] * (dz - m1[j] - (xv[j] - mu[j]) * k2[j]);
         }
@@ -451,6 +455,24 @@
     return TODA_OK;
 }
 
+extern "C" int toda_rows_bn_bwd_from_partials(const float* dy, const float* x, const float* stats, const float* gamma, int n, int c, int relu,
+                                              double* sums, int blocks, float* dx, double* colsum_ws, float* dx_colsum, void* stream) {
+    hipStream_t s = (hipStream_t)stream;
+    TODA_CHECK_ARG((colsum_ws == nullptr) == (dx_colsum == nullptr), "rows_bn_bwd_from_partials: colsum workspace and result go together");
+    TODA_CHECK_ARG(c >= 4 && c % 4 == 0 && c <= DN_BLOCK / 2 && DN_BLOCK % c == 0,
+                   "rows_bn_bwd_from_partials: channels must be a multiple of 4 dividing 256, <= 128 (got %d)", c);
+    TODA_CHECK_ARG(n > 0 && blocks >= 1, "rows_bn_bwd_from_partials: needs rows and at least one partial per column (got %d, %d)", n, blocks);
+    TODA_CHECK_ARG(dy && x && stats && gamma && sums && dx, "rows_bn_bwd_from_partials: null argument");
+    hipLaunchKernelGGL(fold_partials_kernel, dim3(2 * c), dim3(DN_BLOCK), 0, s, sums, blocks, 2 * c);
+    const long long n4 = (long long)n * c / 4;
+    const int grid = ew_grid(n4, c);
+    hipLaunchKernelGGL(rows_bn_bwd_apply_kernel, dim3(grid), dim3(DN_BLOCK), 0, s, (const f32x4*)dy, (const f32x4*)x, (const f32x4*)nullptr, stats,
+                       gamma, sums, n4, c, n, relu, (f32x4*)dx, (f32x4*)nullptr, colsum_ws);
+    if (dx_colsum) hipLaunchKernelGGL(colsum_fold_kernel, dim3(c), dim3(DN_BLOCK), 0, s, (const double*)colsum_ws, grid, dx_colsum);
+    TODA_LAUNCH_CHECK();
+    return TODA_OK;
+}
+
 extern "C" int toda_rows_bn_bwd_res(const float* dy, const float* x, const float* residual, const float* stats,
                                     const float* gamma, int n, int c, int relu, double* sums, float* dx, float* dres,
                                     void* stream) {
diff --git a/toda_amd/csrc/spconv.hip b/toda_amd/csrc/spconv.hip
--- a/toda_amd/csrc/spconv.hip
+++ b/toda_amd/csrc/spconv.hip
@@ -1187,7 +1187,8 @@
 
 static int gather_gemm_impl(const float* in, int n_in, int c_gather, const float* wp, const int32_t* nbr, int n_out, int k_vol,
                             int c_produce, const float* bias, float* out, const int32_t* order, double* stats, void* stream,
-                            const unsigned char* cls_sorted = nullptr, const toda::GatherClasses* cls_table = nullptr);
+                            const unsigned char* cls_sorted = nullptr, const toda::GatherClasses* cls_table = nullptr,
+                            const toda::BnBwdEpilogue* bnb = nullptr);
 
 namespace toda {
 constexpr int CLS_ROWS = 8192, CLS_PER = CLS_ROWS / 256;
@@ -1348,9 +1349,44 @@
     const int Q = tiles_pow2(c_gather), NT = tiles_pow2(c_produce);
     return (c_gather & 3) == 0 && Q >= 2 && NT >= Q && Q * NT <= 32 && !(Q == 8 && NT == 8) && c_produce % 4 == 0 && c_produce == 16 * NT;
 }
-}
-
-
+static bool gg_bnbwd_supported(int c_gather, int c_produce) {
+    return use_split(c_gather, c_produce) &&
+           ((c_gather == 32 && c_produce == 32) || (c_gather == 64 && (c_produce == 32 || c_produce == 64)) || (c_gather == 128 && c_produce == 128));
+}
+}
+
+extern "C" int toda_spconv_gather_gemm_bnbwd_supported(int c_gather, int c_produce) { return gg_bnbwd_supported(c_gather, c_produce) ? 1 : 0; }
+
+extern "C" size_t toda_spconv_gather_gemm_bnbwd_doubles(int n_out, int c_produce) { return toda_spconv_gather_gemm_stats_doubles(n_out, c_produce); }
+
+extern "C" int toda_spconv_gather_gemm_bnbwd(const float* in, int n_in, int c_gather, const float* wp, const int32_t* nbr, int n_out, int k_vol,
+                                             int c_produce, float* out, const int32_t* order, const unsigned char* cls_sorted,
+                                             const int32_t* ksize, const int32_t* stride, const int32_t* padding, const float* bn_x,
+                                             const float* bn_stats, int relu, double* sums, size_t sums_doubles, int* blocks_out, void* stream) {
+    TODA_CHECK_ARG(gg_bnbwd_supported(c_gather, c_produce), "gather_gemm_bnbwd: unsupported channel pair (%d -> %d) on matrix path %d", c_gather,
+                   c_produce, matrix_path());
+    TODA_CHECK_ARG(n_out > 0 && n_in > 0 && k_vol >= 1, "gather_gemm_bnbwd: empty table (%d rows from %d)", n_out, n_in);
+    TODA_CHECK_ARG(in && wp && nbr && out && bn_x && bn_stats && sums && blocks_out, "gather_gemm_bnbwd: null argument");
+    TODA_CHECK_ARG(((uintptr_t)bn_x & 15) == 0 && ((uintptr_t)bn_stats & 15) == 0, "gather_gemm_bnbwd: bn_x and bn_stats must be 16-byte aligned");
+    TODA_CHECK_ARG(sums_doubles >= toda_spconv_gather_gemm_bnbwd_doubles(n_out, c_produce), "gather_gemm_bnbwd: sums buffer too small");
+    TODA_CHECK_ARG(cls_sorted == nullptr || (order && ksize && stride && padding), "gather_gemm_bnbwd: a class-sorted launch needs order, ksize, stride and padding");
+    GatherClasses table;
+    if (cls_sorted) {
+        TODA_CHECK_ARG(ksize[0] * ksize[1] * ksize[2] == k_vol, "gather_gemm_bnbwd: kernel size does not match the table's %d offsets", k_vol);
+        TODA_CHECK_ARG(class_table(ksize, stride, padding, &table) == 0, "gather_gemm_bnbwd: needs <= 8 residue classes and <= 27 offsets");
+    }
+    const toda::BnBwdEpilogue bnb{bn_x, bn_stats, relu ? 1 : 0};
+    *blocks_out = 0;
+    g_stats_blocks_out = blocks_out;
+    const int rc = gather_gemm_impl(in, n_in, c_gather, wp, nbr, n_out, k_vol, c_produce, nullptr, out, order, sums, stream, cls_sorted,
+                                    cls_sorted ? &table : nullptr, &bnb);
+    g_stats_blocks_out = nullptr;
+    if (rc == TODA_OK && *blocks_out <= 0) {
+        set_error("gather_gemm_bnbwd: the launch took no sums");
+        return TODA_EINVAL;
+    }
+    return rc;
+}
 
 extern "C" int toda_spconv_gather_gemm_ordered(const float* in, int n_in, int c_gather, const float* wp, const int32_t* nbr,
                                                int n_out, int k_vol, int c_produce, const float* bias, float* out,
@@ -1395,7 +1431,7 @@
 
 static int gather_gemm_impl(const float* in, int n_in, int c_gather, const float* wp, const int32_t* nbr, int n_out, int k_vol,
                             int c_produce, const float* bias, float* out, const int32_t* order, double* stats, void* stream,
-                            const unsigned char* cls_sorted, const toda::GatherClasses* cls_table) {
+                            const unsigned char* cls_sorted, const toda::GatherClasses* cls_table, const toda::BnBwdEpilogue* bnb) {
     toda::GatherClasses classes = {};
     if (cls_sorted && cls_table) classes = *cls_table;
     else cls_sorted = nullptr;
@@ -1404,6 +1440,8 @@
     TODA_CHECK_ARG(n_out >= 0 && n_in >= 0 && k_vol >= 1, "gather_gemm: bad sizes");
     TODA_CHECK_ARG((unsigned long long)n_in * c_gather * 4ull < 0xFFFFFFF0ull, "gather_gemm: gathered table must be < 4 GiB");
     if (n_out == 0) return TODA_OK;
+    TODA_CHECK_ARG(bnb == nullptr || (n_in > 0 && stats != nullptr && gg_bnbwd_supported(c_gather, c_produce)),
+                   "gather_gemm: no BatchNorm-backward epilogue for this launch (%d -> %d, matrix path %d)", c_gather, c_produce, matrix_path());
     if (n_in == 0) {
         TODA_CHECK_ARG(bias == nullptr, "gather_gemm: empty input with bias is unsupported");
         TODA_HIP(hipMemsetAsync(out, 0, (size_t)n_out * c_produce * sizeof(float), (hipStream_t)stream));
@@ -1415,14 +1453,20 @@
     static const int env_lds_raw = getenv("TODA_GG_LDS") ? atoi(getenv("TODA_GG_LDS")) : 1;
     const int env_lds = env_lds_raw == 2 ? 1 : (env_lds_raw == 1 ? (Q >= 2 && NT >= Q) : 0);
     if (use_split(c_gather, c_produce)) {
-        TODA_CHECK_ARG(k_vol >= 1 && !(cls_sorted && stats), "gather_gemm (split path): no statistics on a class-sorted launch");
+        TODA_CHECK_ARG(k_vol >= 1 && !(cls_sorted && stats && !bnb), "gather_gemm (split path): no statistics on a class-sorted launch");
         const toda::u32x4* wps = reinterpret_cast<const toda::u32x4*>(wp);
-#define SPL(KK, SS, NN, BB, WW)                                                                                                            \
-    GG_LAUNCH(HIP_KERNEL_NAME(gg_split_kernel<KK, SS, NN, 2, BB, WW, (NN == 2)>), dim3(cdiv(cdiv(n_out, 32), BB / 64)), dim3(BB), 0, s, in, n_in, wps, \
-              nbr, n_out, k_vol, c_produce, bias, out, order, stats, cls_sorted, classes)
+#define SPL_(KK, SS, NN, BB, WW, BNB, ARG)                                                                                                 \
+    GG_LAUNCH(HIP_KERNEL_NAME(gg_split_kernel<KK, SS, NN, 2, BB, WW, (NN == 2), BNB>), dim3(cdiv(cdiv(n_out, 32), BB / 64)), dim3(BB), 0, s, in, n_in, \
+              wps, nbr, n_out, k_vol, c_produce, bias, out, order, stats, cls_sorted, classes, ARG)
+#define SPL(KK, SS, NN, BB, WW) SPL_(KK, SS, NN, BB, WW, false, toda::BnBwdEpilogue{})
         const int blk = 256;
         const int kc = c_gather / 32, nt = c_produce / 16;
-        if (0) {}
+        if (bnb) {
+            if (kc == 1 && nt == 2) SPL_(1, 1, 2, 256, 4, true, *bnb);
+            else if (kc == 2 && nt == 2) SPL_(2, 1, 2, 256, 4, true, *bnb);
+            else if (kc == 2 && nt == 4) SPL_(2, 1, 4, 256, 4, true, *bnb);
+            else SPL_(4, 1, 8, 256, 3, true, *bnb);
+        }
         else if (kc == 1 && nt == 2) SPL(1, 1, 2, 256, 4);
         else if (kc == 1 && nt == 4) SPL(1, 1, 4, 256, 4);
         else if (kc == 1 && nt == 8) SPL(1, 1, 8, 256, 3);
@@ -1433,6 +1477,7 @@
         else if (kc == 4 && nt == 4) SPL(4, 1, 4, 256, 4);
         else SPL(4, 1, 8, 256, 3);
 #undef SPL
+#undef SPL_
         TODA_LAUNCH_CHECK();
         if (stats) {
             fold_or_defer(stats, cdiv(cdiv(n_out, 32), blk / 64), c_produce, s);
diff --git a/toda_amd/csrc/spconv_split.cuh b/toda_amd/csrc/spconv_split.cuh
--- a/toda_amd/csrc/spconv_split.cuh
+++ b/toda_amd/csrc/spconv_split.cuh
@@ -1,5 +1,6 @@
 #pragma once
 #include "split_common.cuh"
+#include "bn_rows.cuh"
 
 namespace toda {
 
@@ -87,11 +88,16 @@
                          (unsigned)v[6] | ((unsigned)v[7] << 16)};
 }
 
-template <int KC, int KCS, int NT, int RT, int BLK, int WAVES, bool IL = false>
+struct BnBwdEpilogue {
+    const float* x;
+    const float* stats;
+    int relu;
+};
+template <int KC, int KCS, int NT, int RT, int BLK, int WAVES, bool IL = false, bool BNB = false>
 __global__ void __launch_bounds__(BLK, WAVES)
 gg_split_kernel(const float* __restrict__ in, int n_in, const u32x4* __restrict__ wps, const int* __restrict__ nbr, int n_out, int K, int cp,
                 const float* __restrict__ bias, float* __restrict__ out, const int* __restrict__ order, double* __restrict__ stats,
-                const unsigned char* __restrict__ cls_sorted, const GatherClasses classes) {
+                const unsigned char* __restrict__ cls_sorted, const GatherClasses classes, const BnBwdEpilogue bnb) {
     static_assert(KC % KCS == 0, "whole stages per offset");
     constexpr int CG = 32 * KC;
     constexpr int SPO = KC / KCS;
@@ -322,18 +328,61 @@
     if (stats) {
         float (*st_sh)[2][16 * NT] = reinterpret_cast<float (*)[2][16 * NT]>(wl);
         float sm[NT], sq[NT];
+        if constexpr (BNB) {
+            auto load_nt = [](const float* __restrict__ p, float (&v)[NT]) {
+                if constexpr (NT == 2) {
+                    const float2 t = *reinterpret_cast<const float2*>(p);
+                    v[0] = t.x, v[1] = t.y;
+                } else {
+#pragma unroll
+                    for (int n = 0; n < NT; n += 4) {
+                        const f32x4 t = *reinterpret_cast<const f32x4*>(p + n);
+                        v[n] = t[0], v[n + 1] = t[1], v[n + 2] = t[2], v[n + 3] = t[3];
+                    }
+                }
+            };
+            float mu[NT], is[NT], sc[NT], sf[NT];
+            load_nt(bnb.stats + NT * r, mu);
+            load_nt(bnb.stats + cp + NT * r, is);
+            load_nt(bnb.stats + 2 * cp + NT * r, sc);
+            load_nt(bnb.stats + 3 * cp + NT * r, sf);
+#pragma unroll
+            for (int n = 0; n < NT; ++n) sm[n] = sq[n] = 0.0f;
+#pragma unroll
+            for (int rt = 0; rt < RT; ++rt) {
+                float xv[4][NT];
+#pragma unroll
+                for (int reg = 0; reg < 4; ++reg) {
+                    const int pos = row0 + rt * 16 + 4 * g + reg;
+                    const int row = __shfl(rows[rt], 4 * g + reg, 64);
+                    load_nt(bnb.x + (size_t)(pos < n_out ? row : 0) * cp + NT * r, xv[reg]);
+                }
+#pragma unroll
+                for (int reg = 0; reg < 4; ++reg) {
+                    if (row0 + rt * 16 + 4 * g + reg >= n_out) continue;
+#pragma unroll
+                    for (int n = 0; n < NT; ++n) {
+                        const float dz = bn_relu_mask(acc[rt][n][reg], bn_pre(xv[reg][n], sc[n], sf[n]), bnb.relu);
+                        sm[n] += dz;
+                        sq[n] += dz * ((xv[reg][n] - mu[n]) * is[n]);
+                    }
+                }
+            }
+        }
 #pragma unroll
         for (int n = 0; n < NT; ++n) {
-            sm[n] = sq[n] = 0.0f;
-#pragma unroll
-            for (int rt = 0; rt < RT; ++rt)
-#pragma unroll
-                for (int reg = 0; reg < 4; ++reg)
-                    if (row0 + rt * 16 + 4 * g + reg < n_out) {
-                        const float v = acc[rt][n][reg];
-                        sm[n] += v;
-                        sq[n] += v * v;
-                    }
+            if constexpr (!BNB) {
+                sm[n] = sq[n] = 0.0f;
+#pragma unroll
+                for (int rt = 0; rt < RT; ++rt)
+#pragma unroll
+                    for (int reg = 0; reg < 4; ++reg)
+                        if (row0 + rt * 16 + 4 * g + reg < n_out) {
+                            const float v = acc[rt][n][reg];
+                            sm[n] += v;
+                            sq[n] += v * v;
+                        }
+            }
             sm[n] += __shfl_xor(sm[n], 16, 64);
             sq[n] += __shfl_xor(sq[n], 16, 64);
             sm[n] += __shfl_xor(sm[n], 32, 64);
diff --git a/toda_amd/lib.py b/toda_amd/lib.py
--- a/toda_amd/lib.py
+++ b/toda_amd/lib.py
@@ -48,6 +48,9 @@
     "toda_spconv_gather_gemm_stats_doubles": (_sz, [_i, _i]),
     "toda_spconv_gather_gemm_stats": (_i, [_vp, _i, _i, _vp, _vp, _i, _i, _i, _vp, _vp, _vp, _sz, _vp]),
     "toda_spconv_gather_gemm_stats_partials": (_i, [_vp, _i, _i, _vp, _vp, _i, _i, _i, _vp, _vp, _vp, _sz, _vp, _vp]),
+    "toda_spconv_gather_gemm_bnbwd_supported": (_i, [_i, _i]),
+    "toda_spconv_gather_gemm_bnbwd_doubles": (_sz, [_i, _i]),
+    "toda_spconv_gather_gemm_bnbwd": (_i, [_vp, _i, _i, _vp, _vp, _i, _i, _i, _vp, _vp, _vp, _vp, _vp, _vp, _vp, _vp, _i, _vp, _sz, _vp, _vp]),
     "toda_spconv_gather_gemm_compact_supported": (_i, [_i, _i, _i]),
     "toda_spconv_gather_gemm_compact": (_i, [_vp, _i, _i, _vp, _i, _i, _i, _i, _vp, _i, _i, _i, _vp, _vp, _vp]),
     "toda_spconv_gather_gemm_compact_stats_doubles": (_sz, [_i, _i]),
@@ -67,6 +70,7 @@
     "toda_rows_bn_bwd_res": (_i, [_vp, _vp, _vp, _vp, _vp, _i, _i, _i, _vp, _vp, _vp, _vp]),
     "toda_rows_bn_bwd_colsum_doubles": (_sz, [_i, _i]),
     "toda_rows_bn_bwd_res_colsum": (_i, [_vp, _vp, _vp, _vp, _vp, _i, _i, _i, _vp, _vp, _vp, _vp, _vp, _vp]),
+    "toda_rows_bn_bwd_from_partials": (_i, [_vp, _vp, _vp, _vp, _i, _i, _i, _vp, _i, _vp, _vp, _vp, _vp]),
     "toda_conv3x3s2_supported": (_i, [_i, _i, _i, _i, _i]),
     "toda_conv3x3s2_fwd": (_i, [_vp, _vp, _i, _i, _i, _i, _i, _vp, _vp]),
     "toda_conv3x3s2_dgrad": (_i, [_vp, _vp, _i, _i, _i, _i, _i, _vp, _vp]),
diff --git a/toda_amd/ops.py b/toda_amd/ops.py
--- a/toda_amd/ops.py
+++ b/toda_amd/ops.py
@@ -648,7 +648,33 @@
     return bool(L.load().toda_spconv_gather_gemm_stats_supported(int(c_gather), int(c_produce)))
 
 
-def gather_gemm_with_stats(feat, wp, nbr, c_produce, bias=None, partials=False):
+def gather_gemm_bn_bwd_supported(c_gather, c_produce):
+    return bool(L.load().toda_spconv_gather_gemm_bnbwd_supported(int(c_gather), int(c_produce)))
+
+
+def _gather_gemm_bn_bwd(feat, wp, nbr, c_produce, bn_bwd, order=None, cls_sorted=None, geom=None):
+    import ctypes
+    lib = L.load()
+    K, n_out = nbr.shape
+    x, stats, relu = bn_bwd
+    assert x.shape == (n_out, c_produce) and x.is_contiguous() and stats.shape == (4, c_produce) and stats.is_contiguous()
+    out = torch.empty((n_out, c_produce), dtype=torch.float32, device=feat.device)
+    nd = lib.toda_spconv_gather_gemm_bnbwd_doubles(n_out, c_produce)
+    sums = torch.empty((nd,), dtype=torch.float64, device=feat.device)
+    blocks = ctypes.c_int(0)
+    ks, st, pd = (L.host_i32(g) for g in geom) if geom is not None else (None, None, None)
+    rc = lib.toda_spconv_gather_gemm_bnbwd(L.ptr(feat), feat.shape[0], feat.shape[1], L.ptr(wp), L.ptr(nbr), n_out, K, c_produce, L.ptr(out),
+                                           L.ptr(order), L.ptr(cls_sorted), L.hptr(ks) if ks is not None else None,
+                                           L.hptr(st) if st is not None else None, L.hptr(pd) if pd is not None else None, L.ptr(x), L.ptr(stats),
+                                           int(bool(relu)), L.ptr(sums), nd, ctypes.addressof(blocks), L.stream())
+    L.check(rc, "toda_spconv_gather_gemm_bnbwd")
+    return out, sums, int(blocks.value)
+
+
+def gather_gemm_with_stats(feat, wp, nbr, c_produce, bias=None, partials=False, bn_bwd=None, order=None):
+    if bn_bwd is not None:
+        assert bias is None
+        return _gather_gemm_bn_bwd(feat, wp, nbr, c_produce, bn_bwd, order=order)
     lib = L.load()
     K, n_out = nbr.shape
     out = torch.empty((n_out, c_produce), dtype=torch.float32, device=feat.device)
@@ -723,7 +749,9 @@
     return out
 
 
-def gather_gemm_classed(feat, wp, nbr, c_produce, order, cls_sorted, ksize, stride, padding):
+def gather_gemm_classed(feat, wp, nbr, c_produce, order, cls_sorted, ksize, stride, padding, bn_bwd=None):
+    if bn_bwd is not None:
+        return _gather_gemm_bn_bwd(feat, wp, nbr, c_produce, bn_bwd, order=order, cls_sorted=cls_sorted, geom=(ksize, stride, padding))
     lib = L.load()
     K, n_out = nbr.shape
     out = torch.empty((n_out, c_produce), dtype=torch.float32, device=feat.device)
@@ -786,6 +814,7 @@
         ctx.rb = rb
         ctx.wp_bwd = wp_bwd
         ctx.has_bias = bias is not None
+        ctx.bn_bwd = _take_bn_out(features) if (features.is_cuda and ctx.needs_input_grad[0]) else None
         if want_stats:
             ctx.mark_non_differentiable(sums)
             return out, sums, blocks
@@ -815,7 +844,18 @@
             wp_t = ctx.wp_bwd if ctx.wp_bwd is not None else pack_weight(weight, True, rb.flip_bwd)
             _check_mm(wp_t)
             co = rb.class_order()
-            if co is not None:
+            bnb = ctx.bn_bwd
+            if bnb is not None and not (BN_BWD_EPILOGUE and gout.shape[0] > 0 and rb.nbr_bwd.shape[1] > 0
+                                        and gather_gemm_bn_bwd_supported(gout.shape[1], weight.shape[-1])):
+                bnb = None
+            if bnb is not None:
+                if co is not None:
+                    gfeat, part, blocks = gather_gemm_classed(gout, wp_t, rb.nbr_bwd, weight.shape[-1], co[0], co[1], rb.ksize, rb.geom["stride"],
+                                                              rb.geom["padding"], bnb)
+                else:
+                    gfeat, part, blocks = gather_gemm_with_stats(gout, wp_t, rb.nbr_bwd, weight.shape[-1], None, bn_bwd=bnb)
+                _DY_SUMS[gfeat.data_ptr()] = (gfeat, (part, blocks, bnb[0].data_ptr()), gfeat._version)
+            elif co is not None:
                 gfeat = gather_gemm_classed(gout, wp_t, rb.nbr_bwd, weight.shape[-1], co[0], co[1], rb.ksize, rb.geom["stride"], rb.geom["padding"])
             else:
                 gfeat = gather_gemm(gout, wp_t, rb.nbr_bwd, weight.shape[-1], None)
@@ -933,6 +973,27 @@
     return ent[1]
 
 
+BN_BWD_EPILOGUE = _os.environ.get("TODA_BN_BWD_EPILOGUE", "1") == "1"
+_BN_OUT = {}
+_DY_SUMS = {}
+
+
+def _same_tensor(ent, t):
+    return ent is not None and ent[0].shape == t.shape and ent[0]._version == ent[2] and t.stride() == ent[0].stride()
+
+
+def _take_bn_out(features):
+    ent = _BN_OUT.pop(features.data_ptr(), None) if _BN_OUT else None
+    return ent[1] if _same_tensor(ent, features) else None
+
+
+def _take_dy_sums(gy, x):
+    ent = _DY_SUMS.pop(gy.data_ptr(), None) if _DY_SUMS else None
+    if not _same_tensor(ent, gy) or ent[1][2] != x.data_ptr():
+        return None
+    return ent[1][0], ent[1][1]
+
+
 class _BNRows(torch.autograd.Function):
 
     @staticmethod
@@ -940,6 +1001,10 @@
         lib = L.load()
         if _DX_COLSUM:
             _DX_COLSUM.clear()
+        if _DY_SUMS:
+            _DY_SUMS.clear()
+        if _BN_OUT:
+            _BN_OUT.clear()
         ctx.colsum = bool(colsum) and BN_BWD_COLSUM
         x = x.contiguous()
         residual = residual.contiguous() if residual is not None else None
@@ -962,6 +1027,8 @@
         L.check(rc, "toda_rows_affine_act")
         ctx.save_for_backward(x, stats, weight, residual)
         ctx.meta = (n, c, bool(relu), bool(training))
+        if BN_BWD_EPILOGUE and training and residual is None and x.is_cuda and n > 0 and ctx.needs_input_grad[0]:
+            _BN_OUT[y.data_ptr()] = (y, (x.detach(), stats, bool(relu)), y._version)
         return y
 
     @staticmethod
@@ -990,9 +1057,24 @@
             gx = dz * stats[2]
             xhat = (x - stats[0]) * stats[1]
             return gx, (dz * xhat).sum(0), dz.sum(0), None, None, None, None, None, None, (dz if want_res else None), None, None
-        sums = torch.empty((L.load().toda_rows_reduce_doubles(n, c),), dtype=torch.float64, device=x.device)
         gx = torch.empty_like(x)
         gamma = weight if weight is not None else torch.ones(c, device=x.device)
+        pre = _take_dy_sums(gy, x) if (_DY_SUMS and residual is None) else None
+        if pre is not None:
+            lib = L.load()
+            sums, blocks = pre
+            cs_ws = cs = None
+            if ctx.colsum:
+                cs_ws = torch.empty((lib.toda_rows_bn_bwd_colsum_doubles(n, c),), dtype=torch.float64, device=x.device)
+                cs = torch.empty((c,), dtype=torch.float32, device=x.device)
+            rc = lib.toda_rows_bn_bwd_from_partials(L.ptr(gy), L.ptr(x), L.ptr(stats), L.ptr(gamma), n, c, int(relu), L.ptr(sums), int(blocks),
+                                                    L.ptr(gx), L.ptr(cs_ws), L.ptr(cs), L.stream())
+            L.check(rc, "toda_rows_bn_bwd_from_partials")
+            if ctx.colsum:
+                _DX_COLSUM[gx.data_ptr()] = (gx, cs, gx._version)
+            gs = sums[2 * c:3 * c].view(torch.float32)
+            return gx, gs[c:], gs[:c], None, None, None, None, None, None, None, None, None
+        sums = torch.empty((L.load().toda_rows_reduce_doubles(n, c),), dtype=torch.float64, device=x.device)
         gres = torch.empty_like(x) if want_res else None
         if ctx.colsum:
             lib = L.load()
```

After: 149.5 (median of 6 runs). About the same (+0.7%).
